# Andrcraft9/ocean_model_arch

Measured on AMD Instinct MI355X. Metric: cell-updates/s, SW barotropic step on 4096x4096 box; %HBM BW at 1/2/4/8 GPU, higher is better.
Workload: dtype f64

## Files before the change

### include/ocn_sw.h

```cpp
#ifndef OCN_SW_H
#define OCN_SW_H

#include <stdint.h>

#ifdef __cplusplus
extern "C" {
#endif

#define OCN_ABI_VERSION 5

enum {
    OCN_OK = 0,
    OCN_ERR_ARG = 1,
    OCN_ERR_HIP = 2,
    OCN_ERR_COMM = 3,
    OCN_ERR_STATE = 4,
    OCN_ERR_BLOWUP = 5
};

typedef struct ocn_block {
    int32_t nx_start, nx_end, ny_start, ny_end;
    int32_t bnd_x1, bnd_x2, bnd_y1, bnd_y2;
    int64_t pitch;
} ocn_block;
// ... 168 lines not shown
int ocn_ctx_comm_info(ocn_ctx *ctx, ocn_comm_info *out);
typedef struct ocn_overlap_info {
    int32_t level, state, kind, pad;
    double seq_ms, overlapped_ms;
} ocn_overlap_info;
int ocn_ctx_overlap_info(ocn_ctx *ctx, ocn_overlap_info *out);
typedef struct ocn_clock_info {
    int64_t launches;
    double clock_ghz, sampled_ms;
} ocn_clock_info;
int ocn_ctx_clock_info(ocn_ctx *ctx, int32_t reset, ocn_clock_info *out);
int ocn_ctx_set_watchdog(ocn_ctx *ctx, double seconds);

int ocn_ctx_set_topography(ocn_ctx *ctx, const float *h, int64_t count);
int ocn_ctx_init_state(ocn_ctx *ctx);

int ocn_ctx_sync(ocn_ctx *ctx, int field_id);
int ocn_ctx_stage(ocn_ctx *ctx, int stage_id, double tau);
int ocn_ctx_tracer_stage(ocn_ctx *ctx, int stage_id, int tracer, double tau);
int ocn_ctx_step(ocn_ctx *ctx, double tau, int32_t nsteps, int32_t check_every);
int ocn_ctx_synchronize(ocn_ctx *ctx);
int ocn_ctx_complete(ocn_ctx *ctx);

int ocn_ctx_download(ocn_ctx *ctx, int k, int field_id, void *host);
int ocn_ctx_upload(ocn_ctx *ctx, int k, int field_id, const void *host);
int ocn_ctx_output_r4(ocn_ctx *ctx, int k, int field_id, float undef, float *host);

int ocn_ctx_set_option(ocn_ctx *ctx, int32_t key, int64_t value);
int ocn_ctx_get_option(const ocn_ctx *ctx, int32_t key, int64_t *value);
enum { OCN_OPT_GRAPH = 1, OCN_OPT_OVERLAP = 2, OCN_OPT_STAGE_TIMING = 3, OCN_OPT_FUSED = 4, OCN_OPT_COMPACT = 5,
       OCN_OPT_MARCH = 6, OCN_OPT_FLIP = 7, OCN_OPT_RECOMPUTE = 8, OCN_OPT_ONEPASS = 9,
       OCN_OPT_KNOWN_CONSTANTS = 10, OCN_OPT_ONEPASS_LAST = 11, OCN_OPT_LAZY_TAIL = 12, OCN_OPT_X2 = 13,
       OCN_OPT_BATCH = 14, OCN_OPT_PAIR = 15, OCN_OPT_MULTI = 16, OCN_OPT_TRACER_STEP = 17,
       OCN_OPT_MULTI_SPIN = 18, OCN_OPT_X4 = 19, OCN_OPT_CO_LAUNCH = 20, OCN_OPT_XCHG_DELAY = 21 };

enum { OCN_TIMER_FUSED_A = OCN_NUM_STAGES, OCN_TIMER_FUSED_B, OCN_TIMER_FUSED_C1, OCN_TIMER_TRACER,
       OCN_TIMER_FUSED_CA = OCN_TIMER_TRACER + OCN_NUM_TSTAGES, OCN_TIMER_ONEPASS, OCN_TIMER_ONEPASS2,
       OCN_TIMER_ONEPASS2_LAST, OCN_TIMER_ONEPASS_MULTI, OCN_TIMER_TRACER_STEP, OCN_TIMER_EXCHANGE,
       OCN_TIMER_EXPOSED, OCN_NUM_TIMERS };

int ocn_ctx_stage_times(ocn_ctx *ctx, double *ms, int64_t *counts);
int ocn_ctx_stage_stats(ocn_ctx *ctx, double *ms, int64_t *counts, double *ms_max);

#define OCN_ENS_MAX_MEMBERS 256
typedef struct ocn_ens_group {
    int32_t variant, rows, tiles, members;
    int32_t member[OCN_ENS_MAX_MEMBERS];
    int32_t first_tile[OCN_ENS_MAX_MEMBERS];
} ocn_ens_group;
int ocn_ens_plan(const ocn_block *geom, const int32_t *variant, int32_t members, int64_t capacity, ocn_ens_group *out,
                 int32_t cap, int32_t *count);

typedef struct ocn_ens ocn_ens;
int ocn_ens_create(const ocn_basin *basin, const ocn_sw_params *sw, const ocn_decomp *dec, const int32_t *mask,
                   int32_t members, ocn_ens **out);
int ocn_ens_destroy(ocn_ens *ens);
int ocn_ens_size(const ocn_ens *ens);
int ocn_ens_member(ocn_ens *ens, int32_t i, ocn_ctx **out);
int ocn_ens_init_state(ocn_ens *ens);
int ocn_ens_step(ocn_ens *ens, double tau, int32_t nsteps, int32_t check_every);
int ocn_ens_complete(ocn_ens *ens);
int ocn_ens_synchronize(ocn_ens *ens, int32_t *status);
typedef struct ocn_ens_info_t {
    int32_t members, groups, batched, rows, tiles, max_group;
    int64_t capacity;
} ocn_ens_info_t;
int ocn_ens_info(ocn_ens *ens, ocn_ens_info_t *out);
// ... 20 lines not shown
```

### ocean_model_arch_amd/_codeobj.py

```python
from __future__ import annotations

import hashlib
import struct

_BUNDLE_MAGIC = b"__CLANG_OFFLOAD_BUNDLE__"


def _sections(elf: bytes):
    if elf[:4] != b"\x7fELF" or elf[4] != 2 or elf[5] != 1:
        raise ValueError("not an ELF64 little-endian image")
    shoff, = struct.unpack_from("<Q", elf, 0x28)
    shentsize, shnum, shstrndx = struct.unpack_from("<HHH", elf, 0x3A)
    hdrs = []
    for i in range(shnum):
        name, _typ, _flags, addr, off, size = struct.unpack_from("<IIQQQQ", elf, shoff + i * shentsize)
        hdrs.append((name, addr, off, size))
    stroff = hdrs[shstrndx][2]
    out = {}
    for i, (name, addr, off, size) in enumerate(hdrs):
        end = elf.index(b"\0", stroff + name)
        out[elf[stroff + name:end].decode()] = (off, size, addr, i)
    return out


# ... 10 lines not shown
            triple = fat[p + 24:p + 24 + tlen].decode()
            p += 24 + tlen
            if triple.endswith("gfx950"):
                yield fat[pos + eoff:pos + eoff + esize]
        pos = fat.find(_BUNDLE_MAGIC, pos + 1)


def gfx950_code_object(lib_path: str) -> bytes:
    for code in gfx950_code_objects(lib_path):
        return code
    raise ValueError("no gfx950 code object in " + lib_path)


def kernel_symbols(code: bytes) -> dict:
    secs = _sections(code)
    symoff, symsize, _a, _i = secs[".symtab"]
    stroff = secs[".strtab"][0]
    by_index = {v[3]: v for v in secs.values()}
    out = {}
    for k in range(symsize // 24):
        st_name, st_info, _other, shndx, value, size = struct.unpack_from("<IBBHQQ", code, symoff + 24 * k)
        if (st_info & 0xF) != 2 or size == 0 or shndx not in by_index:
            continue
        end = code.index(b"\0", stroff + st_name)
        name = code[stroff + st_name:end].decode()
        off, _s, addr, _i = by_index[shndx]
        start = off + (value - addr)
        out[name] = code[start:start + size]
    return out


def march_step_symbol(args: str, batched: bool = False) -> str:
    bits = "".join("Lb1E" if a.strip() == "true" else "Lb0E" for a in args.split(","))
    if batched:
        return f"_ZN3ocn9k_march_bINS_9MarchStepII{bits}EEEEvNS_10MarchGridBENS_4PackIT_EE".replace("II", "I")
    return f"_ZN3ocn7k_marchINS_9MarchStepII{bits}EEEEvNS_9MarchGridET_".replace("II", "I")


def kernel_code_sha(lib_path: str, symbol: str) -> str | None:
    syms = kernel_symbols(gfx950_code_object(lib_path))
    code = syms.get(symbol)
    return hashlib.sha256(code).hexdigest()[:16] if code is not None else None


def sha_by_demangled(lib_path: str, names) -> dict:
    import subprocess
    syms = kernel_symbols(gfx950_code_object(lib_path))
    mangled = sorted(syms)
    dem = subprocess.run(["c++filt"], input="\n".join(mangled), capture_output=True, text=True, check=True).stdout.split("\n")
    key = {"".join(d.split()): m for m, d in zip(mangled, dem)}
    out = {}
    for n in names:
        m = key.get("".join(n.split()))
        if m:
            out[n] = (m, hashlib.sha256(syms[m]).hexdigest()[:16])
    return out
```

### ocean_model_arch_amd/_lib.py

```python
from __future__ import annotations

import ctypes as C
import os
import re
import subprocess

_HERE = os.path.dirname(os.path.abspath(__file__))
LIB_PATH = os.environ.get("OCN_LIB_PATH") or os.path.join(_HERE, "libocn_sw.so")
_CSRC = os.path.join(_HERE, "csrc")

OCN_OK, OCN_ERR_ARG, OCN_ERR_HIP, OCN_ERR_COMM, OCN_ERR_STATE, OCN_ERR_BLOWUP = range(6)

R4_NAMES = ["lu", "luu", "luh", "lcu", "lcv", "llu", "llv", "dx", "dy", "dxt", "dyt", "dxh", "dyh",
            "dxb", "dyb", "rlh_s", "r_diss"]
R8_NAMES = ["ssh", "sshn", "sshp", "ubrtr", "ubrtrn", "ubrtrp", "vbrtr", "vbrtrn", "vbrtrp",
            "hhq", "hhq_p", "hhq_n", "hhu", "hhu_p", "hhu_n", "hhv", "hhv_p", "hhv_n",
            "hhh", "hhh_p", "hhh_n", "hhq_rest", "vort", "str_t", "str_s", "mu",
            "RHSx", "RHSy", "RHSx_adv", "RHSy_adv", "RHSx_dif", "RHSy_dif"]
OCN_FIELD_END = 32 + len(R8_NAMES)
OCN_TRACER_BASE = OCN_FIELD_END + 2
MAX_TRACERS = 64
_TRACER_RE = re.compile(r"^(ff1|ff1p|ff1n)_([0-9]+)$")


# ... 24 lines not shown


def is_r8_name(name: str) -> bool:
    return name not in R4_NAMES

STAGES = ["sw_update_ssh", "hh_update", "uv_trans_vort", "uv_trans", "stress_components", "uv_diff2",
          "sw_update_uv", "sw_next_step", "hh_shift", "hh_init", "check_ssh_err"]
STAGE_ID = {n: i for i, n in enumerate(STAGES)}
TSTAGES = ["tran_diff_fluxes", "tran_diff_tracer", "tracer_next_step"]
TSTAGE_ID = {n: i for i, n in enumerate(TSTAGES)}
TIMERS = STAGES + ["fused_a", "fused_b", "fused_c1"] + TSTAGES + ["fused_ca", "onepass", "onepass2", "onepass2_last", "onepass_multi", "tracer_step",
                                                                       "exchange", "exposed"]
OPT_GRAPH = 1
OPT_OVERLAP = 2
OPT_STAGE_TIMING = 3
OPT_FUSED = 4
OPT_COMPACT = 5
OPT_MARCH = 6
OPT_FLIP = 7
OPT_RECOMPUTE = 8
OPT_ONEPASS = 9
OPT_KNOWN_CONSTANTS = 10
OPT_ONEPASS_LAST = 11
OPT_LAZY_TAIL = 12
OPT_X2 = 13
OPT_BATCH = 14
OPT_PAIR = 15
OPT_MULTI = 16
OPT_TRACER_STEP = 17
OPT_MULTI_SPIN = 18
OPT_X4 = 19
OPT_CO_LAUNCH = 20
OPT_XCHG_DELAY = 21

KERNEL_SYMBOLS = ["ocn_sw_update_ssh", "ocn_hh_update", "ocn_uv_trans_vort", "ocn_uv_trans",
                  "ocn_stress_components", "ocn_uv_diff2", "ocn_sw_update_uv", "ocn_sw_next_step",
                  "ocn_hh_shift", "ocn_hh_init", "ocn_check_ssh_err", "ocn_tran_diff_fluxes",
                  "ocn_tran_diff_tracer", "ocn_tracer_next_step"]
CTX_SYMBOLS = ["ocn_decompose", "ocn_halo_schedule", "ocn_ctx_create", "ocn_ctx_destroy", "ocn_ctx_block_count", "ocn_ctx_block_info",
               "ocn_ctx_field", "ocn_ctx_stream", "ocn_comm_unique_id", "ocn_ctx_attach_comm", "ocn_ctx_attach_loopback",
               "ocn_ctx_set_topography", "ocn_ctx_init_state", "ocn_ctx_sync", "ocn_ctx_stage", "ocn_ctx_tracer_stage", "ocn_ctx_step", "ocn_ctx_synchronize",
               "ocn_ctx_download", "ocn_ctx_complete", "ocn_ctx_upload", "ocn_ctx_output_r4", "ocn_ctx_set_option", "ocn_ctx_get_option", "ocn_ctx_stage_times", "ocn_ctx_stage_stats",
               "ocn_ctx_comm_info", "ocn_ctx_overlap_info", "ocn_ctx_clock_info", "ocn_ctx_set_watchdog", "ocn_last_error", "ocn_abi_version",
               "ocn_build_id", "ocn_launch_count"]
ENS_SYMBOLS = ["ocn_ens_plan", "ocn_ens_create", "ocn_ens_destroy", "ocn_ens_size", "ocn_ens_member",
               "ocn_ens_init_state", "ocn_ens_step", "ocn_ens_complete", "ocn_ens_synchronize", "ocn_ens_info",
               "ocn_ens_set_option", "ocn_ens_stats", "ocn_ens_stats_download", "ocn_ens_stats_output_r4",
               "ocn_ens_extrema"]
ALL_SYMBOLS = KERNEL_SYMBOLS + CTX_SYMBOLS + ENS_SYMBOLS
ENS_MAX_MEMBERS = 256
ENS_OPT_CAPACITY = 1
ENS_OPT_MAX_GROUP = 2
ENS_STATS = {"mean": 1, "var": 2, "spread": 4, "min": 8, "max": 16}


class OcnLibraryError(RuntimeError):
    pass


class OcnError(RuntimeError):
    def __init__(self, code: int, msg: str):
        super().__init__(f"[ocn error {code}] {msg}")
        self.code = code


class OcnBlock(C.Structure):
# ... 162 lines not shown
```

### ocean_model_arch_amd/csrc/ctx_setup.hip

```cpp
#include "ocn_ctx.h"

namespace ocn {

__global__ void k_topography(ocn_block g, double *h, const float *lu, const float *topo, int nxi)
{
    const int w = g.bnd_x2 - g.bnd_x1 + 1, rows = g.bnd_y2 - g.bnd_y1 + 1;
    const long i = (long)blockIdx.x * blockDim.x + threadIdx.x;
    if (i >= (long)w * rows) return;
    const int m = g.bnd_x1 + (int)(i % w), n = g.bnd_y1 + (int)(i / w);
    const long at = (long)(m - g.bnd_x1) + (long)(n - g.bnd_y1) * g.pitch;
    float v = 0.0f;
    if (m >= g.nx_start && m <= g.nx_end && n >= g.ny_start && n <= g.ny_end) v = topo[(long)(m - 3) + (long)(n - 3) * nxi];
    if (fabsf(lu[at]) < 0.5f) v = 0.0f;
    h[at] = (double)v;
}

__global__ void k_fill_r8(double *p, long n, double v)
{
    long i = (long)blockIdx.x * blockDim.x + threadIdx.x;
    if (i < n) p[i] = v;
}

static std::vector<int> uniform_sizes(int total, int parts, std::string &err)
{
// ... 185 lines not shown
        for (int id = OCN_SSH; id < OCN_SSH + nr8; ++id)
            if (std::find(order.begin(), order.end(), id) == order.end()) order.push_back(id);
        for (int k = 1; k <= ntr; ++k) order.push_back(-3 - k);
        b.ffp_alt.assign((size_t)ntr, nullptr);
        for (int id : order) {
            char *p = base + off + 256 - 16 + xr;
            off += r8b;
            if (id == -1) b.sshp_alt = p;
            else if (id == -2) b.up_alt = p;
            else if (id == -3) b.vp_alt = p;
            else if (id < -3) b.ffp_alt[(size_t)(-4 - id)] = p;
            else b.ptr[field_slot(id)] = p;
        }
        for (int id = 0; id < OCN_NUM_R4; ++id) {
            b.ptr[field_slot(id)] = base + off + 256 - 8;
            off += r4b;
        }
    }
    for (LBlock &b : c->blocks) {
        const size_t n = (size_t)b.g.pitch * (b.g.bnd_y2 - b.g.bnd_y1 + 1);
        const size_t nrow = row_table_size((unsigned)(b.g.bnd_y2 - b.g.bnd_y1 + 1));
        HIPCHK(hipMalloc(&b.bits, n));
        c->allocs.push_back(b.bits);
        HIPCHK(hipMalloc(&b.rows, nrow * sizeof(float)));
        c->allocs.push_back(b.rows);
        RC(allocate_x2(c, b));
    }
    const size_t kcb = 16 * c->blocks.size();
    HIPCHK(hipMalloc(&c->d_nbad, 256 + kcb));
    c->allocs.push_back(c->d_nbad);
    HIPCHK(hipMalloc(&c->d_bar, kMultiBarBytes));
    c->allocs.push_back(c->d_bar);
    HIPCHK(hipMemsetAsync(c->d_nbad, 0, 256 + kcb, c->stream));
    c->d_fbz = c->d_nbad + 16;
    c->d_flags = c->d_nbad + 32;
    for (size_t i = 0; i < c->blocks.size(); ++i) c->blocks[i].kc = (double *)((char *)c->d_nbad + 256) + 2 * i;
    return OCN_OK;
}

int prepare_static(ocn_ctx *c)
{
    if (!c->compact_req || c->r4_escaped) { c->compact = false; return OCN_OK; }
    if (!c->static_dirty) return OCN_OK;
    HIPCHK(hipMemsetAsync(c->d_flags, 0, 3 * sizeof(int32_t), c->stream));
    RC(each_block(c, c->stream, [&](const LBlock &b) { return launch_prepare(&b.g, b.ptr.data(), b.bits, b.rows, c->d_flags, c->stream, b.own); }));
    if (c->ext_ok)
        for (const LBlock &b : c->blocks) RC(launch_rows_ext(&b.g, b.rows, b.rows_x, b.ext, c->d_flags + 1, c->stream));
    const bool x4_tabs = c->ext_ok && has_exchange(c);
    int32_t *d_mask = nullptr;
    if (x4_tabs) {
        const size_t nxy = (size_t)c->basin.nx * c->basin.ny;
        HIPCHK(hipMallocAsync((void **)&d_mask, nxy * sizeof(int32_t), c->stream));
        HIPCHK(hipMemcpyAsync(d_mask, c->mask.data(), nxy * sizeof(int32_t), hipMemcpyHostToDevice, c->stream));
        for (const LBlock &b : c->blocks)
            RC(launch_x4_tables(&b.g, b.bits, b.rows, b.ext, b.bits_x4, b.rows_x4, d_mask, c->basin.nx, c->basin.ny, b.own,
                                c->d_flags + 2, c->stream));
        HIPCHK(hipFreeAsync(d_mask, c->stream));
    }
    int32_t flags[3] = {0, 0, 0};
    HIPCHK(hipMemcpyAsync(flags, c->d_flags, sizeof(flags), hipMemcpyDeviceToHost, c->stream));
    HIPCHK(hipStreamSynchronize(c->stream));
    c->ring_sea = (flags[0] & kCompactRingSea) != 0;
    c->edge_ring_sea = (flags[0] & kCompactEdgeRingSea) != 0;
    c->udiv_ok = (flags[0] & kCompactDivisorRange) == 0;
    c->rows_x_ok = c->ext_ok && flags[1] == 0;
    c->x4_tab_ok = x4_tabs && flags[2] == 0;
    c->compact = (flags[0] & ~(kCompactRingSea | kCompactDivisorRange | kCompactEdgeRingSea)) == 0;
    c->static_dirty = false;
    return OCN_OK;
}

static const float kPi = 3.1415926f;
static const double kDPi = 3.14159265358979;
static const double kLatExtr = 89.99999;
static const float kRadEarth = 6371000.0f;
static const float kEarthAngVel = 7.2921159e-5f;
static double dsind(double x) { return std::sin((x / 180.0) * kDPi); }
static double dcosd(double x) { return std::cos((x / 180.0) * kDPi); }

struct GridTables {
    std::vector<float> cos_t, cos_v;
    std::vector<double> sin_v, cosy_v, cos_xu;
    float ext_ct[kExtRows], ext_cv[kExtRows];
    double ext_sin_v[kExtRows], ext_cosy_v[kExtRows];
};
static void grid_tables(const ocn_ctx *c, const ocn_block &g, GridTables &t)
{
    const ocn_basin &bs = c->basin;
    const int w = g.bnd_x2 - g.bnd_x1 + 1, h = g.bnd_y2 - g.bnd_y1 + 1, mmm = 3, nnn = 3;
    std::vector<double> xt(w), xu(w, 0.0), yt(h), yv(h, 0.0);
    for (int m = g.bnd_x1; m <= g.bnd_x2; ++m) xt[m - g.bnd_x1] = bs.rlon + (double)(m - mmm) * bs.dxst;
    for (int n = g.bnd_y1; n <= g.bnd_y2; ++n) yt[n - g.bnd_y1] = bs.rlat + (double)(n - nnn) * bs.dyst;
    for (int i = 0; i + 1 < w; ++i) xu[i] = (xt[i] + xt[i + 1]) / 2.0;
    for (int i = 0; i + 1 < h; ++i) yv[i] = (yt[i] + yt[i + 1]) / 2.0;
    auto lat_mod = [](double y) { return std::max(std::min(y, kLatExtr), -kLatExtr); };
    t.cos_t.assign(h, 0.0f); t.cos_v.assign(h, 0.0f); t.sin_v.assign(h, 0.0); t.cosy_v.assign(h, 0.0);
    t.cos_xu.assign(w, 0.0);
    for (int n = g.ny_start - 1; n <= g.ny_end + 1; ++n) {
        const int r = n - g.bnd_y1;
        t.cos_t[r] = (float)dcosd(lat_mod(yt[r]));
// ... 193 lines not shown
```

### ocean_model_arch_amd/csrc/ocn_ctx.h

```cpp
#pragma once
#include <hip/hip_runtime.h>
#include <rccl/rccl.h>

#include <algorithm>
#include <array>
#include <atomic>
#include <chrono>
#include <cmath>
#include <condition_variable>
#include <cstdio>
#include <cstdlib>
#include <cstring>
#include <deque>
#include <map>
#include <mutex>
#include <string>
#include <thread>
#include <vector>

#include "ocn_internal.h"

namespace ocn {

#define HIPCHK(call)                                          \
// ... 106 lines not shown

#ifndef OCN_COMM_PRIO
#define OCN_COMM_PRIO 1
#endif
struct ocn_ctx {
    ocn_basin basin;
    ocn_sw_params sw;
    ocn_decomp dec;
    std::vector<int32_t> mask;
    std::vector<float> topo;
    int bnx = 1, bny = 1;
    std::vector<GBlock> gblocks;
    std::vector<LBlock> blocks;
    hipStream_t stream = nullptr;
    hipStream_t comm_stream = nullptr;
    hipEvent_t ev_fork = nullptr, ev_join = nullptr;
    hipEvent_t ev_fb = nullptr;
    int32_t *h_fbz = nullptr;
    bool fb_copy = false;
    int overlap = -1;
    int ov_state = 0, ov_kind = 0, ov_level = 2;
    hipEvent_t ov_ev[4] = {nullptr, nullptr, nullptr, nullptr};
    double ov_ms[2] = {0.0, 0.0};
    int xdelay_us = 0;
    int32_t *d_nbad = nullptr;
    unsigned *d_bar = nullptr;
    ncclComm_t comm = nullptr;
    bool comm_aborted = false;
    Loopback *lb = nullptr;
    hipEvent_t lb_ev_a = nullptr, lb_ev_b = nullptr;
    std::map<std::vector<int>, HaloPlan> plans;
    bool initialized = false;
    bool use_graph = false;
    struct Graph { hipGraphExec_t exec; double tau; ocn::StepKind kind; bool compact, march, ring_sea; int role, kc_mode; };
    std::vector<Graph> graphs;
    std::vector<void *> allocs;
    bool stage_timing = false;
    struct Rec { int stage; hipEvent_t a, b; };
    std::vector<Rec> recs;
    std::vector<hipEvent_t> event_pool;
    double stage_ms[OCN_NUM_TIMERS] = {0};
    int64_t stage_n[OCN_NUM_TIMERS] = {0};
    bool fused = true;
    std::vector<int> sync_a, sync_a_reuse, sync_b, sync_ca, sync_ca_reuse;
    bool compact_req = true, compact = false, static_dirty = true;
    bool march = true;
    mutable bool r4_escaped = false;
    bool flip = true, coherent = false, flip_used = false, rc_used = false;
    bool capturing = false;
    bool sync_pending = false;
    bool ring_sea = true;
    bool udiv_ok = true;
    bool recompute = true;
    bool onepass = true;
    int pair = 1;
    bool pair_used = false;
    bool multi = true, multi_used = false;
    bool tr_step = true, tr_call = false, tr_pending = false;
    bool tr_forked = false;
    mutable bool tr_alt_ok = false;
    bool known_const = true;
    bool last_hybrid = true;
    bool one_used = false;
    mutable bool alt_ok = false;
    mutable bool hh_consistent = false, r8_handed = false;
    mutable bool hn_fresh = false;
    mutable bool hqn_stale = false;
    mutable int fb_state = 0;
    int kc_mode = 0;
    int32_t *d_fbz = nullptr;
    bool lazy = true, open = false, open_x2 = false;
    double open_tau = 0.0;
    bool open_pair = false;
    int deferred = 0;
    bool deferred_check[2] = {false, false};
    bool x2 = true, rows_x_ok = false, edge_ring_sea = true, x2_dev_ok = false;
    mutable bool ext_ok = false, hrx_ok = false;
    bool ring2_saved = false, x2_used = false;
    int x4 = 1;
    bool x4_tab_ok = false, x4_dev_ok = false, x4_used = false;
    bool fb_x2 = false;
    mutable bool coherent_known = false, r8_escaped = false;
    int multi_spin = kMultiSpin;
    bool co_launch = true, co_used = false;
    double stage_max[OCN_NUM_TIMERS] = {0};
    int64_t xchg = 0, xdone = -1;
    std::mutex xmu;
    std::deque<std::pair<int64_t, hipEvent_t>> xq;
    std::vector<hipEvent_t> xpool;
    double wd_s = 0;
    std::thread wd;
    std::mutex wd_mu;
    std::condition_variable wd_cv;
    bool wd_stop = false;
    int call_depth = 0;
    std::chrono::steady_clock::time_point call_t0;
    const char *call_name = "";
    std::atomic<bool> wd_fired{false};
    std::string wd_msg;
    std::mutex comm_mu;
    bool comm_abort_done = false;
    int role = 0;
    int steps_run = 0;
    int64_t launches = 0;
    int32_t *d_flags = nullptr;
    bool batch = true;
    ocn::Batcher batcher;
    ocn_ens *ens = nullptr;
    bool ens_collect = false, ens_pending = false;
    ocn::StepKind ens_k{};
};

namespace ocn {

inline int num_r8(const ocn_ctx *c)
{
    return OCN_NUM_R8 + (c->sw.use_tracers > 0 ? 2 + 3 * c->sw.tracer_num : 0);
}
inline bool has_r8(const ocn_ctx *c, int id) { return id >= OCN_SSH && id < OCN_SSH + num_r8(c); }
inline bool has_field(const ocn_ctx *c, int id) { return is_r4(id) || has_r8(c, id); }
inline bool is_tracer_field(int id) { return id >= OCN_TRACER_BASE; }
inline bool is_alt_field(int id) { return id == OCN_SSHP || id == OCN_UBRTRP || id == OCN_VBRTRP; }
inline size_t field_bytes(const LBlock &b) { return (size_t)b.g.pitch * (b.g.bnd_y2 - b.g.bnd_y1 + 1) * 8; }
inline bool has_comm(const ocn_ctx *c) { return c->comm || c->lb || c->comm_aborted; }
inline OnepassKC kc_of(const ocn_ctx *c, const LBlock &b) { return OnepassKC{c->kc_mode, c->d_fbz, b.kc}; }

int make_seglist(ocn_ctx *c, const std::vector<Seg> &v, SegList &out);
int launch_segs(const SegList &l, hipStream_t s, int32_t *cmp = nullptr);
int get_plan(ocn_ctx *c, const std::vector<int> &fields, HaloPlan *&out, int depth = 1, int priv = 0);
int run_sync(ocn_ctx *c, const std::vector<int> &fields, hipStream_t stream = nullptr, int32_t *cmp = nullptr,
             int depth = 1, int priv = 0);
constexpr int kVoteWords = 8;
int allreduce_max(ocn_ctx *c, int32_t *word, hipStream_t s, int words = 1);
int nccl_rc(ncclResult_t r, const char *what);
int fail_fatal(ocn_ctx *c, int rc);
int64_t poll_xdone(ocn_ctx *c);
void wd_loop(ocn_ctx *c);

struct CallGuard {
    ocn_ctx *c;
    CallGuard(ocn_ctx *ctx, const char *name);
    ~CallGuard();
};
template <class F> static int guarded(ocn_ctx *c, const char *name, F &&f)
{
    if (c->wd_fired.load()) return set_error(OCN_ERR_COMM, c->wd_msg);
    int rc;
    {
        CallGuard g(c, name);
        rc = f();
    }
    if (c->wd_fired.load()) {
        std::lock_guard<std::mutex> g(c->comm_mu);
        if (c->comm) { c->comm = nullptr; c->comm_aborted = true; }
        return set_error(OCN_ERR_COMM, c->wd_msg);
    }
    return rc;
}

void set_mask(ocn_ctx *c, const int32_t *mask);
int decompose(ocn_ctx *c);
int host_ctx(const ocn_basin *basin, const ocn_decomp *dec, const int32_t *mask, ocn_ctx *&c);
int allocate(ocn_ctx *c);
int upload_field(ocn_ctx *c, const LBlock &b, int id, const void *host, bool async);
// ... 42 lines not shown
```

### ocean_model_arch_amd/csrc/ocn_ctx.hip

```cpp
#include "ocn_ctx.h"

namespace ocn {

static thread_local std::string g_last_error;

int set_error(int code, const std::string &msg)
{
    g_last_error = msg;
    return code;
}

static std::atomic<long long> g_launches{0};
void count_launch() { g_launches.fetch_add(1, std::memory_order_relaxed); }

int check_hip(hipError_t e, const char *what)
{
    if (e == hipSuccess) return OCN_OK;
    return set_error(OCN_ERR_HIP, std::string(what) + ": " + hipGetErrorString(e));
}

template <typename T>
__global__ void k_output_r4(const T *src, const float *lu, long pitch, int w, int h, float undef, float *dst)
{
    const int i = (int)(blockIdx.x * blockDim.x + threadIdx.x), j = (int)blockIdx.y;
// ... 303 lines not shown
    c->role ^= 16;
}
static int copy_to_alt(ocn_ctx *c, int nsw, bool tracers)
{
    for (LBlock &b : c->blocks) {
        const std::pair<void *, int> sw[3] = {{b.sshp_alt, OCN_SSHP}, {b.up_alt, OCN_UBRTRP}, {b.vp_alt, OCN_VBRTRP}};
        for (int i = 0; i < nsw; ++i)
            HIPCHK(hipMemcpyAsync(sw[i].first, b.ptr[field_slot(sw[i].second)], field_bytes(b), hipMemcpyDeviceToDevice,
                                  c->stream));
        for (int t = 1; tracers && t <= c->sw.tracer_num; ++t)
            HIPCHK(hipMemcpyAsync(b.ffp_alt[(size_t)t - 1], b.ptr[field_slot(OCN_FF1P(t))], field_bytes(b),
                                  hipMemcpyDeviceToDevice, c->stream));
    }
    return OCN_OK;
}
static int copy_pairs(ocn_ctx *c)
{
    for (const LBlock &b : c->blocks)
        for (const auto &pr : kFlipPairs)
            HIPCHK(hipMemcpyAsync(b.ptr[field_slot(pr[1])], b.ptr[field_slot(pr[0])], field_bytes(b),
                                  hipMemcpyDeviceToDevice, c->stream));
    return OCN_OK;
}
static bool is_flip_field(int id)
{
    for (const auto &pr : kFlipPairs)
        if (id == pr[0] || id == pr[1]) return true;
    return id >= OCN_TRACER_BASE && (id - OCN_TRACER_BASE) % 3 != 1;
}

enum { kVoteIncoherent = 0, kVoteIneligible, kVoteUdiv, kVoteHhStale, kVoteX2, kVoteX4, kVoteOvSeq, kVoteOvOv,
       kVoteUsed };
static_assert(kVoteUsed <= kVoteWords, "vote words");
struct VoteIn { bool eligible, udiv_ok, hh_consistent, x2_ok, x4_ok; };
struct VoteOut { bool udiv_ok, hh_consistent, x2_ok, x4_ok; };

struct HaloZero {
    const double *a[6], *d[9];
    int w, h, nxs, nxe, nys, nye, bx1, by1;
    long pitch;
    unsigned own;
};
__global__ void k_halo_zero(HaloZero q, int32_t *flag)
{
    const long i = (long)blockIdx.x * blockDim.x + threadIdx.x;
    if (i >= (long)q.w * q.h) return;
    const int m = q.bx1 + (int)(i % q.w), n = q.by1 + (int)(i / q.w);
    const unsigned cx = m < q.nxs ? 0u : m > q.nxe ? 2u : 1u, cy = n < q.nys ? 0u : n > q.nye ? 2u : 1u;
    if ((cx == 1u && cy == 1u) || ((q.own >> (cx * 3u + cy)) & 1u)) return;
    const long at = (i % q.w) + (i / q.w) * q.pitch;
    auto nz = [&](const double *p) {
        unsigned long long x;
        const double v = p[at];
        __builtin_memcpy(&x, &v, 8);
        return x != 0ull;
    };
    bool bad = false;
    for (int k = 0; k < 6; ++k) bad |= nz(q.a[k]);
    const bool outer = (m == q.nxe + 1 && n >= q.nys - 1 && n <= q.nye + 1) ||
                       (n == q.nye + 1 && m >= q.nxs - 1 && m <= q.nxe + 1);
    if (outer)
        for (int k = 0; k < 9; ++k) bad |= nz(q.d[k]);
    if (bad) atomicOr(flag, 1);
}
static int launch_halo_zero(ocn_ctx *c, int32_t *flag)
{
    static const int ids[6] = {OCN_SSH, OCN_SSHP, OCN_UBRTR, OCN_UBRTRP, OCN_VBRTR, OCN_VBRTRP};
    static const int dids[9] = {OCN_HHU, OCN_HHU_P, OCN_HHU_N, OCN_HHV, OCN_HHV_P, OCN_HHV_N, OCN_HHH, OCN_HHH_P, OCN_HHH_N};
    for (const LBlock &b : c->blocks) {
        HaloZero q{};
        for (int k = 0; k < 6; ++k) q.a[k] = b.f<double>(ids[k]);
        for (int k = 0; k < 9; ++k) q.d[k] = b.f<double>(dids[k]);
        q.w = b.g.bnd_x2 - b.g.bnd_x1 + 1; q.h = b.g.bnd_y2 - b.g.bnd_y1 + 1;
        q.nxs = b.g.nx_start; q.nxe = b.g.nx_end; q.nys = b.g.ny_start; q.nye = b.g.ny_end;
        q.bx1 = b.g.bnd_x1; q.by1 = b.g.bnd_y1; q.pitch = (long)b.g.pitch; q.own = b.own;
        const long pts = (long)q.w * q.h;
        hipLaunchKernelGGL(k_halo_zero, dim3((unsigned)((pts + 255) / 256)), dim3(256), 0, c->stream, q, flag);
        RC(check_launch());
    }
    return OCN_OK;
}

static int check_coherence(ocn_ctx *c, const VoteIn &in, VoteOut &out)
{
    int32_t host[kVoteWords] = {0};
    host[kVoteIneligible] = !in.eligible;
    host[kVoteUdiv] = !in.udiv_ok;
    host[kVoteHhStale] = !in.hh_consistent;
    host[kVoteX2] = !in.x2_ok;
    host[kVoteX4] = !in.x4_ok;
    host[kVoteOvSeq] = host[kVoteOvOv] = INT32_MAX;
    if (c->ov_state == 2) {
        float ms[2] = {0.f, 0.f};
        HIPCHK(hipEventSynchronize(c->ov_ev[3]));
        HIPCHK(hipEventElapsedTime(&ms[0], c->ov_ev[0], c->ov_ev[1]));
        HIPCHK(hipEventElapsedTime(&ms[1], c->ov_ev[2], c->ov_ev[3]));
        for (int i = 0; i < 2; ++i) {
            c->ov_ms[i] = ms[i];
            host[kVoteOvSeq + i] = (int32_t)std::min(1.0e9, std::max(1.0, std::round(1000.0 * ms[i])));
        }
    }
    HIPCHK(hipMemcpyAsync(c->d_flags, host, sizeof(host), hipMemcpyHostToDevice, c->stream));
    if (in.eligible)
        RC(each_block(c, c->stream, [&](const LBlock &b) { return launch_coherence(&b.g, b.ptr.data(), b.bits, c->d_flags, c->stream); }));
    if (in.eligible && c->sw.use_tracers > 0 && c->tr_step)
        for (int t = 1; t <= c->sw.tracer_num; ++t)
            RC(each_block(c, c->stream, [&](const LBlock &b) {
                return launch_tracer_coherence(&b.g, b.ptr.data(), b.bits, t, c->d_flags, c->stream);
            }));
    const bool exch = has_exchange(c);
    if (exch) RC(run_sync(c, kHaloCheck, c->stream, c->d_flags));
    if (exch && c->x2) {
        RC(run_sync(c, {OCN_SSHP, OCN_UBRTRP, OCN_VBRTRP}, c->stream, c->d_flags + kVoteX2));
        if (c->sw.use_tracers > 0 && c->tr_step) RC(run_sync(c, {OCN_MU}, c->stream, c->d_flags + kVoteX2));
        RC(launch_halo_zero(c, c->d_flags + kVoteX2));
    }
    RC(allreduce_max(c, c->d_flags, c->stream, kVoteUsed));
    int32_t w[kVoteWords] = {0};
    HIPCHK(hipMemcpyAsync(w, c->d_flags, sizeof(int32_t) * kVoteUsed, hipMemcpyDeviceToHost, c->stream));
    HIPCHK(hipStreamSynchronize(c->stream));
    c->coherent = w[kVoteIncoherent] == 0 && w[kVoteIneligible] == 0;
    c->coherent_known = !c->r8_escaped && !has_comm(c);
    out.udiv_ok = w[kVoteUdiv] == 0;
    out.hh_consistent = w[kVoteHhStale] == 0;
    out.x2_ok = w[kVoteX2] == 0 && exch && c->x2;
    c->x2_dev_ok = out.x2_ok;
    out.x4_ok = out.x2_ok && w[kVoteX4] == 0;
    if (w[kVoteOvSeq] != INT32_MAX && w[kVoteOvOv] != INT32_MAX) {
        c->ov_ms[0] = 1.0e-3 * w[kVoteOvSeq];
        c->ov_ms[1] = 1.0e-3 * w[kVoteOvOv];
        c->ov_level = w[kVoteOvOv] < w[kVoteOvSeq] ? 2 : 1;
        c->ov_state = 3;
    } else if (c->ov_state == 2) {
        c->ov_state = 0;
    }
    c->x4_dev_ok = out.x4_ok;
    return OCN_OK;
}

static bool flip_eligible(ocn_ctx *c)
{
    return c->flip && c->fused && c->compact && c->march;
}

static bool reuse_allowed(const ocn_ctx *c)
{
    return c->sw.trans_terms > 0 || !(has_exchange(c) || has_comm(c));
}

static int run_tracer_step(ocn_ctx *c, double tau);
static int run_tracer_step(ocn_ctx *c, double tau, hipStream_t st);
static int tracer_step_block(ocn_ctx *c, const LBlock &b, int k, double tau, hipStream_t st);
static std::vector<int> with_tracers(const ocn_ctx *c, const std::vector<int> &fields);

static bool side_fed(const LBlock &b, int side)
{
    static const int diag[5][2] = {{0, 0}, {5, 6}, {7, 8}, {5, 7}, {6, 8}};
    return b.nbr_rank[side - 1] >= 0 || b.nbr_rank[diag[side][0] - 1] >= 0 || b.nbr_rank[diag[side][1] - 1] >= 0;
}
static Range inner_range(const LBlock &b, int ew, int ns)
{
    Range r{b.g.nx_start, b.g.nx_end, b.g.ny_start, b.g.ny_end};
    if (side_fed(b, 2)) r.m0 += ew;
    if (side_fed(b, 1)) r.m1 -= ew;
    if (side_fed(b, 4)) r.n0 += ns;
    if (side_fed(b, 3)) r.n1 -= ns;
    return r;
}
static int band_cols(const LBlock &b, int tile, int depth)
// ... 701 lines not shown
#ifndef OCN_BUILD_ID
#define OCN_BUILD_ID "unknown"
#endif
const char *ocn_build_id(void) { return OCN_BUILD_ID; }
int64_t ocn_launch_count(void) { return (int64_t)g_launches.load(std::memory_order_relaxed); }

extern "C++" int ocn::ctx_create(const ocn_basin *basin, const ocn_sw_params *sw, const ocn_decomp *dec, const int32_t *mask,
                                 hipStream_t shared, ocn_ens *ens, ocn_ctx **out)
{
    if (!basin || !sw || !dec || !out) return set_error(OCN_ERR_ARG, "null argument");
    if (basin->nx < 5 || basin->ny < 5) return set_error(OCN_ERR_ARG, "nx, ny must be >= 5");
    if (dec->bnx < 1 || dec->bny < 1 || dec->nranks < 1 || dec->rank < 0 || dec->rank >= dec->nranks)
        return set_error(OCN_ERR_ARG, "bad decomposition request");
    if (sw->use_tracers > 0 && (sw->tracer_num < 1 || sw->tracer_num > kMaxTracers))
        return set_error(OCN_ERR_ARG, "tracer_num must be 1.." + std::to_string(kMaxTracers));
    ocn_ctx *c = new ocn_ctx();
    c->basin = *basin; c->sw = *sw; c->dec = *dec;
    c->bnx = dec->bnx; c->bny = dec->bny;
    c->ens = ens;
    set_mask(c, mask);
    int rc = check_hip(hipSetDevice(dec->device), "hipSetDevice");
    if (shared) c->stream = shared;
    else if (!rc) rc = check_hip(hipStreamCreateWithFlags(&c->stream, hipStreamNonBlocking), "hipStreamCreate");
    if (!rc) {
        int lo = 0, hi = 0;
        rc = check_hip(hipDeviceGetStreamPriorityRange(&lo, &hi), "hipDeviceGetStreamPriorityRange");
        if (!rc)
            rc = check_hip(hipStreamCreateWithPriority(&c->comm_stream, hipStreamNonBlocking, OCN_COMM_PRIO ? hi : lo),
                           "hipStreamCreateWithPriority");
    }
    if (!rc) rc = check_hip(hipEventCreateWithFlags(&c->ev_fork, hipEventDisableTiming), "hipEventCreate");
    if (!rc) rc = check_hip(hipEventCreateWithFlags(&c->ev_join, hipEventDisableTiming), "hipEventCreate");
    if (!rc) rc = check_hip(hipEventCreateWithFlags(&c->ev_fb, hipEventDisableTiming), "hipEventCreate");
    if (!rc) rc = check_hip(hipHostMalloc((void **)&c->h_fbz, sizeof(int32_t), hipHostMallocDefault), "hipHostMalloc");
    if (!rc) rc = decompose(c);
    if (!rc) rc = allocate(c);
    if (!rc) rc = prebuild_plans(c);
    if (!rc) rc = check_hip(hipStreamSynchronize(c->stream), "hipStreamSynchronize");
    if (rc) { ctx_destroy(c); return rc; }
    *out = c;
    return OCN_OK;
}

int ocn_ctx_create(const ocn_basin *basin, const ocn_sw_params *sw, const ocn_decomp *dec, const int32_t *mask,
                   ocn_ctx **out)
{
    return ctx_create(basin, sw, dec, mask, nullptr, nullptr, out);
}

int ocn_ctx_destroy(ocn_ctx *c)
{
    if (c && c->ens) return set_error(OCN_ERR_ARG, "a member of an ensemble is destroyed by ocn_ens_destroy");
    return ctx_destroy(c);
}

extern "C++" int ocn::ctx_destroy(ocn_ctx *c)
{
    if (!c) return OCN_OK;
    if (c->wd.joinable()) {
        {
            std::lock_guard<std::mutex> g(c->wd_mu);
            c->wd_stop = true;
            c->wd_cv.notify_all();
        }
        c->wd.join();
    }
    (void)hipSetDevice(c->dec.device);
// ... 230 lines not shown
        fields_changed(c, Changed::Stage);
        RC(prepare_static(c));
        return envoke(c, stage_id, tau);
    });
}

static void drop_graphs(ocn_ctx *c)
{
    for (auto &g : c->graphs) (void)hipGraphExecDestroy(g.exec);
    c->graphs.clear();
}

extern "C++" int ocn::run_step(ocn_ctx *c, double tau, const StepKind &k)
{
    if (c->tr_forked) {
        RC(join_sync(c));
        c->tr_forked = false;
    }
    if (c->tr_call && k.one && !k.x2) RC(run_tracer_step(c, tau));
    if (!c->fused) c->hn_fresh = false;
    RC(c->fused ? one_step_fused(c, tau, k) : one_step(c, tau, k.check));
    if (c->tr_call && k.one) {
        c->tr_pending = true;
        return OCN_OK;
    }
    return expl_tracer(c, tau, c->compact);
}

static int graph_step(ocn_ctx *c, double tau, const StepKind &k)
{
    c->hn_fresh = false;
    for (const auto &g : c->graphs)
        if (g.tau == tau && g.kind == k && g.compact == c->compact && g.march == c->march && g.ring_sea == c->ring_sea &&
            g.role == c->role && g.kc_mode == c->kc_mode) {
            HIPCHK(hipGraphLaunch(g.exec, c->stream));
            if (k.rc) swap_sshp(c);
            if (k.one || k.one_last) swap_alt3(c);
            if (k.flip || k.one_last) swap_roles(c);
            return OCN_OK;
        }
    if (c->graphs.size() >= 16) drop_graphs(c);
    const int role = c->role;
    hipGraph_t graph;
    HIPCHK(hipStreamBeginCapture(c->stream, hipStreamCaptureModeThreadLocal));
    c->capturing = true;
    int rc = run_step(c, tau, k);
    c->capturing = false;
    hipError_t e = hipStreamEndCapture(c->stream, &graph);
    if (rc) return rc;
    HIPCHK(e);
    hipGraphExec_t exec;
    e = hipGraphInstantiate(&exec, graph, nullptr, nullptr, 0);
    (void)hipGraphDestroy(graph);
    HIPCHK(e);
    c->graphs.push_back(ocn_ctx::Graph{exec, tau, k, c->compact, c->march, c->ring_sea, role, c->kc_mode});
    HIPCHK(hipGraphLaunch(exec, c->stream));
    return OCN_OK;
}

int ocn_ctx_tracer_stage(ocn_ctx *c, int stage_id, int tracer, double tau)
{
    return entry(c, __func__, [&]() -> int {
        HIPCHK(hipSetDevice(c->dec.device));
        if (c->sw.use_tracers <= 0 || tracer < 1 || tracer > c->sw.tracer_num)
            return set_error(OCN_ERR_ARG, "no such tracer (use_tracers / tracer_num)");
        if (stage_id < 0 || stage_id >= OCN_NUM_TSTAGES) return set_error(OCN_ERR_ARG, "bad tracer stage id");
        RC(complete_open(c));
        return tracer_stage(c, stage_id, tracer, tau, false);
    });
}

static int alt_home(ocn_ctx *c)
{
    if (!(c->role & 4)) return OCN_OK;
    RC(copy_to_alt(c, 3, false));
    swap_alt3(c);
    return OCN_OK;
}

static void learn_fb(ocn_ctx *c)
{
    if (c->fb_state != kFbDevice) return;
    int32_t f = 0;
    if (hipMemcpy(&f, c->d_fbz, sizeof(f), hipMemcpyDeviceToHost) != hipSuccess) return;
    c->fb_state = f == 0 ? kFbZero : f == 1 ? kFbHr : kFbGeneral;
    c->fb_copy = false;
}

static void learn_fb_async(ocn_ctx *c)
{
    if (c->fb_state != kFbDevice || !c->fb_copy || hipEventQuery(c->ev_fb) != hipSuccess) return;
    const int32_t f = *(volatile int32_t *)c->h_fbz;
    c->fb_state = f == 0 ? kFbZero : f == 1 ? kFbHr : kFbGeneral;
    c->fb_copy = false;
}

static int kc_of_fb(const ocn_ctx *c)
{
    return c->fb_state == kFbZero ? OCN_KC_KNOWN : c->fb_state == kFbHr ? OCN_KC_KNOWN_HR
         : c->fb_state == kFbGeneral ? OCN_KC_GENERAL : OCN_KC_DEVICE;
}
static int prepare_kc(ocn_ctx *c, bool x2 = false)
{
    if (!c->known_const || c->r8_handed) { c->kc_mode = OCN_KC_GENERAL; return OCN_OK; }
    learn_fb_async(c);
    if (c->fb_state != kFbUnchecked && x2 && !c->fb_x2) c->fb_state = kFbUnchecked;
    if (c->fb_state == kFbUnchecked) {
        HIPCHK(hipMemsetAsync(c->d_fbz, 0, sizeof(int32_t), c->stream));
        for (const LBlock &b : c->blocks) {
            std::vector<void *> tab = b.ptr;
            if (x2) tab[field_slot(OCN_HHQ_REST)] = b.hr_x;
            const Range r = x2 ? Range{b.g.nx_start, b.g.nx_end, b.g.ny_start, b.g.ny_end} : inner_range(b, 1, 1);
            RC(launch_fallback_check(&b.g, tab.data(), b.bits, r, c->d_fbz, b.kc, c->stream, x2 ? b.own : 0u));
        }
        if (!c->capturing) {
            HIPCHK(hipMemcpyAsync(c->h_fbz, c->d_fbz, sizeof(int32_t), hipMemcpyDeviceToHost, c->stream));
            HIPCHK(hipEventRecord(c->ev_fb, c->stream));
            c->fb_copy = true;
        }
        c->fb_state = kFbDevice;
        c->fb_x2 = x2;
    }
    c->kc_mode = kc_of_fb(c);
    return OCN_OK;
}

extern "C++" int ocn::finish_call(ocn_ctx *c, int rc)
{
    if (const int rj = join_sync(c); rc == OCN_OK) rc = rj;
    if (rc != OCN_OK) c->ring2_saved = false;
    if (c->role & 1) swap_roles(c);
    if (c->role & 2) {
        RC(copy_to_alt(c, 1, false));
        swap_sshp(c);
    }
    if ((c->role & 4) && c->r8_handed) RC(alt_home(c));
    if (c->role & 8) swap_tracer_roles(c);
    if (c->role & 16) {
        RC(copy_to_alt(c, 0, true));
        swap_tracer_alt(c);
    }
    c->tr_pending = false;
    c->hh_consistent = rc == OCN_OK && !c->r8_handed;
    return rc;
}

static bool lazy_allowed(const ocn_ctx *c, bool x2)
{
    return c->lazy && !has_comm(c) && !c->r8_handed && (c->sw.use_tracers <= 0 || c->tr_step) &&
           (x2 || (!c->ring_sea && !has_exchange(c)));
}

static bool x2_local(const ocn_ctx *c)
{
    if (!c->x2 || !c->compact || !c->rows_x_ok || c->edge_ring_sea || !has_exchange(c))
        return false;
    for (const GBlock &g : c->gblocks)
        if (g.rank >= 0 && (g.g.nx_end - g.g.nx_start < 1 || g.g.ny_end - g.g.ny_start < 1)) return false;
    return true;
}

static bool x4_local(const ocn_ctx *c)
{
    if (!c->x4 || !c->x4_tab_ok || !c->known_const || c->r8_handed || (c->sw.use_tracers > 0 && !c->tr_step) ||
        !c->march)
        return false;
    if (c->sw.use_tracers > 0 && c->x4 < 3 && !(has_comm(c) && c->dec.nranks > 1)) return false;
    for (const GBlock &g : c->gblocks)
        if (g.rank >= 0 && (g.g.nx_end - g.g.nx_start < 3 || g.g.ny_end - g.g.ny_start < 3)) return false;
    for (const LBlock &b : c->blocks)
        if (b.g.pitch < (int64_t)(b.g.bnd_x2 - b.g.bnd_x1 + 1 + 2 * kXRing)) return false;
    return true;
}
static bool x4_now(const ocn_ctx *c)
{
    return (c->kc_mode == OCN_KC_KNOWN || c->kc_mode == OCN_KC_KNOWN_HR) &&
           (has_comm(c) ? c->x4_dev_ok : x4_local(c) && c->fb_x2);
}

static int await_kc(ocn_ctx *c, bool x2, int nsteps)
{
    if (c->kc_mode != OCN_KC_DEVICE || !c->fb_copy || c->capturing || has_comm(c) || nsteps < 4) return OCN_OK;
    c->kc_mode = OCN_KC_KNOWN;
    const bool pairs = x2 ? x4_now(c) : pair_ok(c);
    c->kc_mode = OCN_KC_DEVICE;
    if (!pairs) return OCN_OK;
    HIPCHK(hipEventSynchronize(c->ev_fb));
    learn_fb_async(c);
    c->kc_mode = kc_of_fb(c);
    return OCN_OK;
}

static StepKind continuing_step(bool check, bool x2)
{
    StepKind k{};
    k.check = check;
    k.flip = k.one = k.next_one = k.a_done = true;
    k.x2 = x2;
    return k;
}
static StepKind continuing_pair(bool check, bool check2, bool x2)
{
    StepKind k = continuing_step(check, x2);
    k.pair = true;
    k.check2 = check2;
    return k;
}
static StepKind multi_step(bool check, int nsteps)
{
    StepKind k = continuing_step(check, false);
    k.multi = nsteps;
    return k;
}
static StepKind last_step(ocn_ctx *c, bool check)
{
    StepKind k{};
    k.last = k.one_last = true;
    k.check = check;
    k.x2_end = c->ring2_saved;
    c->ring2_saved = false;
    return k;
}
// ... 11 lines not shown
    if (!c->open) return OCN_OK;
    c->open = false;
    HIPCHK(hipSetDevice(c->dec.device));
    if (c->deferred) {
        const int d = c->deferred;
        c->deferred = 0;
        c->open_pair = false;
        if (d == 2 && pair_ok(c))
            return finish_call(c, run_step(c, c->open_tau, last_pair(c->deferred_check[0], c->deferred_check[1])));
        if (d == 2) {
            const StepKind k1 = continuing_step(c->deferred_check[0], c->open_x2);
            if (const int rc = run_step(c, c->open_tau, k1)) return finish_call(c, rc);
        }
        return finish_call(c, run_step(c, c->open_tau, last_step(c, c->deferred_check[d - 1])));
    }
    swap_roles(c);
    swap_alt3(c);
    c->tr_pending = false;
    if (c->open_pair) {
        c->open_pair = false;
        if (pair_ok(c)) return finish_call(c, run_step(c, c->open_tau, last_pair(false, false)));
        if (const int rc = run_step(c, c->open_tau, continuing_step(false, c->open_x2))) return finish_call(c, rc);
        c->tr_pending = false;
    }
    return finish_call(c, run_step(c, c->open_tau, last_step(c, false)));
}

static int step_impl(ocn_ctx *c, double tau, int32_t nsteps, int32_t check_every)
{
    HIPCHK(hipSetDevice(c->dec.device));
    if (nsteps < 0) return set_error(OCN_ERR_ARG, "nsteps < 0");
    if (nsteps == 0) return OCN_OK;
    const bool graph_ok = c->use_graph && !has_comm(c) && !c->stage_timing && !(c->sw.use_tracers > 0 && c->tr_step);
    c->pair_used = false;
    c->co_used = false;
    c->multi_used = false;
    if (c->open) {
        if (tau == c->open_tau && c->onepass && lazy_allowed(c, c->open_x2)) {
            RC(prepare_kc(c, c->open_x2));
            const bool pairs = c->open_x2 ? x4_now(c) : pair_ok(c);
            c->x4_used = c->open_x2 && pairs;
            int rc = OCN_OK;
            if (pairs) {
                std::vector<char> chk(c->deferred_check, c->deferred_check + c->deferred);
                for (int s = 1; s <= nsteps; ++s) chk.push_back(check_every > 0 && (s % check_every == 0));
                c->deferred = 0;
                size_t i = 0;
                for (; i + 2 < chk.size() && rc == OCN_OK; i += 2) {
                    const StepKind k = continuing_pair(chk[i], chk[i + 1], c->open_x2);
                    rc = graph_ok ? graph_step(c, tau, k) : run_step(c, tau, k);
                    c->open_pair = c->pair_used = true;
                }
                if (rc == OCN_OK) {
                    c->deferred = (int)(chk.size() - i);
                    for (int j = 0; j < c->deferred; ++j) c->deferred_check[j] = chk[i + j];
                }
            } else {
                for (int j = 0; j < c->deferred && rc == OCN_OK; ++j)
                    rc = run_step(c, tau, continuing_step(c->deferred_check[j], c->open_x2));
                c->deferred = 0;
                if (!c->open_x2 && !graph_ok && nsteps >= 2 && rc == OCN_OK && multi_ok(c, check_every)) {
                    const StepKind k = multi_step(check_every == 1, nsteps);
                    if (c->ens_collect) { c->ens_k = k; c->ens_pending = true; }
                    else rc = run_step(c, tau, k);
                    c->open_pair = false;
                    c->multi_used = true;
                } else {
                    for (int s = 1; s <= nsteps && rc == OCN_OK; ++s) {
                        const StepKind k = continuing_step(check_every > 0 && (s % check_every == 0), c->open_x2);
                        rc = graph_ok ? graph_step(c, tau, k) : run_step(c, tau, k);
                        c->open_pair = false;
                    }
                }
            }
            if (rc) { c->open = false; c->deferred = 0; c->open_pair = false; return finish_call(c, rc); }
            return OCN_OK;
        }
        RC(complete_open(c));
    }
    RC(prepare_static(c));
    const bool eligible = flip_eligible(c);
    const bool x2_here = x2_local(c);
    const bool x4_here = x2_here && x4_local(c) && (c->fb_state == kFbZero || c->fb_state == kFbHr) && c->fb_x2;
    const bool lazy_cand = eligible && c->onepass && lazy_allowed(c, x2_here);
    bool udiv_ok = c->udiv_ok, first_one = c->hh_consistent, x2_ok = x2_here && c->x2_dev_ok;
    int N = lazy_cand ? nsteps + 1 : nsteps;
    if (N >= 2 && (eligible || (has_comm(c) && c->flip)) && !c->coherent_known) {
        VoteOut v;
        RC(check_coherence(c, VoteIn{eligible, c->udiv_ok, c->hh_consistent, x2_here, x4_here}, v));
        udiv_ok = v.udiv_ok;
        first_one = v.hh_consistent;
        x2_ok = x2_here && v.x2_ok;
    }
    bool flip_call = false, ca = false, one_call = false;
    const bool tr_ok = c->sw.use_tracers <= 0 ||
                       (c->tr_step && first_one &&
                        (has_exchange(c) ? x2_ok && c->last_hybrid
                                         : !c->ring_sea && (c->last_hybrid || (c->blocks.size() == 1 && !has_comm(c)))));
    auto decide = [&](int n) {
        flip_call = n >= 2 && eligible && c->coherent && (c->sw.full_free_surface != 1 || reuse_allowed(c));
        ca = flip_call && c->sw.full_free_surface == 1;
        one_call = ca && c->onepass && (n >= 3 || (n >= 2 && first_one)) && c->sw.trans_terms > 0 &&
                   c->sw.ksw_lat > 0 && tr_ok && udiv_ok;
    };
    decide(N);
    const bool x2_call = one_call && x2_ok && c->last_hybrid;
    const bool lazy_end = lazy_cand && one_call && (nsteps >= 2 || first_one) &&
                          (x2_call || (!c->ring_sea && !has_exchange(c)));
    if (!lazy_end && N != nsteps) decide(N = nsteps);
    c->x2_used = x2_call && one_call;
    c->flip_used = flip_call;
    c->tr_call = c->sw.use_tracers > 0 && one_call;
    c->tr_pending = false;
    if (c->tr_call && !c->tr_alt_ok) {
        RC(copy_to_alt(c, 0, true));
        c->tr_alt_ok = true;
    }
    c->hh_consistent = false;
    const bool last_one = one_call && ((c->blocks.size() == 1 && !has_exchange(c) && !has_comm(c) && !c->ring_sea) ||
                                       c->last_hybrid);
    c->one_used = one_call;
    if (x2_call && one_call) {
// ... 18 lines not shown
    const bool pairs = one_call && (x2_call ? x4_call : pair_ok(c));
    auto plain_one = [&](int s) {
        const bool one = one_call && (s >= 2 || first_one) && s <= N - 1, next_one = one_call && s + 1 <= N - 1;
        const bool next_a = ca && flip_call && s != N && !next_one && !(last_one && s + 1 == N);
        return one && !next_a && !(last_one && s == N);
    };
    int rc = OCN_OK;
    for (int s = 1; s <= nsteps && rc == OCN_OK; ++s) {
        StepKind k;
        k.check = check_every > 0 && (s % check_every == 0);
        k.first = s == 1;
        k.last = s == N;
        k.flip = flip_call && !k.last;
        k.one = one_call && (s >= 2 || first_one) && s <= N - 1;
        k.next_one = one_call && s + 1 <= N - 1;
        k.one_last = last_one && k.last;
        k.a_done = ca && !k.first;
        k.next_a = ca && k.flip && !k.next_one && !(last_one && s + 1 == N);
        k.next_reuse = k.next_a && s + 1 < N;
        k.rc = rc_call && k.flip && !k.first;
        k.rc_next = rc_call && s + 1 < N;
        k.x2 = x2_call && k.one;
        k.x2_save = k.x2 && !c->ring2_saved;
        k.x2_end = k.one_last && c->ring2_saved;
        if (k.x2_save) c->ring2_saved = true;
        if (k.x2_end) c->ring2_saved = false;
        if (pairs && k.one && s + 1 < nsteps && plain_one(s + 1)) {
            k.pair = true;
            k.check2 = check_every > 0 && ((s + 1) % check_every == 0);
            k.next_one = one_call && s + 2 <= N - 1;
            k.next_a = k.next_reuse = false;
            ++s;
            c->pair_used = true;
        }
        rc = graph_ok ? graph_step(c, tau, k) : run_step(c, tau, k);
    }
    if (lazy_end && rc == OCN_OK) {
        c->open = true;
        c->open_pair = false;
        c->deferred = 0;
        c->open_tau = tau;
        c->open_x2 = x2_call;
        return OCN_OK;
    }
    return finish_call(c, rc);
}

extern "C++" int ocn::step_entry(ocn_ctx *c, double tau, int32_t nsteps, int32_t check_every)
{
    if (!c->initialized) return set_error(OCN_ERR_STATE, "ocn_ctx_init_state not called");
    return fail_fatal(c, step_impl(c, tau, nsteps, check_every));
}

int ocn_ctx_step(ocn_ctx *c, double tau, int32_t nsteps, int32_t check_every)
{
    return entry(c, __func__, [&] { return step_entry(c, tau, nsteps, check_every); });
}

int ocn_ctx_complete(ocn_ctx *c)
{
    return entry(c, __func__, [&] { return complete_open(c); });
}

static int run_deferred(ocn_ctx *c)
{
    if (!c->open || !c->deferred) return OCN_OK;
// ... 155 lines not shown
        return OCN_OK;
    case OCN_OPT_OVERLAP:
        if (c->overlap != value) drop_graphs(c);
        c->overlap = value < 0 ? -1 : value > 2 ? 2 : (int)value;
        if (c->overlap < 0) c->ov_state = 0;
        return OCN_OK;
    case OCN_OPT_XCHG_DELAY: c->xdelay_us = value < 0 ? 0 : value > 1000000 ? 1000000 : (int)value; return OCN_OK;
    case OCN_OPT_MARCH:
        if (c->march != (value != 0)) drop_graphs(c);
        c->march = value != 0;
        return OCN_OK;
    case OCN_OPT_FLIP: c->flip = value != 0; return OCN_OK;
    case OCN_OPT_RECOMPUTE: c->recompute = value != 0; return OCN_OK;
    case OCN_OPT_ONEPASS: c->onepass = value != 0; return OCN_OK;
    case OCN_OPT_ONEPASS_LAST: c->last_hybrid = value != 0; return OCN_OK;
    case OCN_OPT_KNOWN_CONSTANTS:
        c->known_const = value != 0;
        return OCN_OK;
    case OCN_OPT_LAZY_TAIL: c->lazy = value != 0; return OCN_OK;
    case OCN_OPT_X2: c->x2 = value != 0; c->coherent_known = false; return OCN_OK;
    case OCN_OPT_PAIR: c->pair = value < 0 ? 0 : value > 2 ? 2 : (int)value; return OCN_OK;
    case OCN_OPT_MULTI: c->multi = value != 0; return OCN_OK;
    case OCN_OPT_TRACER_STEP:
        c->tr_step = value != 0;
        c->coherent_known = false;
        return OCN_OK;
    case OCN_OPT_MULTI_SPIN: c->multi_spin = value < 1 ? 1 : value > kMultiSpin ? kMultiSpin : (int)value; return OCN_OK;
    case OCN_OPT_X4:
        c->x4 = value <= 0 ? 0 : value >= 3 ? 3 : 1;
        c->coherent_known = false;
        c->hrx_ok = false;
        return OCN_OK;
    case OCN_OPT_CO_LAUNCH: c->co_launch = value != 0; return OCN_OK;
    case OCN_OPT_BATCH:
        if (c->batch != (value != 0)) drop_graphs(c);
        c->batch = value != 0;
        return OCN_OK;
    case OCN_OPT_COMPACT:
        c->compact_req = value != 0;
        c->r4_escaped = false;
        c->static_dirty = true;
        return OCN_OK;
    default: return set_error(OCN_ERR_ARG, "unknown option");
    }
}

int ocn_ctx_get_option(const ocn_ctx *c, int32_t key, int64_t *value)
{
    if (!c || !value) return set_error(OCN_ERR_ARG, "null argument");
    switch (key) {
    case OCN_OPT_GRAPH: *value = c->use_graph; return OCN_OK;
    case OCN_OPT_STAGE_TIMING: *value = c->stage_timing; return OCN_OK;
    case OCN_OPT_FUSED: *value = c->fused; return OCN_OK;
    case OCN_OPT_OVERLAP: *value = overlap_level(c); return OCN_OK;
    case OCN_OPT_COMPACT: *value = c->compact; return OCN_OK;
    case OCN_OPT_MARCH: *value = c->march; return OCN_OK;
    case OCN_OPT_FLIP: *value = c->flip && c->flip_used; return OCN_OK;
    case OCN_OPT_RECOMPUTE: *value = c->recompute && c->rc_used; return OCN_OK;
    case OCN_OPT_ONEPASS: {
        const bool z = c->kc_mode == OCN_KC_KNOWN || (c->kc_mode == OCN_KC_DEVICE && c->fb_state == kFbZero);
        const bool h = c->kc_mode == OCN_KC_KNOWN_HR || (c->kc_mode == OCN_KC_DEVICE && c->fb_state == kFbHr);
        *value = c->onepass && c->one_used ? (z ? 2 : h ? 3 : 1) : 0;
        return OCN_OK;
    }
    case OCN_OPT_KNOWN_CONSTANTS: *value = c->known_const; return OCN_OK;
    case OCN_OPT_ONEPASS_LAST: *value = c->last_hybrid; return OCN_OK;
    case OCN_OPT_LAZY_TAIL: *value = c->open ? 2 : c->lazy; return OCN_OK;
    case OCN_OPT_X2: *value = c->x2 && c->x2_used; return OCN_OK;
    case OCN_OPT_BATCH: *value = c->batch; return OCN_OK;
    case OCN_OPT_PAIR: *value = c->pair_used ? 2 : c->pair > 0; return OCN_OK;
    case OCN_OPT_MULTI: *value = c->multi_used ? 2 : c->multi; return OCN_OK;
    case OCN_OPT_TRACER_STEP: *value = c->tr_call ? 2 : c->tr_step; return OCN_OK;
    case OCN_OPT_MULTI_SPIN: *value = c->multi_spin; return OCN_OK;
    case OCN_OPT_X4: *value = c->x4_used ? 2 : c->x4 ? 1 : 0; return OCN_OK;
    case OCN_OPT_CO_LAUNCH: *value = c->co_used ? 2 : c->co_launch; return OCN_OK;
    case OCN_OPT_XCHG_DELAY: *value = c->xdelay_us; return OCN_OK;
    default: return set_error(OCN_ERR_ARG, "unknown option");
    }
}

}
```

### ocean_model_arch_amd/csrc/ocn_internal.h

```cpp
#pragma once
#include <hip/hip_runtime.h>

#include <initializer_list>
#include <string>
#include <vector>

#include "../../include/ocn_sw.h"

#ifndef OCN_TW
#define OCN_TW 64
#endif
#ifndef OCN_ROWS
#define OCN_ROWS 8
#endif
#ifndef OCN_XCD_REMAP
#define OCN_XCD_REMAP 1
#endif
#define OCN_WY (256 / OCN_TW)
static_assert(OCN_TW % 64 == 0 && 256 % OCN_TW == 0, "OCN_TW must be 64, 128 or 256");

#ifndef OCN_FIELD_SKEW
#define OCN_FIELD_SKEW 0
#endif
static_assert(OCN_FIELD_SKEW % 256 == 0, "OCN_FIELD_SKEW must keep fields 256-B aligned");
// ... 36 lines not shown
                    const ocn_sw_params &sw, int32_t *nbad, hipStream_t s, const double *sshp_in = nullptr,
                    const double *up_in = nullptr, const double *vp_in = nullptr);
struct TailCopy { const double *src[3]; double *dst[3]; };
int launch_fused_c2(const ocn_block *b, void *const *ptr, int nptr, const Compact *cp, int part,
                    const ocn_sw_params &sw, bool full, hipStream_t s, bool keep_n = false,
                    const TailCopy *copy = nullptr);
int launch_fused_ca(const ocn_block *b, void *const *ptr, int nptr, const Compact *cp, int part,
                    const ocn_sw_params &sw, double tau_next, bool next_reuse, bool skip_rc, hipStream_t s,
                    const Range *inner = nullptr);
size_t row_table_size(unsigned nrows);

struct GridInit {
    ocn_block g;
    const int32_t *mask;
    int nx;
    float *r4[OCN_NUM_R4];
    const float *cos_t, *cos_v;
    const double *sin_v, *cosy_v, *cos_xu;
    double cos_rot, sin_rot, sin_extr;
    float sx, sy, cor, sqrt2;
    int curve;
    static constexpr int kExt = 6;
    float ext_ct[kExt], ext_cv[kExt];
    double ext_sin_v[kExt], ext_cosy_v[kExt];
    float *ext;
};
constexpr int kExtRows = GridInit::kExt;
constexpr int kExtRowFloats = kExtRows * (OCN_NUM_R4 - OCN_DX);
constexpr int kXRing = 2;
int launch_init_grid(const GridInit &q, hipStream_t s);
int launch_gaussian(const ocn_block &g, double *p, const float *lu, int nx0, int ny0, double sigma, hipStream_t s);
int launch_fill_field(const ocn_block &g, double *p, double v, hipStream_t s);
enum { OCN_KC_GENERAL = 0, OCN_KC_KNOWN = 1, OCN_KC_DEVICE = 2, OCN_KC_KNOWN_HR = 3 };
struct OnepassKC { int mode; const int32_t *flag; const double *kc; };
int launch_onepass(const ocn_block *b, void *const *ptr, int nptr, const Compact *cp, const ocn_sw_params &sw,
                   double tau, int32_t *nbad, double *sshp_out, double *up_out, double *vp_out, hipStream_t s,
                   const Range *range, bool last, const OnepassKC &kc, unsigned own = 0,
                   const Range *frame_of = nullptr);
int clock_read(bool reset, unsigned long long out[3]);
int launch_onepass_pair(const ocn_block *b, void *const *ptr, int nptr, const Compact *cp, const ocn_sw_params &sw,
                        double tau, int32_t *nbad1, int32_t *nbad2, double *sshp_out, double *up_out, double *vp_out,
                        hipStream_t s, const OnepassKC &kc, bool last = false);
int launch_onepass_pair_x4(const ocn_block *bx, void *const *ptr, int nptr, const Compact *cp, const ocn_sw_params &sw,
                           double tau, int32_t *nbad1, int32_t *nbad2, double *sshp_out, double *up_out, double *vp_out,
                           hipStream_t s, const OnepassKC &kc, unsigned own, const Range *range = nullptr,
                           int nblk = 1, const Range *frame_of = nullptr, double *const *trs = nullptr);
int launch_x4_tables(const ocn_block *g, const uint8_t *bits, const float *rows, const float *ext, uint8_t *bits4,
                     float *rows4, const int32_t *mask, int nx, int ny, unsigned own, int32_t *flags, hipStream_t s);
constexpr size_t kMultiBarBytes = 17 * 128;
constexpr int kMultiSpin = 1 << 20;
int onepass_multi_fits(const ocn_block *b);
int launch_onepass_multi(const ocn_block *b, void *const *ptr, int nptr, const Compact *cp, const ocn_sw_params &sw,
                         double tau, int nsteps, int32_t *nbad, double *sshp_alt, double *up_alt, double *vp_alt,
                         unsigned *ctr, int32_t *err, hipStream_t s, const OnepassKC &kc, int spin = kMultiSpin);
struct EnsMember {
    const ocn_block *b;
    void *const *ptr;
    int nptr;
    const Compact *cp;
    int32_t *nbad;
    double *alt[3];
    unsigned *ctr;
    int32_t *err;
    const double *kc;
    int spin;
};
int onepass_multi_variant(int kc_mode, double tau, bool check);
size_t onepass_multi_b_entry_bytes();
long onepass_multi_b_capacity();
int launch_onepass_multi_b(const EnsMember *m, int n, int variant, int rows, const ocn_sw_params &sw, double tau,
                           int nsteps, void *d_tab, void *h_tab, size_t tab_bytes, long capacity, hipStream_t s);
constexpr int kEnsStatsReg = 32;
int launch_ens_stats(const ocn_block *b, const double *const *src, int n, bool need_var, double *const out[5],
                     hipStream_t s);
struct EnsPartial { double min, max; long long nonfinite, count; };
struct EnsExtBlock { long off, pitch; int w, h, first_tile, tiles_x; };
struct EnsExtSrc { const double *src; const float *lu; };
int ens_extrema_tiles(int w, int h, int *tiles_x);
int launch_ens_extrema(const EnsExtBlock *d_blk, int nblk, const EnsExtSrc *d_tab, int members, int ntiles,
                       EnsPartial *d_part, EnsPartial *d_out, hipStream_t s);
int launch_fallback_check(const ocn_block *b, void *const *ptr, const uint8_t *bits, const Range &r, int32_t *flag,
                          double *kc, hipStream_t s, unsigned own = 0);
int launch_prepare(const ocn_block *b, void *const *ptr, uint8_t *bits, float *rows, int32_t *flags, hipStream_t s,
                   unsigned own = 0);
int launch_rows_ext(const ocn_block *b, const float *rows, float *rows_x, const float *ext, int32_t *flags,
                    hipStream_t s);
constexpr int kCompactEdgeRingSea = 16;
int launch_stage(const ocn_block *b, void *const *ptr, int nptr, const Compact *cp, int stage, const ocn_sw_params &sw,
                 double tau, int32_t *nbad, hipStream_t s);
int launch_tracer(const ocn_block *b, void *const *ptr, int nptr, const Compact *cp, int stage, int k, double tau,
                  double ts, hipStream_t s);
int launch_tracer_step(const ocn_block *b, void *const *ptr, int nptr, const Compact *cp, int k, double tau,
                       double ts, double *ffn_out, double *ffp_out, unsigned own, hipStream_t s, bool ext = false);
int launch_coherence(const ocn_block *b, void *const *ptr, const uint8_t *bits, int32_t *flags, hipStream_t s);
int launch_tracer_coherence(const ocn_block *b, void *const *ptr, const uint8_t *bits, int k, int32_t *flags,
                            hipStream_t s);
constexpr int kCompactRingSea = 4;
constexpr int kCompactDivisorRange = 8;

struct BatchEntry {
    virtual ~BatchEntry() {}
    virtual int flush(hipStream_t s) = 0;
    virtual bool co_flush(BatchEntry *next, hipStream_t s, int &rc) { (void)next; (void)s; (void)rc; return false; }
    const void *kind = nullptr;
};
struct Batcher {
    bool active = false;
    bool co_launch = false;
    int co_launched = 0;
    hipStream_t s = nullptr;
    int cur = -1;
    std::vector<BatchEntry *> entries;
    int flush();
    ~Batcher();
};
extern thread_local Batcher *g_batcher;
void batch_begin(Batcher *bt, hipStream_t s);
inline void batch_next(Batcher *bt) { if (bt) bt->cur = -1; }
int batch_end(Batcher *bt);

int check_hip(hipError_t e, const char *what);
void count_launch();
int batch_violation();
inline int check_launch()
{
    count_launch();
    if (g_batcher && g_batcher->active) return batch_violation();
    return check_hip(hipGetLastError(), "kernel launch");
}

}
// ... 1 lines not shown
```

### ocean_model_arch_amd/csrc/sw_kernels.hip

```cpp
#include <hip/hip_runtime.h>

#include <climits>
#include <cmath>
#include <cstdlib>
#include <cstring>
#include <map>
#include <mutex>
#include <type_traits>

#include "ocn_internal.h"
#include "sw_stencils.h"

namespace ocn {

#define RC_KB(x) do { int _rc = (x); if (_rc) return _rc; } while (0)

template <typename Body>
__device__ __forceinline__ void range_tile(int w0, int m0, int m1, int n0, int n1, int ntx, int tile, const Body &body)
{
    const int tx = tile % ntx, ty = tile / ntx;
    const int m = w0 + tx * OCN_TW + (int)threadIdx.x;
    if (m < m0 || m > m1) return;
    const int nb = n0 + ty * OCN_ROWS;
    const int ne = min(n1, nb + OCN_ROWS - 1);
// ... 1454 lines not shown
typedef unsigned ocn_u32x2 __attribute__((ext_vector_type(2)));
template <int AUX = 0>
__device__ __forceinline__ void st_on(double *p, unsigned nbytes, unsigned i, double v, bool on)
{
    const __amdgpu_buffer_rsrc_t r = __builtin_amdgcn_make_buffer_rsrc(p, (short)0, (int)nbytes, 0x00020000);
    __builtin_amdgcn_raw_buffer_store_b64(__builtin_bit_cast(ocn_u32x2, v), r, on ? i * 8u : 0xfffffff8u, 0, AUX);
}

__device__ __forceinline__ double udiv(double x, double d, double rd)
{
    const double q = x * rd;
    const double t = __builtin_fma(q, d, -x);
    return __builtin_fma(-t, rd, q);
}
__device__ __forceinline__ void exp_check(int &acc, double x)
{
    acc = min(acc, __builtin_amdgcn_frexp_exp(x));
}
constexpr int kUdivMinExp = -899;

enum RowC { RC_DX, RC_DY, RC_DXT, RC_DYT, RC_DXH, RC_DYH, RC_DXB, RC_DYB, RC_RDXT, RC_RDYH, RC_RDXH, RC_RDYT,
            RC_RDXB, RC_RDYB, RC_RAT0, RC_RAT1, RC_RAT2, RC_RAT3, RC_RLH, RC_DY2, RC_DX2, RC_AREA, RC_RAREA,
            RC_DXB2, RC_DYB2, RC_RDSELF, RC_RDNEXT, kRowC };
#ifndef OCN_PAIR_WAVES
#define OCN_PAIR_WAVES OCN_STEP_WAVES
#endif
#ifndef OCN_PAIR_MAX_ROWS
#define OCN_PAIR_MAX_ROWS 150
#endif
constexpr int kStepLdsRows = 4 * OCN_STEP_ROWS + 4 > OCN_PAIR_MAX_ROWS + 10 ? 4 * OCN_STEP_ROWS + 4 : OCN_PAIR_MAX_ROWS + 10;

__shared__ double g_step_rc[kStepLdsRows * kRowC];
__shared__ unsigned g_step_rlo;
__shared__ double g_pair[4][6][120];

__device__ __forceinline__ double row_const(const float *rows, unsigned nrows, unsigned r, int k)
{
    auto g = [&](int id) { return rows[(unsigned)(id - OCN_DX) * nrows + r]; };
    auto rc = [&](int j) { return ((const double *)(rows + recip_offset(nrows)))[(unsigned)j * nrows + r]; };
    switch (k) {
    case RC_DX: return D(g(OCN_DX));
    case RC_DY: return D(g(OCN_DY));
    case RC_DXT: return D(g(OCN_DXT));
    case RC_DYT: return D(g(OCN_DYT));
    case RC_DXH: return D(g(OCN_DXH));
    case RC_DYH: return D(g(OCN_DYH));
    case RC_DXB: return D(g(OCN_DXB));
    case RC_DYB: return D(g(OCN_DYB));
    case RC_RDXT: return rc(OCN_RC_DXT);
    case RC_RDYH: return rc(OCN_RC_DYH);
    case RC_RDXH: return rc(OCN_RC_DXH);
    case RC_RDYT: return rc(OCN_RC_DYT);
    case RC_RDXB: return rc(OCN_RC_DXB);
    case RC_RDYB: return rc(OCN_RC_DYB);
    case RC_RAT0: case RC_RAT1: case RC_RAT2: case RC_RAT3:
        return D(rows[(unsigned)(kNumRowFields + k - RC_RAT0) * nrows + r]);
    case RC_RLH: return D(g(OCN_RLH_S));
    case RC_DY2: { const float a = g(OCN_DY); return D(a * a); }
    case RC_DX2: { const float a = g(OCN_DX); return D(a * a); }
    case RC_AREA: { const float a = g(OCN_DX) * g(OCN_DY); return D(a); }
    case RC_RAREA: return rc(OCN_RC_AREA);
    case RC_DXB2: { const float a = g(OCN_DXB); return D(a * a); }
    case RC_DYB2: { const float a = g(OCN_DYB); return D(a * a); }
    case RC_RDSELF: { const float a = g(OCN_R_DISS); const float rd = a + a; return D(rd); }
    case RC_RDNEXT: {
        const float a = g(OCN_R_DISS), an = rows[(unsigned)(OCN_R_DISS - OCN_DX) * nrows + min(r + 1, nrows - 1)];
// ... 13 lines not shown
    const unsigned hi = c == 0 ? 0x7ff00000u : 0x3ff00000u - ((c >> 1) << 20);
    return __builtin_bit_cast(double, (unsigned long long)hi << 32);
}

constexpr int kRing = 5;

struct StepRegs {
    template <class T> struct Win {
        T r[kRing];
        template <int PH> __device__ __forceinline__ T &s(int k) { return r[(PH + k) % kRing]; }
        template <int PH> __device__ __forceinline__ T s(int k) const { return r[(PH + k) % kRing]; }
        template <int PH> __device__ __forceinline__ T at(int dx, int dy) const
        {
            if (dy < -1 || dy > 2) ocn_march_bad_access();
            return shz(s<PH>(dy + 1), dx);
        }
        __device__ __forceinline__ void rotate() { r[0] = r[1]; r[1] = r[2]; r[2] = r[3]; }
    };
    Win<double> u, v, up, vp, ssh, shp, hr, mu;
    Win<unsigned> bits;
    double rhsx, rhsy;
    Win<double> hu, hv, hh, hu1, hv1, vort, stt, sts;
    Win<double> w0, w1;
    Win<double> pu, pv, vh, t3, cx, rr, dt, dxq;
    Win<double> w0r, vr;
    const __attribute__((address_space(4))) float *rows;
    const __attribute__((address_space(4))) double *rcp;
    unsigned nrows, rn;
    double qb, qc;
    double tau, inv_tau, f;
    int32_t *nbp;
    bool cnt;
    int pj;
    double fyx, fyy, vht, a2t;
    double hr0, mu0;
    const __attribute__((address_space(3))) double *lds;
    unsigned rlo;
    template <bool LDS> __device__ __forceinline__ double cst(int k, int dy) const
    {
        if (LDS) return lds[(rn + dy - rlo) * kRowC + k];
        switch (k) {
        case RC_RDXT: return rc(OCN_RC_DXT, dy);
        case RC_RDYH: return rc(OCN_RC_DYH, dy);
        case RC_RDXH: return rc(OCN_RC_DXH, dy);
        case RC_RDYT: return rc(OCN_RC_DYT, dy);
        case RC_RDXB: return rc(OCN_RC_DXB, dy);
        case RC_RDYB: return rc(OCN_RC_DYB, dy);
        case RC_RAREA: return rc(OCN_RC_AREA, dy);
        default: break;
        }
        return row_const_s(k, dy);
    }
    __device__ __forceinline__ double row_const_s(int k, int dy) const
    {
        auto g = [&](int id) { return met(id, dy); };
        switch (k) {
        case RC_DX: return D(g(OCN_DX));
        case RC_DY: return D(g(OCN_DY));
        case RC_DXT: return D(g(OCN_DXT));
        case RC_DYT: return D(g(OCN_DYT));
        case RC_DXH: return D(g(OCN_DXH));
        case RC_DYH: return D(g(OCN_DYH));
        case RC_DXB: return D(g(OCN_DXB));
        case RC_DYB: return D(g(OCN_DYB));
        case RC_RAT0: case RC_RAT1: case RC_RAT2: case RC_RAT3: return D(met(OCN_DX + kNumRowFields + k - RC_RAT0, dy));
        case RC_RLH: return D(g(OCN_RLH_S));
        case RC_DY2: { const float a = g(OCN_DY); return D(a * a); }
        case RC_DX2: { const float a = g(OCN_DX); return D(a * a); }
        case RC_AREA: { const float a = g(OCN_DX) * g(OCN_DY); return D(a); }
        case RC_DXB2: { const float a = g(OCN_DXB); return D(a * a); }
        case RC_DYB2: { const float a = g(OCN_DYB); return D(a * a); }
        case RC_RDSELF: { const float a = g(OCN_R_DISS); const float rd = a + a; return D(rd); }
// ... 9 lines not shown
    {
        return rows[(unsigned)(id - OCN_DX) * nrows + row(dy)];
    }
    __device__ __forceinline__ double rc(int k, int dy) const
    {
        return rcp[(unsigned)k * nrows + row(dy)];
    }
    __device__ __forceinline__ void rotate()
    {
        u.rotate(); v.rotate(); up.rotate(); vp.rotate(); ssh.rotate(); shp.rotate(); hr.rotate(); mu.rotate();
        bits.rotate();
        hu.rotate(); hv.rotate(); hh.rotate(); hu1.rotate(); hv1.rotate(); vort.rotate(); stt.rotate(); sts.rotate();
        w0.rotate(); w1.rotate(); pu.rotate(); pv.rotate(); vh.rotate(); t3.rotate(); cx.rotate(); rr.rotate();
        w0r.rotate(); vr.rotate();
        dt.rotate(); dxq.rotate();
    }
    template <int PH> __device__ __forceinline__ unsigned bit(int id, int dx, int dy) const
    {
        return (bits.at<PH>(dx, dy) >> id) & 1u;
    }
    template <int PH> __device__ __forceinline__ float mk(int id, int dx, int dy) const
    {
        return (bits.at<PH>(dx, dy) >> id) & 1u ? 1.0f : 0.0f;
    }
    template <int PH> __device__ __forceinline__ double mkd(int id, int dx, int dy) const
    {
        const unsigned hi = ((bits.at<PH>(dx, dy) >> id) & 1u) * 0x3ff00000u;
        return __builtin_bit_cast(double, (unsigned long long)hi << 32);
    }
};

#define OCN_MD(id, dy) D(x.met((id), (dy)))

template <bool P2, bool LAST = false, bool ZF = false, bool X2 = false, bool HR = false, bool PAIR = false,
          bool WT = false>
struct MarchStep {
    static_assert(!PAIR || !X2 || (ZF && !LAST), "two-step launches with exchanges: the known-constant variants");
    static constexpr int kStAux = WT ? 16 : 0;
    static constexpr bool kPair = PAIR;
    static constexpr bool kX2 = X2;
    static constexpr bool kCoTracer = X2 && ZF && !HR && !LAST && !WT;
    static constexpr int kPairCols = 116;
    static constexpr bool kAligned = false;
    static constexpr int kHalo = 2;
    static constexpr int kWaves = PAIR ? OCN_PAIR_WAVES : OCN_STEP_WAVES;
    ocn_block b; Tab<true> t; ocn_sw_params sw; double tau; int32_t *nbad;
    double *sshp_out, *up_out, *vp_out;
    const double *kc; const int32_t *fbz; int gate;
    unsigned own;
    int32_t *nbad2 = nullptr;
    double *trs[4] = {nullptr, nullptr, nullptr, nullptr};
    static constexpr bool kGate = true;
    __device__ __forceinline__ bool enabled() const
    {
        if (gate == 0) return true;
        const int f = *(const volatile int32_t *)fbz;
        return gate == 1 ? f == 0 : gate == 3 ? f == 1 : (f & 2) != 0;
    }

    __device__ __forceinline__ double qtau(const StepRegs &x, double a) const { return P2 ? a * x.inv_tau : a / x.tau; }

    struct Batch { double u, v, up, vp, ssh, shp, hr, mu, rhsx, rhsy; unsigned bits; };
    __device__ __forceinline__ int rowc(int r, int RO) const { return RO == 1 ? min(max(r, b.bnd_y1), b.bnd_y2) : r; }
    template <int RO = 0> __device__ __forceinline__ void load(const StepRegs &x, Batch &q, int m, int n) const
    {
        if constexpr (RO == 2) {
            const Geo I = geo(&b);
            const Pt c2 = I(m, n + 2);
            q.ssh = g_pair[(n + 2) & 3][0][x.pj]; q.shp = g_pair[(n + 2) & 3][1][x.pj];
            q.u = g_pair[(n + 2) & 3][2][x.pj]; q.up = g_pair[(n + 2) & 3][3][x.pj];
            q.v = g_pair[(n + 1) & 3][4][x.pj]; q.vp = g_pair[(n + 1) & 3][5][x.pj];
            q.hr = ZF && !HR ? x.hr0 : ld(t.f(OCN_HHQ_REST), c2);
            q.bits = ld(t.bits, c2);
            if (ZF) {
                q.mu = x.mu0;
                q.rhsx = q.rhsy = 0.0;
            } else {
                q.mu = ld(t.f(OCN_MU), I(m, n + 1));
                q.rhsx = ld(t.f(OCN_RHSX), I(m, n));
                q.rhsy = ld(t.f(OCN_RHSY), I(m, n));
            }
            return;
        }
        const Geo I = geo(&b);
        const Pt c = I(m, rowc(n, RO)), c1 = I(m, rowc(n + 1, RO)), c2 = I(m, rowc(n + 2, RO));
        q.u = ld(t.f(OCN_UBRTR), c2); q.up = ld(t.f(OCN_UBRTRP), c2);
        q.ssh = ld(t.f(OCN_SSH), c2); q.shp = ld(t.f(OCN_SSHP), c2);
        q.hr = ZF && !HR ? x.hr0 : ld(t.f(OCN_HHQ_REST), c2);
        q.bits = ld(t.bits, c2);
        q.v = ld(t.f(OCN_VBRTR), c1); q.vp = ld(t.f(OCN_VBRTRP), c1); q.mu = ZF ? x.mu0 : ld(t.f(OCN_MU), c1);
        if (ZF) q.rhsx = q.rhsy = 0.0;
        else { q.rhsx = ld(t.f(OCN_RHSX), c); q.rhsy = ld(t.f(OCN_RHSY), c); }
    }
    template <int PH> __device__ __forceinline__ static void take(StepRegs &x, const Batch &q)
    {
        x.u.s<PH>(3) = q.u; x.up.s<PH>(3) = q.up; x.ssh.s<PH>(3) = q.ssh; x.shp.s<PH>(3) = q.shp; x.hr.s<PH>(3) = q.hr;
        x.bits.s<PH>(3) = q.bits;
        x.v.s<PH>(2) = q.v; x.vp.s<PH>(2) = q.vp; x.mu.s<PH>(2) = q.mu;
        x.rhsx = q.rhsx; x.rhsy = q.rhsy;
    }

    template <int PH> __device__ __forceinline__ static void weights(StepRegs &x, int dy)
    {
        const int k = dy + 1;
        const double gx = x.cst<kLds>(RC_DX, dy), gy = x.cst<kLds>(RC_DY, dy);
        const double l = x.mkd<PH>(OCN_LU, 0, dy);
        x.w0.s<PH>(k) = (x.hr.s<PH>(k) + x.ssh.s<PH>(k)) * gx * gy * l;
        x.w1.s<PH>(k) = (x.hr.s<PH>(k) + x.shp.s<PH>(k)) * gx * gy * l;
        x.w0r.s<PH>(k) = shz(x.w0.s<PH>(k), 1);
    }

    struct Fallback {
        bool llu, llv, luh, vt, st, ss;
        double hu, hv, hh, hu1, hv1, vort, stt, sts;
    };
    template <int PH, int RO = 0>
    __device__ __forceinline__ void fallback(const StepRegs &x, Fallback &f, int m, int r, int slot) const
    {
        const Pt c = geo(&b)(m, rowc(r, RO));
        const unsigned bc = x.bits.s<PH>(slot);
        bool hh_rng = m >= b.nx_start - 1 && m <= b.nx_end && r >= b.ny_start - 1 && r <= b.ny_end;
        bool in = m >= b.nx_start && m <= b.nx_end && r >= b.ny_start && r <= b.ny_end;
        if (X2) {
            const bool owned = (own >> (own_class(m, b.nx_start, b.nx_end) * 3u + own_class(r, b.ny_start, b.ny_end))) & 1u;
            hh_rng = hh_rng || owned;
            in = in || owned;
        }
        f.llu = hh_rng && (bc & (1u << OCN_LLU));
        f.llv = hh_rng && (bc & (1u << OCN_LLV));
        f.luh = hh_rng && (bc & (1u << OCN_LUH));
        f.vt = in && (bc & (1u << OCN_LUU));
        f.st = in && (bc & (1u << OCN_LU));
// ... 21 lines not shown
            for (int i = 0; i < N; ++i) out[i] = a[i] / d[i];
        } else {
            double q[N], t[N];
#pragma unroll
            for (int i = 0; i < N; ++i) q[i] = a[i] * rd[i];
#pragma unroll
            for (int i = 0; i < N; ++i) t[i] = __builtin_fma(q[i], d[i], -a[i]);
#pragma unroll
            for (int i = 0; i < N; ++i) out[i] = __builtin_fma(-t[i], rd[i], q[i]);
        }
    }
    template <bool E, int PH>
    __device__ __forceinline__ void derive(StepRegs &x, const Fallback &fb, int &acc, double &qb_next,
                                           double &qc_next) const
    {
        weights<PH>(x, 2);
        const unsigned b00 = x.bit<PH>(OCN_LU, 0, 1), b10 = x.bit<PH>(OCN_LU, 1, 1), b01 = x.bit<PH>(OCN_LU, 0, 2),
                       b11 = x.bit<PH>(OCN_LU, 1, 2);
        const unsigned cu = b00 + b10, cv = b00 + b01, ch = cu + b01 + b11;
        const double dxt = x.cst<kLds>(RC_DXT, 1), dyt = x.cst<kLds>(RC_DYT, 1), dxh = x.cst<kLds>(RC_DXH, 1),
                     dyh = x.cst<kLds>(RC_DYH, 1), dxb = x.cst<kLds>(RC_DXB, 1), dyb = x.cst<kLds>(RC_DYB, 1);
        const double w00 = x.w0.s<PH>(2), w10 = x.w0r.s<PH>(2), w01 = x.w0.s<PH>(3), w11 = x.w0r.s<PH>(3);
        const double p00 = x.w1.s<PH>(2), p10 = shz(p00, 1), p01 = x.w1.s<PH>(3);
        const double s0 = w00 + w10;
        const double rxt = x.cst<kLds>(RC_RDXT, 1), ryh = x.cst<kLds>(RC_RDYH, 1), rxh = x.cst<kLds>(RC_RDXH, 1),
                     ryt = x.cst<kLds>(RC_RDYT, 1);
        const double ru = rcp_sea(cu), rv = rcp_sea(cv);
        const double a_u0 = s0 * ru, a_v0 = (w00 + w01) * rv, a_u1 = (p00 + p10) * ru, a_v1 = (p00 + p01) * rv;
        const double sh = s0 + w01 + w11;
        const double a_h0 = ch == 3 ? (E ? sh / 3.0 : udiv(sh, 3.0, 1.0 / 3.0)) : sh * rcp_sea(ch);
        if (!E) exp_check(acc, sh);
        if (!E) {
            exp_check(acc, a_u0); exp_check(acc, a_v0); exp_check(acc, a_h0); exp_check(acc, a_u1);
            exp_check(acc, a_v1); exp_check(acc, x.up.s<PH>(2)); exp_check(acc, x.vp.s<PH>(2)); exp_check(acc, x.up.s<PH>(3));
        }
        double q1[9], q2[5];
        dvn<E, 9>({a_u0, a_v0, a_h0, a_u1, a_v1, x.up.s<PH>(2), x.vp.s<PH>(2), x.up.s<PH>(3), x.vp.s<PH>(2)},
                  {dxt, dxh, dxb, dxt, dxh, dyh, dxh, x.cst<kLds>(RC_DXT, 2), dyt},
                  {rxt, rxh, x.cst<kLds>(RC_RDXB, 1), rxt, rxh, ryh, rxh, x.cst<kLds>(RC_RDXT, 2), ryt}, q1);
        dvn<E, 5>({q1[0], q1[1], q1[2], q1[3], q1[4]}, {dyh, dyt, dyb, dyh, dyt},
                  {ryh, ryt, x.cst<kLds>(RC_RDYB, 1), ryh, ryt}, q2);
        const double u0 = q2[0], v0 = q2[1], h0 = q2[2], u1 = q2[3], v1 = q2[4];
        const double u_0 = x.u.s<PH>(2), u_1 = x.u.s<PH>(3), v_0 = x.v.s<PH>(2), v_r = shz(v_0, 1);
        x.vr.s<PH>(2) = v_r;
        const double vort = (v_r * dyt - v_0 * dyt) - (u_1 * x.cst<kLds>(RC_DXT, 2) - u_0 * dxt)
                            - ((v_r - v_0) * dyb - (u_1 - u_0) * dxb);
        const double qa = q1[5], qb = q1[6], qc1 = q1[7], qe = q1[8];
        const double st = x.cst<kLds>(RC_RAT0, 1) * (qa - shz(qa, -1)) - x.cst<kLds>(RC_RAT1, 1) * (qb - x.qb);
        const double ss = x.cst<kLds>(RC_RAT2, 1) * (qc1 - x.qc) + x.cst<kLds>(RC_RAT3, 1) * (shz(qe, 1) - qe);
        qb_next = qb;
        qc_next = qc1;
        const double hu = fb.llu ? u0 : fb.hu;
        const double hv = fb.llv ? v0 : fb.hv;
        const double hh = fb.luh ? h0 : fb.hh;
        const double vt = fb.vt ? vort : fb.vort;
        const double stt = fb.st ? st : fb.stt;
        x.hu.s<PH>(2) = hu; x.hv.s<PH>(2) = hv; x.hh.s<PH>(2) = hh; x.vort.s<PH>(2) = vt; x.stt.s<PH>(2) = stt;
        x.hu1.s<PH>(2) = fb.llu ? u1 : fb.hu1;
        x.hv1.s<PH>(2) = fb.llv ? v1 : fb.hv1;
        x.sts.s<PH>(2) = fb.ss ? ss : fb.sts;
        x.pu.s<PH>(2) = u_0 * dyh * hu;
        x.pv.s<PH>(2) = v_0 * dxh * hv;
        x.vh.s<PH>(2) = vt * hh;
        x.t3.s<PH>(2) = v_0 * hv * dxh;
        const double rr = x.cst<kLds>(RC_RLH, 1) * hh * dxb * dyb;
        x.rr.s<PH>(2) = rr;
        x.cx.s<PH>(2) = rr * (v_r + v_0);
        const double hq = x.hr.s<PH>(2) + x.ssh.s<PH>(2);
        if constexpr (kLds) {
            x.dt.s<PH>(2) = x.cst<kLds>(RC_DY2, 1) * hq * stt;
            x.dxq.s<PH>(2) = x.cst<kLds>(RC_DX2, 1) * hq * stt;
        } else {
            x.dt.s<PH>(2) = x.cst<kLds>(RC_DY2, 1) * x.mu.s<PH>(2) * hq * stt;
            x.dxq.s<PH>(2) = x.cst<kLds>(RC_DX2, 1) * x.mu.s<PH>(2) * hq * stt;
        }
    }

    template <int PH> __device__ __forceinline__ void face(StepRegs &x) const
    {
        const double u = x.u.s<PH>(1), v = x.v.s<PH>(1), u_n = x.u.s<PH>(2), v_n = x.v.s<PH>(2);
        const double v_r = x.vr.s<PH>(1);
        const double pv = x.pv.s<PH>(1), pvn = x.pv.s<PH>(2), luu = x.mkd<PH>(OCN_LUU, 0, 0);
        x.fyx = (pv + shz(pv, 1)) / 2.0 * (u_n + u) / 2.0 * luu;
        x.vht = x.vh.s<PH>(1) * (v_r + v);
        x.fyy = (pv + pvn) / 2.0 * (v + v_n) / 2.0;
        if constexpr (ZF) {
            const double mu = x.mu.s<PH>(1), mu_n = x.mu.s<PH>(2), muh_p = (mu + mu + mu_n + mu_n) / 4.0;
            (void)muh_p;
            x.a2t = x.cst<kLds>(RC_DXB2, 0) * x.hh.s<PH>(1) * x.sts.s<PH>(1);
        }
    }

    struct Out {
        bool lu = false, cu = false, cv = false, uu = false;
        double sshn = 0.0, fx = 0.0, un = 0.0, fa = 0.0, vn = 0.0, fb = 0.0;
        double vort = 0.0, sts = 0.0, stt = 0.0, rxa = 0.0, rxd = 0.0, rya = 0.0, ryd = 0.0;
        double fyx = 0.0, fyy = 0.0, vht = 0.0, a2t = 0.0;
    };
    template <bool E, int PH>
    __device__ __forceinline__ void step(const StepRegs &x, const Lane &L, int n, int &acc, bool &bad, Out &o) const
    {
        (void)n;
        const double u = x.u.s<PH>(1), v = x.v.s<PH>(1), hu = x.hu.s<PH>(1), hv = x.hv.s<PH>(1), hh = x.hh.s<PH>(1);
        const double dxt = x.cst<kLds>(RC_DXT, 0), dyt = x.cst<kLds>(RC_DYT, 0), dxh = x.cst<kLds>(RC_DXH, 0),
                     dyh = x.cst<kLds>(RC_DYH, 0);
        const double t1 = u * hu * dyh;
        const double a_ssh = t1 - shz(t1, -1) + x.t3.s<PH>(1) - x.t3.s<PH>(0);
        if (!E) exp_check(acc, a_ssh);
        const double u_r = shz(u, 1), u_n = x.u.s<PH>(2);
        const double v_r = x.vr.s<PH>(1), v_n = x.v.s<PH>(2);
        const double pu = x.pu.s<PH>(1), pun = x.pu.s<PH>(2), pv = x.pv.s<PH>(1), pvn = x.pv.s<PH>(2);
        const double luu = x.mkd<PH>(OCN_LUU, 0, 0);
        double rxa, rya;
        {
            const double fx_p = (pu + shz(pu, 1)) / 2.0 * (u + u_r) / 2.0;
            const double fx_m = shz(fx_p, -1);
            const double fy_p = (pv + shz(pv, 1)) / 2.0 * (u_n + u) / 2.0 * luu;
            const double cor = x.vh.s<PH>(1) * (v_r + v);
            rxa = -(fx_p - fx_m + fy_p - x.fyx) + (cor + x.vht) / 4.0;
            o.fyx = fy_p;
            o.vht = cor;
        }
        {
            const double fy_p = (pv + pvn) / 2.0 * (v + v_n) / 2.0;
            const double sn = pu + pun;
            const double fx_p = sn / 2.0 * (v_r + v) / 2.0;
            const double fx_m = shz(fx_p, -1);
            const double q = x.vh.s<PH>(1) * (u_n + u);
            rya = -(fx_p - fx_m + fy_p - x.fyy) - (q + shz(q, -1)) / 4.0;
            o.fyy = fy_p;
        }
        double rxd, ryd;
        double q_ssh = 0.0;
        {
            auto sh = [](double a, int d) { return ZF ? a : shz(a, d); };
            const double mu = x.mu.s<PH>(1), mu_r = sh(mu, 1), mu_l = sh(mu, -1), mu_n = x.mu.s<PH>(2), mu_s = x.mu.s<PH>(0);
            const double muh_p = (mu + mu_r + mu_n + sh(mu_n, 1)) / 4.0;
            const double muh_m = (mu + mu_r + mu_s + sh(mu_s, 1)) / 4.0;
            const double muh_m2 = (mu + mu_l + mu_n + sh(mu_n, -1)) / 4.0;
            const double dxb2 = x.cst<kLds>(RC_DXB2, 0), dxb2m = x.cst<kLds>(RC_DXB2, -1), dyb2 = x.cst<kLds>(RC_DYB2, 0);
            const double sts = x.sts.s<PH>(1);
            const double dtc = x.dt.s<PH>(1);
            double a2, a4;
            if constexpr (ZF) {
                (void)dxb2m; (void)muh_m; (void)muh_m2;
                (void)muh_p;
                const double a2p = dxb2 * hh * sts, a4p = dyb2 * hh * sts;
                a2 = a2p - x.a2t;
                a4 = a4p - shz(a4p, -1);
                o.a2t = a2p;
            } else {
                a2 = dxb2 * muh_p * hh * sts - dxb2m * muh_m * x.hh.s<PH>(0) * x.sts.s<PH>(0);
                a4 = dyb2 * muh_p * hh * sts - dyb2 * muh_m2 * shz(hh, -1) * shz(sts, -1);
            }
            const double a1 = shz(dtc, 1) - dtc, a3 = x.dxq.s<PH>(2) - x.dxq.s<PH>(1);
            {
                if (!E) { exp_check(acc, a1); exp_check(acc, a2); exp_check(acc, a3); exp_check(acc, a4); }
                double qd[5];
                dvn<E, 5>({a_ssh, a1, a2, a3, a4}, {x.cst<kLds>(RC_AREA, 0), dyh, dxt, dxh, dyt},
                          {x.cst<kLds>(RC_RAREA, 0), x.cst<kLds>(RC_RDYH, 0), x.cst<kLds>(RC_RDXT, 0),
                           x.cst<kLds>(RC_RDXH, 0), x.cst<kLds>(RC_RDYT, 0)}, qd);
                q_ssh = qd[0];
                rxd = qd[1] + qd[2];
                ryd = -qd[3] + qd[4];
            }
        }
        const double sshn = x.shp.s<PH>(1) + 2.0 * x.tau * (-q_ssh);
        double un, vn;
        {
            const double g = D(OCN_FREE_FALL_ACC);
            const double ssh = x.ssh.s<PH>(1);
            {
                const double bp = qtau(x, hu * dxt * dyh / 2.0);
                const double bp0 = qtau(x, x.hu1.s<PH>(1) * dxt * dyh / 2.0);
                const double slx = -(g * (shz(ssh, 1) - ssh) * dyh * hu);
                const double fric = (kLds ? x.cst<kLds>(RC_RDSELF, 0) : x.cst<kLds>(RC_RDSELF, 0) / 2.0) * x.up.s<PH>(1) * dxt *
                                    dyh * hu;
                const double grx = x.rhsx + slx + rxd + rxa - fric + (x.cx.s<PH>(1) + x.cx.s<PH>(0)) / 4.0;
                un = (x.up.s<PH>(1) * bp0 + grx) / (bp);
            }
            {
                const double bp = qtau(x, hv * dyt * dxh / 2.0);
                const double bp0 = qtau(x, x.hv1.s<PH>(1) * dyt * dxh / 2.0);
                const double sly = -(g * (x.ssh.s<PH>(2) - ssh) * dxh * hv);
                const double fric = (kLds ? x.cst<kLds>(RC_RDNEXT, 0) : x.cst<kLds>(RC_RDNEXT, 0) / 2.0) * x.vp.s<PH>(1) * dxh *
                                    dyt * hv;
                const double c1 = x.rr.s<PH>(1) * (u_n + u);
                const double gry = x.rhsy + sly + ryd + rya - fric - (c1 + shz(c1, -1)) / 4.0;
                vn = (x.vp.s<PH>(1) * bp0 + gry) / (bp);
            }
        }
        const double ts = sw.time_smooth;
        const double fx = asselin(x.ssh.s<PH>(1), sshn, x.shp.s<PH>(1), ts);
        const double fa = asselin(u, un, x.up.s<PH>(1), ts), fb = asselin(v, vn, x.vp.s<PH>(1), ts);
        const unsigned bc = x.bits.s<PH>(1);
        o.lu = L.out && (bc & (1u << OCN_LU));
        o.cu = L.out && (bc & (1u << OCN_LCU));
        o.cv = L.out && (bc & (1u << OCN_LCV));
        o.sshn = sshn; o.fx = fx; o.un = un; o.fa = fa; o.vn = vn; o.fb = fb;
        if (LAST) {
            o.uu = L.out && (bc & (1u << OCN_LUU));
            o.vort = x.vort.s<PH>(1); o.sts = x.sts.s<PH>(1); o.stt = x.stt.s<PH>(1);
            o.rxa = rxa; o.rxd = rxd; o.rya = rya; o.ryd = ryd;
        }
        const bool bd = o.lu && !(sshn < 10000.0 && sshn > -10000.0);
        if (__builtin_expect(x.nbp && x.cnt && bd != (E && bad), 0)) atomicAdd(x.nbp, bd ? 1 : -1);
        bad = bd;
    }

    __device__ __forceinline__ void store_out(const Out &o, unsigned c) const
    {
        const unsigned nbytes = (unsigned)b.pitch * (unsigned)(b.bnd_y2 - b.bnd_y1 + 1) * 8u;
        st_on<kStAux>(t.f(OCN_SSHN), nbytes, c, o.sshn, o.lu);
        st_on<kStAux>(sshp_out, nbytes, c, o.fx, o.lu);
        st_on<kStAux>(t.f(OCN_UBRTRN), nbytes, c, o.un, o.cu);
        st_on<kStAux>(up_out, nbytes, c, o.fa, o.cu);
        st_on<kStAux>(t.f(OCN_VBRTRN), nbytes, c, o.vn, o.cv);
        st_on<kStAux>(vp_out, nbytes, c, o.fb, o.cv);
        if (LAST) {
            st_on<kStAux>(t.f(OCN_VORT), nbytes, c, o.vort, o.uu);
            st_on<kStAux>(t.f(OCN_STR_S), nbytes, c, o.sts, o.uu);
            st_on<kStAux>(t.f(OCN_STR_T), nbytes, c, o.stt, o.lu);
            st_on<kStAux>(t.f(OCN_RHSX_ADV), nbytes, c, o.rxa, o.cu);
            st_on<kStAux>(t.f(OCN_RHSX_DIF), nbytes, c, o.rxd, o.cu);
            st_on<kStAux>(t.f(OCN_RHSY_ADV), nbytes, c, o.rya, o.cv);
            st_on<kStAux>(t.f(OCN_RHSY_DIF), nbytes, c, o.ryd, o.cv);
        }
    }

    __device__ __forceinline__ static void pair_barrier()
    {
        __builtin_amdgcn_fence(__ATOMIC_RELEASE, "workgroup", "local");
        __builtin_amdgcn_s_barrier();
        __builtin_amdgcn_fence(__ATOMIC_ACQUIRE, "workgroup", "local");
    }
    template <int PH> __device__ __forceinline__ void pair_put(const StepRegs &x, const Out &o, int n) const
    {
        const int lane = (int)threadIdx.x & 63;
        if (lane >= kHalo && lane < 64 - kHalo) {
            double(*r)[120] = g_pair[n & 3];
            r[0][x.pj] = o.lu ? o.sshn : x.ssh.s<PH>(1);
            r[1][x.pj] = o.lu ? o.fx : x.shp.s<PH>(1);
            r[2][x.pj] = o.cu ? o.un : x.u.s<PH>(1);
            r[3][x.pj] = o.cu ? o.fa : x.up.s<PH>(1);
            r[4][x.pj] = o.cv ? o.vn : x.v.s<PH>(1);
            r[5][x.pj] = o.cv ? o.fb : x.vp.s<PH>(1);
        }
    }
    static constexpr bool kLds = ZF;
    static constexpr bool kUnroll = ZF;
    static constexpr bool kPrologue = kLds;
    __device__ void prologue(const MarchRect &R, int ty) const
    {
        const int h = R.vert ? 4 * R.rows : R.rows, nb = R.n0 + ty * h;
        if (nb > R.n1) return;
        const int ne = min(R.n1, nb + h - 1), lo = nb - (PAIR ? 5 : 2) - b.bnd_y1, i = (int)threadIdx.x;
        if (i < ne - nb + (PAIR ? 10 : 5)) {
            const unsigned r = (unsigned)min(max(lo + i, 0), (int)t.nrows - 1);
            const double mu0 = kc[1], muh = (mu0 + mu0 + mu0 + mu0) / 4.0;
#pragma unroll
            for (int k = 0; k < kRowC; ++k) {
                double v = row_const(t.rows, t.nrows, r, k);
                if (k == RC_DY2 || k == RC_DX2) v = v * mu0;
                else if (k == RC_DXB2 || k == RC_DYB2) v = v * muh;
                else if (k == RC_RDSELF || k == RC_RDNEXT) v = v / 2.0;
                g_step_rc[i * kRowC + k] = v;
            }
        }
        if (threadIdx.x == 0) g_step_rlo = (unsigned)lo;
        if constexpr (!PAIR) __syncthreads();
    }

    __device__ void march(const Lane &L, int nb, int ne) const
    {
        if constexpr (PAIR) {
            if (L.pr == 1) {
                march_role<1>(L, nb - 2, ne + 2);
                pair_barrier();
                pair_barrier();
            } else {
#pragma unroll
                for (int k = 0; k < 5 + (kPrologue ? 1 : 0); ++k) pair_barrier();
                march_role<2>(L, nb, ne);
            }
            return;
        }
        march_role<0>(L, nb, ne);
    }
    template <int RO> __device__ void march_role(const Lane &L, int nb, int ne) const
    {
        const Geo I = geo(&b);
        StepRegs x{};
        x.nbp = RO == 2 ? nbad2 : nbad;
        x.cnt = true;
        x.pj = L.j;
        if (kLds) x.lds = (const __attribute__((address_space(3))) double *)g_step_rc;
        x.rows = (const __attribute__((address_space(4))) float *)t.rows;
        x.rcp = (const __attribute__((address_space(4))) double *)(t.rows + recip_offset(t.nrows));
        x.nrows = t.nrows;
        x.rn = (unsigned)(nb - 2 - b.bnd_y1);
        x.tau = tau;
        x.inv_tau = 1.0 / tau;
        x.f = (double)sw.full_free_surface;
        if (ZF) { x.hr0 = kc[0]; x.mu0 = kc[1]; }
        const int n0 = nb - 2;
        {
            const Pt c = I(L.m, rowc(n0, RO)), c1 = I(L.m, rowc(n0 + 1, RO));
            if constexpr (RO == 2) {
                x.ssh.s<0>(2) = g_pair[(n0 + 1) & 3][0][x.pj]; x.shp.s<0>(2) = g_pair[(n0 + 1) & 3][1][x.pj];
                x.u.s<0>(2) = g_pair[(n0 + 1) & 3][2][x.pj]; x.up.s<0>(2) = g_pair[(n0 + 1) & 3][3][x.pj];
                x.vp.s<0>(1) = g_pair[n0 & 3][5][x.pj];
            } else {
                x.up.s<0>(2) = ld(t.f(OCN_UBRTRP), c1); x.ssh.s<0>(2) = ld(t.f(OCN_SSH), c1);
                x.shp.s<0>(2) = ld(t.f(OCN_SSHP), c1); x.u.s<0>(2) = ld(t.f(OCN_UBRTR), c1);
                x.vp.s<0>(1) = ld(t.f(OCN_VBRTRP), c);
            }
            x.hr.s<0>(2) = ZF && !HR ? x.hr0 : ld(t.f(OCN_HHQ_REST), c1);
            x.bits.s<0>(2) = ld(t.bits, c1);
        }
        Fallback fb;
        fallback<0, RO>(x, fb, L.m, n0 + 1, 2);
        Batch q;
        load<RO>(x, q, L.m, n0);
        if constexpr (PAIR && RO == 1 && kPrologue) pair_barrier();
        if (kLds) x.rlo = g_step_rlo;
        x.qb = x.vp.s<0>(1) / x.cst<kLds>(RC_DXH, 0);
        x.qc = x.up.s<0>(2) / x.cst<kLds>(RC_DXT, 1);
        weights<0>(x, 1);
        if (RO != 1) store_out(Out{}, 0u);
        if constexpr (RO == 2) pair_barrier();
        iteration<0, true, RO>(x, fb, q, L, n0, nb, ne);
        if constexpr (kUnroll) {
            iteration<1, true, RO>(x, fb, q, L, n0 + 1, nb, ne);
            for (int n = nb;; n += kRing) {
                if (iteration<2, false, RO>(x, fb, q, L, n, nb, ne)) break;
                if (iteration<3, false, RO>(x, fb, q, L, n + 1, nb, ne)) break;
                if (iteration<4, false, RO>(x, fb, q, L, n + 2, nb, ne)) break;
                if (iteration<0, false, RO>(x, fb, q, L, n + 3, nb, ne)) break;
                if (iteration<1, false, RO>(x, fb, q, L, n + 4, nb, ne)) break;
            }
        } else {
            x.rotate();
            iteration<0, true, RO>(x, fb, q, L, n0 + 1, nb, ne);
            x.rotate();
            for (int n = nb;; ++n) {
                if (iteration<0, false, RO>(x, fb, q, L, n, nb, ne)) break;
                x.rotate();
            }
        }
    }

    template <int PH, bool WARM = false, int RO = 0>
    __device__ __forceinline__ bool iteration(StepRegs &x, Fallback &fb, Batch &q, const Lane &L0, int n, int nb,
                                              int ne) const
    {
        Lane L = L0;
        asm volatile("" : "+v"(L.m));
        if (RO == 1) {
            const bool iny = n >= b.ny_start && n <= b.ny_end;
            if constexpr (X2) {
                const bool inx = L.m >= b.nx_start && L.m <= b.nx_end;
                const bool owned =
                    (own >> (own_class(L.m, b.nx_start, b.nx_end) * 3u + own_class(n, b.ny_start, b.ny_end))) & 1u;
                L.out = L.out && ((inx && iny) || owned);
            } else {
                L.out = L.out && iny;
            }
            x.cnt = L.ccol && n >= nb + 2 && n <= ne - 2;
        }
        take<PH>(x, q);
        Fallback fbn;
        if (n < ne) fallback<PH, RO>(x, fbn, L.m, n + 2, 3);
        if (n < ne) load<RO>(x, q, L.m, n + 1);
        Out o;
        {
            int acc = 0;
            double qb, qc;
            derive<false, PH>(x, fb, acc, qb, qc);
            if (__builtin_expect(__builtin_amdgcn_ballot_w64(acc < kUdivMinExp) != 0, 0))
                derive<true, PH>(x, fb, acc, qb, qc);
            acc = 0;
            if (WARM) {
                if (n == nb - 1) face<PH>(x);
            } else {
                bool bad = false;
                step<false, PH>(x, L, n, acc, bad, o);
                if (__builtin_expect(__builtin_amdgcn_ballot_w64(acc < kUdivMinExp) != 0, 0))
                    step<true, PH>(x, L, n, acc, bad, o);
                x.fyx = o.fyx;
                x.fyy = o.fyy;
                x.vht = o.vht;
                if (ZF) x.a2t = o.a2t;
            }
            x.qb = qb;
            x.qc = qc;
        }
        if constexpr (RO == 1) {
            if (!WARM) pair_put<PH>(x, o, n);
            if constexpr (X2) {
                if (!WARM && trs[0]) {
                    const unsigned nbytes = (unsigned)b.pitch * (unsigned)(b.bnd_y2 - b.bnd_y1 + 1) * 8u;
                    const unsigned ci = geo(&b)(L.m, min(max(n, b.bnd_y1), b.bnd_y2)).c;
                    const bool on = L0.out && n >= b.ny_start - 2 && n <= b.ny_end + 2;
                    st_on(trs[0], nbytes, ci, o.lu ? o.sshn : x.ssh.s<PH>(1), on);
                    st_on(trs[1], nbytes, ci, o.lu ? o.fx : x.shp.s<PH>(1), on);
                    st_on(trs[2], nbytes, ci, o.cu ? o.un : x.u.s<PH>(1), on);
                    st_on(trs[3], nbytes, ci, o.cv ? o.vn : x.v.s<PH>(1), on);
                }
            }
            pair_barrier();
            ++x.rn;
            fb = fbn;
            return n >= ne;
        }
        store_out(o, geo(&b)(L.m, n).c);
        if constexpr (RO == 2) pair_barrier();
        ++x.rn;
        fb = fbn;
        return n >= ne;
    }
};
#undef OCN_MD

#define CHECK(...)                                                \
    do {                                                          \
        int _rc = check_block(b);                                 \
        if (_rc) return _rc;                                      \
        _rc = nonnull({__VA_ARGS__});                             \
        if (_rc) return _rc;                                      \
    } while (0)

static int check_block(const ocn_block *b)
{
    if (!b) return set_error(OCN_ERR_ARG, "null ocn_block");
    if (b->nx_start > b->nx_end || b->ny_start > b->ny_end)
        return set_error(OCN_ERR_ARG, "empty interior");
    if (b->bnd_x1 > b->nx_start - 1 || b->bnd_x2 < b->nx_end + 1 || b->bnd_y1 > b->ny_start - 1 ||
        b->bnd_y2 < b->ny_end + 1)
        return set_error(OCN_ERR_ARG, "array bounds must include a 1-wide halo ring");
    if (b->pitch < (int64_t)(b->bnd_x2 - b->bnd_x1 + 1))
        return set_error(OCN_ERR_ARG, "pitch smaller than bnd_x2-bnd_x1+1");
    if (b->pitch * (int64_t)(b->bnd_y2 - b->bnd_y1 + 1) >= (int64_t(1) << 29))
        return set_error(OCN_ERR_ARG, "block array of 2^29 elements or more (32-bit byte offsets of r8 fields)");
    return OCN_OK;
}

static int nonnull(std::initializer_list<const void *> ps)
{
    for (const void *p : ps)
        if (!p) return set_error(OCN_ERR_ARG, "null array pointer");
    return OCN_OK;
}

#define RC_K(x) do { int _rc = (x); if (_rc) return _rc; } while (0)
// ... 137 lines not shown
    g.ntiles = g.r[0].tiles;
    return issue_march(g, body, s);
}

#ifndef OCN_FRAME_STEP_ROWS
#define OCN_FRAME_STEP_ROWS 4
#endif
template <class Body>
static int launch_step_frame(const ocn_block *b, const Range &all, const Range &inner, const Body &body, hipStream_t s)
{
    const Range in = range_clip(all, inner);
    if (range_empty(in)) return launch_step(b, all, body, s);
    const Rects q = frame_rects(all, in);
    MarchGrid g{};
    for (int i = 0; i < 4; ++i) {
        if (q.w[i] <= 0 || q.h[i] <= 0) continue;
        const Range r{q.m0[i], q.m0[i] + q.w[i] - 1, q.n0[i], q.n0[i] + q.h[i] - 1};
        g.r[g.nr] = march_rect<Body>(b, r, OCN_FRAME_STEP_ROWS, i >= 2);
        g.ntiles += g.r[g.nr].tiles;
        ++g.nr;
    }
    return issue_march(g, body, s);
}

struct FallbackCheck {
    ocn_block b; const uint8_t *bits; const double *hu, *hu1, *hv, *hv1, *hh, *vort, *stt, *sts, *rx, *ry; int *flag;
    Range r;
    const double *hr, *mu;
    double *kc;
    unsigned own;
    OCN_HD void operator()(int m, int n) const
    {
        const Pt c = geo(&b)(m, n), c0 = geo(&b)(r.m0, r.n0);
        if (m == r.m0 && n == r.n0) { kc[0] = ld(hr, c0); kc[1] = ld(mu, c0); }
        if (fbits64(ld(hr, c)) != fbits64(ld(hr, c0))) OCN_ATOMIC_OR(flag, 1);
        if (m < r.m0 - 1 || m > r.m1 + 1 || n < r.n0 - 1 || n > r.n1 + 1) return;
        if (fbits64(ld(mu, c)) != fbits64(ld(mu, c0))) OCN_ATOMIC_OR(flag, 2);
        const unsigned bc = ld(bits, c);
        const bool owned = (own >> (own_class(m, b.nx_start, b.nx_end) * 3u + own_class(n, b.ny_start, b.ny_end))) & 1u;
        const bool hh_rng = owned || (m >= b.nx_start - 1 && m <= b.nx_end && n >= b.ny_start - 1 && n <= b.ny_end);
        const bool in = owned || (m >= b.nx_start && m <= b.nx_end && n >= b.ny_start && n <= b.ny_end);
        auto nz = [&](const double *p) { return fbits64(ld(p, c)) != 0; };
        bool bad = false;
        if (!(hh_rng && (bc & (1u << OCN_LLU)))) bad |= nz(hu) || nz(hu1);
        if (!(hh_rng && (bc & (1u << OCN_LLV)))) bad |= nz(hv) || nz(hv1);
        if (!(hh_rng && (bc & (1u << OCN_LUH)))) bad |= nz(hh);
        if (!(in && (bc & (1u << OCN_LUU)))) bad |= nz(vort) || nz(sts);
        if (!(in && (bc & (1u << OCN_LU)))) bad |= nz(stt);
        if (m >= r.m0 && m <= r.m1 && n >= r.n0 && n <= r.n1) bad |= nz(rx) || nz(ry);
        if (bad) OCN_ATOMIC_OR(flag, 2);
    }
};

int launch_fallback_check(const ocn_block *b, void *const *ptr, const uint8_t *bits, const Range &r, int32_t *flag,
                          double *kc, hipStream_t s, unsigned own)
{
    RC_K(check_block(b));
    auto f = [&](int id) { return (const double *)ptr[ocn_field_slot(id)]; };
    const FallbackCheck k{*b, bits, f(OCN_HHU), f(OCN_HHU_P), f(OCN_HHV), f(OCN_HHV_P), f(OCN_HHH), f(OCN_VORT),
                          f(OCN_STR_T), f(OCN_STR_S), f(OCN_RHSX), f(OCN_RHSY), (int *)flag, r, f(OCN_HHQ_REST),
                          f(OCN_MU), kc, own};
    const int m0 = max(r.m0 - 2, b->bnd_x1), m1 = min(r.m1 + 2, b->bnd_x2);
    const int n0 = max(r.n0 - 2, b->bnd_y1), n1 = min(r.n1 + 2, b->bnd_y2);
    if (m0 > m1 || n0 > n1) return OCN_OK;
    return launch_range(m0, m1, n0, n1, k, s);
}

// ... 361 lines not shown
    long cost = -1;
    for (int rows = 8; rows <= OCN_PAIR_MAX_ROWS; ++rows) {
        const long tiles = (h + rows - 1) / rows, waves = 4 * tiles * wx * mult,
                   rounds = (waves + kPairSlots - 1) / kPairSlots, c = rounds * (rows + 8);
        if (cost < 0 || c < cost) { cost = c; best = rows; }
    }
    return best;
}

int launch_onepass_pair(const ocn_block *b, void *const *ptr, int nptr, const Compact *cp, const ocn_sw_params &sw,
                        double tau, int32_t *nbad1, int32_t *nbad2, double *sshp_out, double *up_out, double *vp_out,
                        hipStream_t s, const OnepassKC &kc, bool last)
{
    if (!cp || !cp->march || sw.full_free_surface != 1 || sw.trans_terms <= 0 || sw.ksw_lat <= 0 || !sshp_out ||
        !up_out || !vp_out)
        return set_error(OCN_ERR_ARG, "two-step launch: compact tables, march, full_free_surface = 1, trans_terms and "
                                      "ksw_lat on, three second buffers");
    if (kc.mode == OCN_KC_DEVICE || (kc.mode != OCN_KC_GENERAL && !kc.kc))
        return set_error(OCN_ERR_ARG, "two-step launch: a variant chosen on the host");
    RC_K(check_block(b));
    const Tab<true> t = make_tab<true>(ptr, nptr, cp->bits, cp->rows, block_rows(b), 0);
    const Range r = range_interior(b);
    if (range_empty(r)) return OCN_OK;
    using KP = MarchStep<true, false, true, false, false, true>;
    const int cols = KP::kPairCols, rows = pair_rows(r, cols);
    MarchGrid g{};
    const int ntx = (r.m1 - r.m0 + cols) / cols;
    g.r[0] = MarchRect{r.m0, r.m1, r.n0, r.n1, r.m0, ntx, ntx * ((r.n1 - r.n0 + rows) / rows), max(r.m0 - 4, b->bnd_x1),
                       min(r.m1 + 4, b->bnd_x2), rows, 0};
    g.nr = 1;
    g.ntiles = g.r[0].tiles;
    int ex;
    const bool p2 = std::frexp(tau, &ex) == 0.5 && ex > -1020 && ex < 1020;
#define OCN_PAIR_LAUNCH(P, L, Z, H)                                                                              \
    return issue_march(g, MarchStep<P, L, Z, false, H, true>{*b, t, sw, tau, nbad1, sshp_out, up_out, vp_out,        \
                                                             kc.kc, nullptr, 0, 0u, nbad2}, s)
#define OCN_PAIR_VARIANT(L)                                                                                      \
    if (kc.mode == OCN_KC_GENERAL) { if (p2) OCN_PAIR_LAUNCH(true, L, false, false); OCN_PAIR_LAUNCH(false, L, false, false); } \
    if (kc.mode == OCN_KC_KNOWN_HR) { if (p2) OCN_PAIR_LAUNCH(true, L, true, true); OCN_PAIR_LAUNCH(false, L, true, true); }    \
    if (p2) OCN_PAIR_LAUNCH(true, L, true, false);                                                                \
    OCN_PAIR_LAUNCH(false, L, true, false)
    if (last) { OCN_PAIR_VARIANT(true); }
    OCN_PAIR_VARIANT(false);
#undef OCN_PAIR_VARIANT
#undef OCN_PAIR_LAUNCH
}

int launch_onepass_pair_x4(const ocn_block *bx, void *const *ptr, int nptr, const Compact *cp, const ocn_sw_params &sw,
                           double tau, int32_t *nbad1, int32_t *nbad2, double *sshp_out, double *up_out, double *vp_out,
                           hipStream_t s, const OnepassKC &kc, unsigned own, const Range *range, int nblk,
                           const Range *frame_of, double *const *trs)
{
    if (!cp || !cp->march || sw.full_free_surface != 1 || sw.trans_terms <= 0 || sw.ksw_lat <= 0 || !sshp_out ||
        !up_out || !vp_out)
        return set_error(OCN_ERR_ARG, "x4 two-step launch: compact tables, march, full_free_surface = 1, trans_terms "
                                      "and ksw_lat on, three second buffers");
    if ((kc.mode != OCN_KC_KNOWN && kc.mode != OCN_KC_KNOWN_HR) || !kc.kc)
        return set_error(OCN_ERR_ARG, "x4 two-step launch: a known-constant variant chosen on the host");
    RC_K(check_block(bx));
    if (bx->bnd_x1 > bx->nx_start - 4 || bx->bnd_x2 < bx->nx_end + 4 || bx->bnd_y1 > bx->ny_start - 4 ||
        bx->bnd_y2 < bx->ny_end + 4)
        return set_error(OCN_ERR_ARG, "x4 two-step launch: the geometry must reach 4 points past the interior");
    const Tab<true> t = make_tab<true>(ptr, nptr, cp->bits, cp->rows, block_rows(bx), 0);
    const Range all = range ? *range : range_interior(bx);
    if (range_empty(all)) return OCN_OK;
    using KP = MarchStep<true, false, true, true, false, true>;
    constexpr int P = kPack<KP> < kBatchMax / 4 ? kPack<KP> : kBatchMax / 4;
    const int cols = KP::kPairCols, mult = batching(s) ? std::max(1, std::min(nblk, P)) : 1;
    Range rs[4];
    int nr = 0;
    if (!frame_of) {
        rs[nr++] = all;
    } else {
        const Range &in = *frame_of;
        const Range cand[4] = {{all.m0, all.m1, all.n0, in.n0 - 1}, {all.m0, all.m1, in.n1 + 1, all.n1},
                               {all.m0, in.m0 - 1, in.n0, in.n1}, {in.m1 + 1, all.m1, in.n0, in.n1}};
        for (const Range &q : cand)
            if (!range_empty(q)) rs[nr++] = q;
    }
    MarchGrid g{};
    for (int i = 0; i < nr; ++i) {
        const Range &r = rs[i];
        const int rows = pair_rows(r, cols, mult), ntx = (r.m1 - r.m0 + cols) / cols;
        g.r[g.nr++] = MarchRect{r.m0, r.m1, r.n0, r.n1, r.m0, ntx, ntx * ((r.n1 - r.n0 + rows) / rows),
                                max(r.m0 - 4, bx->bnd_x1), min(r.m1 + 4, bx->bnd_x2), rows, 0};
        g.ntiles += g.r[g.nr - 1].tiles;
    }
    int ex;
    auto go = [&](auto body) {
        if (trs)
            for (int i = 0; i < 4; ++i) body.trs[i] = trs[i];
        return issue_march(g, body, s);
    };
    const bool p2 = std::frexp(tau, &ex) == 0.5 && ex > -1020 && ex < 1020;
    if (kc.mode == OCN_KC_KNOWN_HR) {
        if (p2)
            return go(MarchStep<true, false, true, true, true, true>{*bx, t, sw, tau, nbad1, sshp_out, up_out, vp_out,
                                                                     kc.kc, nullptr, 0, own, nbad2});
        return go(MarchStep<false, false, true, true, true, true>{*bx, t, sw, tau, nbad1, sshp_out, up_out, vp_out, kc.kc,
                                                                  nullptr, 0, own, nbad2});
    }
    if (p2)
        return go(MarchStep<true, false, true, true, false, true>{*bx, t, sw, tau, nbad1, sshp_out, up_out, vp_out, kc.kc,
                                                                  nullptr, 0, own, nbad2});
    return go(MarchStep<false, false, true, true, false, true>{*bx, t, sw, tau, nbad1, sshp_out, up_out, vp_out, kc.kc,
                                                               nullptr, 0, own, nbad2});
}

__global__ void k_bits_x4(ocn_block bx, ocn_block g, const uint8_t *bits, uint8_t *out, const int32_t *mask, int nx, int ny,
                          unsigned own)
{
    const int w = bx.bnd_x2 - bx.bnd_x1 + 1, h = bx.bnd_y2 - bx.bnd_y1 + 1;
    const long i = (long)blockIdx.x * blockDim.x + threadIdx.x;
    if (i >= (long)w * h) return;
    const int m = bx.bnd_x1 + (int)(i % w), n = bx.bnd_y1 + (int)(i / w);
    const unsigned cls = own_class(m, g.nx_start, g.nx_end) * 3u + own_class(n, g.ny_start, g.ny_end);
    unsigned v = 0;
    if (cls != 4u && ((own >> cls) & 1u) && m >= 1 && m < nx && n >= 1 && n < ny) {
        auto lu = [&](int mm, int nn) -> unsigned { return mask[(long)(mm - 1) + (long)(nn - 1) * nx] == 0 ? 1u : 0u; };
        const unsigned a = lu(m, n), b = lu(m + 1, n), c = lu(m, n + 1), d = lu(m + 1, n + 1);
        v = (a << OCN_LU) | ((a & b & c & d) << OCN_LUU) | ((a | b | c | d) << OCN_LUH) | ((a & b) << OCN_LCU) |
            ((a & c) << OCN_LCV) | ((a | b) << OCN_LLU) | ((a | c) << OCN_LLV);
    } else if (m >= g.bnd_x1 && m <= g.bnd_x2 && n >= g.bnd_y1 && n <= g.bnd_y2) {
        v = bits[(long)(m - g.bnd_x1) + (long)(n - g.bnd_y1) * g.pitch];
    }
    out[(long)(m - bx.bnd_x1) + (long)(n - bx.bnd_y1) * bx.pitch] = (uint8_t)v;
}

__global__ void k_rows_x4(float *rows4, unsigned nrows4, const float *rows, unsigned nrows, const float *ext, int *flags)
{
    const unsigned r = blockIdx.x * blockDim.x + threadIdx.x;
    if (r >= nrows4) return;
    float v[kNumRowFields];
    const int e = r == 0 ? 3 : r == 1 ? 2 : r == 2 ? 0 : r == nrows4 - 3 ? 1 : r == nrows4 - 2 ? 4 : r == nrows4 - 1 ? 5 : -1;
    for (int k = 0; k < kNumRowFields; ++k)
        v[k] = e >= 0 ? ext[e * kNumRowFields + k] : rows[(unsigned)k * nrows + (r - kXRing)];
    if (!write_table_row(rows4, nrows4, r, v)) atomicOr(flags, (int)OCN_COMPACT_DIVISOR_RANGE);
}

int launch_x4_tables(const ocn_block *g, const uint8_t *bits, const float *rows, const float *ext, uint8_t *bits4,
                     float *rows4, const int32_t *mask, int nx, int ny, unsigned own, int32_t *flags, hipStream_t s)
{
    RC_K(check_block(g));
    ocn_block bx = *g;
    bx.bnd_x1 -= kXRing; bx.bnd_x2 += kXRing; bx.bnd_y1 -= kXRing; bx.bnd_y2 += kXRing;
    const long pts = (long)(bx.bnd_x2 - bx.bnd_x1 + 1) * (bx.bnd_y2 - bx.bnd_y1 + 1);
    hipLaunchKernelGGL(k_bits_x4, dim3((unsigned)((pts + 255) / 256)), dim3(256), 0, s, bx, *g, bits, bits4, mask, nx, ny,
                       own);
    RC_K(check_launch());
    const unsigned nrows = block_rows(g), nrows4 = block_rows(&bx);
    hipLaunchKernelGGL(k_rows_x4, dim3((nrows4 + 63) / 64), dim3(64), 0, s, rows4, nrows4, rows, nrows, ext, (int *)flags);
    return check_launch();
}

int launch_tracer(const ocn_block *b, void *const *ptr, int nptr, const Compact *cp, int stage, int k, double tau,
                  double ts, hipStream_t s)
{
    const Range ri = range_interior(b), rr = range_ring(b);
    switch (stage) {
    case OCN_TSTAGE_TRAN_DIFF_FLUXES:
        return launch_fused<KTranDiffFluxes>(ri, ri, OCN_PART_ALL, b, ptr, nptr, cp, k, s, 1.0);
    case OCN_TSTAGE_TRAN_DIFF_TRACER:
        return launch_fused<KTranDiffTracer>(ri, ri, OCN_PART_ALL, b, ptr, nptr, cp, k, s, tau);
    case OCN_TSTAGE_TRACER_NEXT_STEP:
        return launch_fused<KTracerNextStep>(rr, rr, OCN_PART_ALL, b, ptr, nptr, cp, k, s, ts);
    default: return set_error(OCN_ERR_ARG, "bad tracer stage id");
    }
}

constexpr int kTrRows = 4;
// ... 463 lines not shown
```

### ocean_model_arch_amd/csrc/sw_stencils.h

```cpp
#pragma once

#include <stdint.h>

#include "../../include/ocn_sw.h"

#ifndef OCN_HD
#define OCN_HD __host__ __device__
#endif
#ifndef OCN_INLINE
#define OCN_INLINE __forceinline__
#endif
#ifndef OCN_ATOMIC_INC
#define OCN_ATOMIC_INC(p) atomicAdd((p), 1)
#endif
#ifndef OCN_ATOMIC_OR
#define OCN_ATOMIC_OR(p, v) atomicOr((p), (v))
#endif
#ifndef OCN_FREE_FALL_ACC
#define OCN_FREE_FALL_ACC 9.8f
#endif

namespace ocn {

struct Pt {
// ... 675 lines not shown
        if (bv) {
            if (do_adv && full) st(a4.RHSy, c, rya);
            if (do_dif && full) st(a6.RHSy, c, ryd);
            st(a7.vbrtrn, c, vn);
        }
    }
};

template <bool C> struct FusedC1 {
    int sx, ex, sy, ey;
    bool do_hh;
    int *nbad;
    SwNextStep<C> a8; HhShift<C> a9;
    OCN_HD void operator()(int m, int n) const
    {
        const Pt c = a8.I(m, n);
        const double x = a8.step(c);
        if (do_hh && (m == ex + 1 || n == ey + 1)) a9(m, n);
        if (nbad && m >= sx && m <= ex && n >= sy && n <= ey && ld(a8.lu, c) > 0.5f && !(x < 10000.0 && x > -10000.0))
            OCN_ATOMIC_INC(nbad);
    }
};

constexpr int kNumMasks = OCN_DX;
constexpr int kNumRowFields = OCN_NUM_R4 - OCN_DX;
constexpr int kNumRowRatios = 4;
constexpr int kRowTable = kNumRowFields + kNumRowRatios;
enum { OCN_RC_DXT = 0, OCN_RC_DYH, OCN_RC_DXH, OCN_RC_DYT, OCN_RC_DXB, OCN_RC_DYB, OCN_RC_AREA, kNumRecips };
OCN_HD inline unsigned recip_offset(unsigned nrows) { return ((unsigned)kRowTable * nrows + 1u) & ~1u; }
inline size_t row_table_floats(unsigned nrows) { return recip_offset(nrows) + 2u * (unsigned)kNumRecips * nrows; }
enum { OCN_COMPACT_MASK_NOT_BINARY = 1, OCN_COMPACT_METRIC_NOT_ROW_CONSTANT = 2,
       OCN_COMPACT_RING_SEA = 4,
       OCN_COMPACT_DIVISOR_RANGE = 8,
       OCN_COMPACT_EDGE_RING_SEA = 16 };

OCN_HD inline unsigned own_class(int v, int lo, int hi) { return v < lo ? 0u : v > hi ? 2u : 1u; }

OCN_HD inline bool write_table_row(float *rows, unsigned nrows, unsigned r, const float *v)
{
    for (int k = 0; k < kNumRowFields; ++k) rows[(unsigned)k * nrows + r] = v[k];
    const float dx = v[0], dy = v[OCN_DY - OCN_DX], dxb = v[OCN_DXB - OCN_DX], dyb = v[OCN_DYB - OCN_DX];
    const float rat[kNumRowRatios] = {dy / dx, dx / dy, dxb / dyb, dyb / dxb};
    for (int k = 0; k < kNumRowRatios; ++k) rows[(unsigned)(kNumRowFields + k) * nrows + r] = rat[k];
    const float area = dx * dy;
    const float g[kNumRecips] = {v[OCN_DXT - OCN_DX], v[OCN_DYH - OCN_DX], v[OCN_DXH - OCN_DX], v[OCN_DYT - OCN_DX],
                                 dxb, dyb, area};
    double *rc = (double *)(rows + recip_offset(nrows));
    bool range = true;
    for (int k = 0; k < kNumRecips; ++k) {
        rc[(unsigned)k * nrows + r] = 1.0 / (double)g[k];
        range &= g[k] >= 0x1p-60f && g[k] <= 0x1p60f;
    }
    return range;
}

struct Prepare {
    Geo I; int ms, me, ns, ne;
    const float *__restrict__ r4[OCN_NUM_R4];
    uint8_t *__restrict__ bits; float *__restrict__ rows; unsigned nrows; int *flags;
    unsigned own;
    int bx2, by2;
    OCN_HD void operator()(int m, int n) const
    {
        const Pt q = I(m, n);
        unsigned b = 0;
        bool bad = false;
        for (int id = 0; id < kNumMasks; ++id) {
            const uint32_t v = fbits(ld(r4[id], q));
            if (v == 0x3f800000u) b |= 1u << id;
            else if (v != 0u) bad = true;
        }
        st(bits, q, (uint8_t)b);
        if (bad) OCN_ATOMIC_OR(flags, (int)OCN_COMPACT_MASK_NOT_BINARY);
        {
            auto sea = [&](int dm, int dn) {
                const int mm = m + dm, nn = n + dn;
                return mm <= bx2 && nn <= by2 && fbits(ld(r4[OCN_LU], I(mm, nn))) == 0x3f800000u;
            };
            const bool s00 = (b >> OCN_LU) & 1u, s10 = sea(1, 0), s01 = sea(0, 1), s11 = sea(1, 1);
            if ((((b >> OCN_LLU) & 1u) && !(s00 || s10)) || (((b >> OCN_LLV) & 1u) && !(s00 || s01)) ||
                (((b >> OCN_LUH) & 1u) && !(s00 || s10 || s01 || s11)))
                OCN_ATOMIC_OR(flags, (int)OCN_COMPACT_DIVISOR_RANGE);
        }
        if (m < ms || m > me || n < ns || n > ne) return;
        const unsigned a8m = (1u << OCN_LU) | (1u << OCN_LCU) | (1u << OCN_LCV);
        const unsigned a9m = (1u << OCN_LU) | (1u << OCN_LLU) | (1u << OCN_LLV) | (1u << OCN_LUH);
        const bool a8w = (m == ms || m == me || n == ns || n == ne) && (b & a8m);
        if (a8w || ((m == me || n == ne) && (b & a9m))) OCN_ATOMIC_OR(flags, (int)OCN_COMPACT_RING_SEA);
        const unsigned cls = own_class(m, ms + 1, me - 1) * 3u + own_class(n, ns + 1, ne - 1);
        if (a8w && !((own >> cls) & 1u)) OCN_ATOMIC_OR(flags, (int)OCN_COMPACT_EDGE_RING_SEA);
        const Pt q0 = I(ms, n);
        bool vary = false;
        float v[kNumRowFields];
        for (int k = 0; k < kNumRowFields; ++k) {
            v[k] = ld(r4[OCN_DX + k], q);
            vary |= fbits(v[k]) != fbits(ld(r4[OCN_DX + k], q0));
        }
        if (m == ms && !write_table_row(rows, nrows, q.r, v)) OCN_ATOMIC_OR(flags, (int)OCN_COMPACT_DIVISOR_RANGE);
        if (vary) OCN_ATOMIC_OR(flags, (int)OCN_COMPACT_METRIC_NOT_ROW_CONSTANT);
    }
};

struct Coherence {
    Geo I; int ms, me, ns, ne;
    const uint8_t *__restrict__ bits;
    const double *a[3], *b[3];
    int *flags;
    OCN_HD void operator()(int m, int n) const
    {
        const Pt q = I(m, n);
        const bool inside = m >= ms && m <= me && n >= ns && n <= ne;
        const unsigned mb = ld(bits, q);
        const unsigned mask_bit[3] = {1u << OCN_LU, 1u << OCN_LCU, 1u << OCN_LCV};
        bool bad = false;
        for (int k = 0; k < 3; ++k) {
            if (inside && (mb & mask_bit[k])) continue;
            uint64_t x, y;
            const double va = ld(a[k], q), vb = ld(b[k], q);
            __builtin_memcpy(&x, &va, 8);
            __builtin_memcpy(&y, &vb, 8);
            bad |= x != y;
        }
        if (bad) OCN_ATOMIC_OR(flags, 1);
    }
};

inline int ocn_field_slot(int id) { return id < OCN_NUM_R4 ? id : OCN_NUM_R4 + (id - OCN_SSH); }
OCN_HD inline Geo geo(const ocn_block *b) { return Geo{b->bnd_x1, b->bnd_y1, (unsigned)b->pitch}; }
OCN_HD inline unsigned block_rows(const ocn_block *b) { return (unsigned)(b->bnd_y2 - b->bnd_y1 + 1); }

#ifndef OCN_RANGE_DEFINED
// ... 273 lines not shown
```

### ocean_model_arch_amd/model.py

```python
from __future__ import annotations

import ctypes as C
from dataclasses import dataclass

import numpy as np

from . import _lib
from ._lib import FIELD_ID, R4_NAMES, R8_NAMES, STAGE_ID, TSTAGE_ID, check, is_r8_name, lib, tracer_names
from .config import BasinConfig, ParallelConfig, SWConfig


@dataclass
class BlockInfo:
    k: int
    bm: int
    bn: int
    nx_start: int
    nx_end: int
    ny_start: int
    ny_end: int
    bnd_x1: int
    bnd_x2: int
    bnd_y1: int
    bnd_y2: int
# ... 172 lines not shown
    def set_lazy_tail(self, on: bool = True):
        check(lib().ocn_ctx_set_option(self.ctx, _lib.OPT_LAZY_TAIL, int(on)), "ocn_ctx_set_option")
        return self

    def set_x2(self, on: bool = True):
        check(lib().ocn_ctx_set_option(self.ctx, _lib.OPT_X2, int(on)), "ocn_ctx_set_option")
        return self

    def set_batch(self, on: bool = True):
        check(lib().ocn_ctx_set_option(self.ctx, _lib.OPT_BATCH, int(on)), "ocn_ctx_set_option")
        return self

    def set_multi(self, on: bool = True):
        check(lib().ocn_ctx_set_option(self.ctx, _lib.OPT_MULTI, int(on)), "ocn_ctx_set_option")
        return self

    def set_x4(self, on=True):
        mode = 3 if on == 3 else int(bool(on))
        check(lib().ocn_ctx_set_option(self.ctx, _lib.OPT_X4, mode), "ocn_ctx_set_option")
        return self

    @property
    def x4_active(self) -> bool:
        return self.option(_lib.OPT_X4) == 2

    def set_co_launch(self, on: bool = True):
        check(lib().ocn_ctx_set_option(self.ctx, _lib.OPT_CO_LAUNCH, int(on)), "ocn_ctx_set_option")
        return self

    @property
    def co_launched(self) -> bool:
        return self.option(_lib.OPT_CO_LAUNCH) == 2

    def set_multi_spin(self, polls: int):
        check(lib().ocn_ctx_set_option(self.ctx, _lib.OPT_MULTI_SPIN, int(polls)), "ocn_ctx_set_option")
        return self

    def set_tracer_step(self, on: bool = True):
        check(lib().ocn_ctx_set_option(self.ctx, _lib.OPT_TRACER_STEP, int(on)), "ocn_ctx_set_option")
        return self

    @property
    def tracer_step_active(self) -> bool:
        return self.option(_lib.OPT_TRACER_STEP) == 2

    def set_pair(self, mode: int = 1):
        check(lib().ocn_ctx_set_option(self.ctx, _lib.OPT_PAIR, int(mode)), "ocn_ctx_set_option")
        return self

    @property
    def multi_active(self) -> bool:
        return self.option(_lib.OPT_MULTI) == 2

    @property
    def pair_active(self) -> bool:
        return self.option(_lib.OPT_PAIR) == 2

    @property
    def x2_active(self) -> bool:
        return bool(self.option(_lib.OPT_X2))

    @property
    def tail_pending(self) -> bool:
        return self.option(_lib.OPT_LAZY_TAIL) == 2

    def complete(self):
# ... 116 lines not shown
```

Before: 60.61 billion.

## Add inviscid specialization of fused march kernel when viscosity and dissipation are zero

Adds an NV template variant of the fused march step. It is chosen when a device-side check shows the lateral viscosity mu is zero everywhere, r_diss is zero in every row, and the metric ratios are finite. The variant skips the viscous stress and diffusion terms, keeps a smaller row-constant LDS table, and adds a cheaper exponent check that falls back to the exact path when needed. The eligibility signal travels through a second fallback flag word, a table flag and a multi-GPU vote. This adds more kernel instantiations and extra control logic, and results could diverge if a check is missed.

```diff
diff --git a/include/ocn_sw.h b/include/ocn_sw.h
--- a/include/ocn_sw.h
+++ b/include/ocn_sw.h
@@ -224,7 +224,8 @@
        OCN_OPT_MARCH = 6, OCN_OPT_FLIP = 7, OCN_OPT_RECOMPUTE = 8, OCN_OPT_ONEPASS = 9,
        OCN_OPT_KNOWN_CONSTANTS = 10, OCN_OPT_ONEPASS_LAST = 11, OCN_OPT_LAZY_TAIL = 12, OCN_OPT_X2 = 13,
        OCN_OPT_BATCH = 14, OCN_OPT_PAIR = 15, OCN_OPT_MULTI = 16, OCN_OPT_TRACER_STEP = 17,
-       OCN_OPT_MULTI_SPIN = 18, OCN_OPT_X4 = 19, OCN_OPT_CO_LAUNCH = 20, OCN_OPT_XCHG_DELAY = 21 };
+       OCN_OPT_MULTI_SPIN = 18, OCN_OPT_X4 = 19, OCN_OPT_CO_LAUNCH = 20, OCN_OPT_XCHG_DELAY = 21,
+       OCN_OPT_INVISCID = 22 };
 
 enum { OCN_TIMER_FUSED_A = OCN_NUM_STAGES, OCN_TIMER_FUSED_B, OCN_TIMER_FUSED_C1, OCN_TIMER_TRACER,
        OCN_TIMER_FUSED_CA = OCN_TIMER_TRACER + OCN_NUM_TSTAGES, OCN_TIMER_ONEPASS, OCN_TIMER_ONEPASS2,
diff --git a/ocean_model_arch_amd/_codeobj.py b/ocean_model_arch_amd/_codeobj.py
--- a/ocean_model_arch_amd/_codeobj.py
+++ b/ocean_model_arch_amd/_codeobj.py
@@ -66,9 +66,10 @@
 
 def march_step_symbol(args: str, batched: bool = False) -> str:
     bits = "".join("Lb1E" if a.strip() == "true" else "Lb0E" for a in args.split(","))
+    body = "10MarchStepT" if len(args.split(",")) == 8 else "9MarchStep"
     if batched:
-        return f"_ZN3ocn9k_march_bINS_9MarchStepII{bits}EEEEvNS_10MarchGridBENS_4PackIT_EE".replace("II", "I")
-    return f"_ZN3ocn7k_marchINS_9MarchStepII{bits}EEEEvNS_9MarchGridET_".replace("II", "I")
+        return f"_ZN3ocn9k_march_bINS_{body}I{bits}EEEEvNS_10MarchGridBENS_4PackIT_EE"
+    return f"_ZN3ocn7k_marchINS_{body}I{bits}EEEEvNS_9MarchGridET_"
 
 
 def kernel_code_sha(lib_path: str, symbol: str) -> str | None:
diff --git a/ocean_model_arch_amd/_lib.py b/ocean_model_arch_amd/_lib.py
--- a/ocean_model_arch_amd/_lib.py
+++ b/ocean_model_arch_amd/_lib.py
@@ -80,6 +80,7 @@
 OPT_X4 = 19
 OPT_CO_LAUNCH = 20
 OPT_XCHG_DELAY = 21
+OPT_INVISCID = 22
 
 KERNEL_SYMBOLS = ["ocn_sw_update_ssh", "ocn_hh_update", "ocn_uv_trans_vort", "ocn_uv_trans",
                   "ocn_stress_components", "ocn_uv_diff2", "ocn_sw_update_uv", "ocn_sw_next_step",
diff --git a/ocean_model_arch_amd/csrc/ctx_setup.hip b/ocean_model_arch_amd/csrc/ctx_setup.hip
--- a/ocean_model_arch_amd/csrc/ctx_setup.hip
+++ b/ocean_model_arch_amd/csrc/ctx_setup.hip
@@ -241,7 +241,7 @@
     HIPCHK(hipMalloc(&c->d_bar, kMultiBarBytes));
     c->allocs.push_back(c->d_bar);
     HIPCHK(hipMemsetAsync(c->d_nbad, 0, 256 + kcb, c->stream));
-    c->d_fbz = c->d_nbad + 16;
+    c->d_fbz = c->d_nbad + kFbzWord;
     c->d_flags = c->d_nbad + 32;
     for (size_t i = 0; i < c->blocks.size(); ++i) c->blocks[i].kc = (double *)((char *)c->d_nbad + 256) + 2 * i;
     return OCN_OK;
@@ -273,8 +273,9 @@
     c->edge_ring_sea = (flags[0] & kCompactEdgeRingSea) != 0;
     c->udiv_ok = (flags[0] & kCompactDivisorRange) == 0;
     c->rows_x_ok = c->ext_ok && flags[1] == 0;
-    c->x4_tab_ok = x4_tabs && flags[2] == 0;
-    c->compact = (flags[0] & ~(kCompactRingSea | kCompactDivisorRange | kCompactEdgeRingSea)) == 0;
+    c->x4_tab_ok = x4_tabs && (flags[2] & ~kCompactViscousRow) == 0;
+    c->rdiss_zero = ((flags[0] | flags[2]) & kCompactViscousRow) == 0;
+    c->compact = (flags[0] & ~(kCompactRingSea | kCompactDivisorRange | kCompactEdgeRingSea | kCompactViscousRow)) == 0;
     c->static_dirty = false;
     return OCN_OK;
 }
diff --git a/ocean_model_arch_amd/csrc/ocn_ctx.h b/ocean_model_arch_amd/csrc/ocn_ctx.h
--- a/ocean_model_arch_amd/csrc/ocn_ctx.h
+++ b/ocean_model_arch_amd/csrc/ocn_ctx.h
@@ -162,7 +162,7 @@
     std::map<std::vector<int>, HaloPlan> plans;
     bool initialized = false;
     bool use_graph = false;
-    struct Graph { hipGraphExec_t exec; double tau; ocn::StepKind kind; bool compact, march, ring_sea; int role, kc_mode; };
+    struct Graph { hipGraphExec_t exec; double tau; ocn::StepKind kind; bool compact, march, ring_sea; int role, kc_mode; bool kc_nv; };
     std::vector<Graph> graphs;
     std::vector<void *> allocs;
     bool stage_timing = false;
@@ -198,6 +198,8 @@
     mutable bool hqn_stale = false;
     mutable int fb_state = 0;
     int kc_mode = 0;
+    bool inviscid = true, rdiss_zero = false, nv_dev_ok = false, kc_nv = false, nv_used = false;
+    mutable bool fb_inviscid = false;
     int32_t *d_fbz = nullptr;
     bool lazy = true, open = false, open_x2 = false;
     double open_tau = 0.0;
@@ -253,13 +255,14 @@
 inline bool is_alt_field(int id) { return id == OCN_SSHP || id == OCN_UBRTRP || id == OCN_VBRTRP; }
 inline size_t field_bytes(const LBlock &b) { return (size_t)b.g.pitch * (b.g.bnd_y2 - b.g.bnd_y1 + 1) * 8; }
 inline bool has_comm(const ocn_ctx *c) { return c->comm || c->lb || c->comm_aborted; }
-inline OnepassKC kc_of(const ocn_ctx *c, const LBlock &b) { return OnepassKC{c->kc_mode, c->d_fbz, b.kc}; }
+inline OnepassKC kc_of(const ocn_ctx *c, const LBlock &b) { return OnepassKC{c->kc_mode, c->d_fbz, b.kc, c->kc_nv}; }
 
 int make_seglist(ocn_ctx *c, const std::vector<Seg> &v, SegList &out);
 int launch_segs(const SegList &l, hipStream_t s, int32_t *cmp = nullptr);
 int get_plan(ocn_ctx *c, const std::vector<int> &fields, HaloPlan *&out, int depth = 1, int priv = 0);
 int run_sync(ocn_ctx *c, const std::vector<int> &fields, hipStream_t stream = nullptr, int32_t *cmp = nullptr,
              int depth = 1, int priv = 0);
+constexpr int kFbzWord = 16, kFbzWords = 2;
 constexpr int kVoteWords = 8;
 int allreduce_max(ocn_ctx *c, int32_t *word, hipStream_t s, int words = 1);
 int nccl_rc(ncclResult_t r, const char *what);
diff --git a/ocean_model_arch_amd/csrc/ocn_ctx.hip b/ocean_model_arch_amd/csrc/ocn_ctx.hip
--- a/ocean_model_arch_amd/csrc/ocn_ctx.hip
+++ b/ocean_model_arch_amd/csrc/ocn_ctx.hip
@@ -359,7 +359,7 @@
 enum { kVoteIncoherent = 0, kVoteIneligible, kVoteUdiv, kVoteHhStale, kVoteX2, kVoteX4, kVoteOvSeq, kVoteOvOv,
        kVoteUsed };
 static_assert(kVoteUsed <= kVoteWords, "vote words");
-struct VoteIn { bool eligible, udiv_ok, hh_consistent, x2_ok, x4_ok; };
+struct VoteIn { bool eligible, udiv_ok, hh_consistent, x2_ok, x4_ok, nv_ok; };
 struct VoteOut { bool udiv_ok, hh_consistent, x2_ok, x4_ok; };
 
 struct HaloZero {
@@ -415,7 +415,7 @@
     host[kVoteUdiv] = !in.udiv_ok;
     host[kVoteHhStale] = !in.hh_consistent;
     host[kVoteX2] = !in.x2_ok;
-    host[kVoteX4] = !in.x4_ok;
+    host[kVoteX4] = !in.x4_ok ? 2 : !in.nv_ok ? 1 : 0;
     host[kVoteOvSeq] = host[kVoteOvOv] = INT32_MAX;
     if (c->ov_state == 2) {
         float ms[2] = {0.f, 0.f};
@@ -452,7 +452,7 @@
     out.hh_consistent = w[kVoteHhStale] == 0;
     out.x2_ok = w[kVoteX2] == 0 && exch && c->x2;
     c->x2_dev_ok = out.x2_ok;
-    out.x4_ok = out.x2_ok && w[kVoteX4] == 0;
+    out.x4_ok = out.x2_ok && w[kVoteX4] < 2;
     if (w[kVoteOvSeq] != INT32_MAX && w[kVoteOvOv] != INT32_MAX) {
         c->ov_ms[0] = 1.0e-3 * w[kVoteOvSeq];
         c->ov_ms[1] = 1.0e-3 * w[kVoteOvOv];
@@ -462,6 +462,7 @@
         c->ov_state = 0;
     }
     c->x4_dev_ok = out.x4_ok;
+    c->nv_dev_ok = w[kVoteX4] == 0;
     return OCN_OK;
 }
 
@@ -1229,7 +1230,7 @@
     if (!rc) rc = check_hip(hipEventCreateWithFlags(&c->ev_fork, hipEventDisableTiming), "hipEventCreate");
     if (!rc) rc = check_hip(hipEventCreateWithFlags(&c->ev_join, hipEventDisableTiming), "hipEventCreate");
     if (!rc) rc = check_hip(hipEventCreateWithFlags(&c->ev_fb, hipEventDisableTiming), "hipEventCreate");
-    if (!rc) rc = check_hip(hipHostMalloc((void **)&c->h_fbz, sizeof(int32_t), hipHostMallocDefault), "hipHostMalloc");
+    if (!rc) rc = check_hip(hipHostMalloc((void **)&c->h_fbz, kFbzWords * sizeof(int32_t), hipHostMallocDefault), "hipHostMalloc");
     if (!rc) rc = decompose(c);
     if (!rc) rc = allocate(c);
     if (!rc) rc = prebuild_plans(c);
@@ -1526,7 +1527,7 @@
     c->hn_fresh = false;
     for (const auto &g : c->graphs)
         if (g.tau == tau && g.kind == k && g.compact == c->compact && g.march == c->march && g.ring_sea == c->ring_sea &&
-            g.role == c->role && g.kc_mode == c->kc_mode) {
+            g.role == c->role && g.kc_mode == c->kc_mode && g.kc_nv == c->kc_nv) {
             HIPCHK(hipGraphLaunch(g.exec, c->stream));
             if (k.rc) swap_sshp(c);
             if (k.one || k.one_last) swap_alt3(c);
@@ -1547,7 +1548,7 @@
     e = hipGraphInstantiate(&exec, graph, nullptr, nullptr, 0);
     (void)hipGraphDestroy(graph);
     HIPCHK(e);
-    c->graphs.push_back(ocn_ctx::Graph{exec, tau, k, c->compact, c->march, c->ring_sea, role, c->kc_mode});
+    c->graphs.push_back(ocn_ctx::Graph{exec, tau, k, c->compact, c->march, c->ring_sea, role, c->kc_mode, c->kc_nv});
     HIPCHK(hipGraphLaunch(exec, c->stream));
     return OCN_OK;
 }
@@ -1575,9 +1576,11 @@
 static void learn_fb(ocn_ctx *c)
 {
     if (c->fb_state != kFbDevice) return;
-    int32_t f = 0;
-    if (hipMemcpy(&f, c->d_fbz, sizeof(f), hipMemcpyDeviceToHost) != hipSuccess) return;
+    int32_t fv[kFbzWords] = {0, 0};
+    if (hipMemcpy(fv, c->d_fbz, sizeof(fv), hipMemcpyDeviceToHost) != hipSuccess) return;
+    const int32_t f = fv[0];
     c->fb_state = f == 0 ? kFbZero : f == 1 ? kFbHr : kFbGeneral;
+    c->fb_inviscid = fv[1] == 0;
     c->fb_copy = false;
 }
 
@@ -1586,6 +1589,7 @@
     if (c->fb_state != kFbDevice || !c->fb_copy || hipEventQuery(c->ev_fb) != hipSuccess) return;
     const int32_t f = *(volatile int32_t *)c->h_fbz;
     c->fb_state = f == 0 ? kFbZero : f == 1 ? kFbHr : kFbGeneral;
+    c->fb_inviscid = ((volatile int32_t *)c->h_fbz)[1] == 0;
     c->fb_copy = false;
 }
 
@@ -1594,13 +1598,23 @@
     return c->fb_state == kFbZero ? OCN_KC_KNOWN : c->fb_state == kFbHr ? OCN_KC_KNOWN_HR
          : c->fb_state == kFbGeneral ? OCN_KC_GENERAL : OCN_KC_DEVICE;
 }
+static bool nv_local(const ocn_ctx *c)
+{
+    return c->inviscid && c->known_const && !c->r8_handed && c->rdiss_zero && c->fb_inviscid &&
+           (c->fb_state == kFbZero || c->fb_state == kFbHr);
+}
+static void set_kc_mode(ocn_ctx *c, int mode)
+{
+    c->kc_mode = mode;
+    c->kc_nv = (mode == OCN_KC_KNOWN || mode == OCN_KC_KNOWN_HR) && nv_local(c) && (!has_comm(c) || c->nv_dev_ok);
+}
 static int prepare_kc(ocn_ctx *c, bool x2 = false)
 {
-    if (!c->known_const || c->r8_handed) { c->kc_mode = OCN_KC_GENERAL; return OCN_OK; }
+    if (!c->known_const || c->r8_handed) { set_kc_mode(c, OCN_KC_GENERAL); return OCN_OK; }
     learn_fb_async(c);
     if (c->fb_state != kFbUnchecked && x2 && !c->fb_x2) c->fb_state = kFbUnchecked;
     if (c->fb_state == kFbUnchecked) {
-        HIPCHK(hipMemsetAsync(c->d_fbz, 0, sizeof(int32_t), c->stream));
+        HIPCHK(hipMemsetAsync(c->d_fbz, 0, kFbzWords * sizeof(int32_t), c->stream));
         for (const LBlock &b : c->blocks) {
             std::vector<void *> tab = b.ptr;
             if (x2) tab[field_slot(OCN_HHQ_REST)] = b.hr_x;
@@ -1608,14 +1622,14 @@
             RC(launch_fallback_check(&b.g, tab.data(), b.bits, r, c->d_fbz, b.kc, c->stream, x2 ? b.own : 0u));
         }
         if (!c->capturing) {
-            HIPCHK(hipMemcpyAsync(c->h_fbz, c->d_fbz, sizeof(int32_t), hipMemcpyDeviceToHost, c->stream));
+            HIPCHK(hipMemcpyAsync(c->h_fbz, c->d_fbz, kFbzWords * sizeof(int32_t), hipMemcpyDeviceToHost, c->stream));
             HIPCHK(hipEventRecord(c->ev_fb, c->stream));
             c->fb_copy = true;
         }
         c->fb_state = kFbDevice;
         c->fb_x2 = x2;
     }
-    c->kc_mode = kc_of_fb(c);
+    set_kc_mode(c, kc_of_fb(c));
     return OCN_OK;
 }
 
@@ -1681,7 +1695,7 @@
     if (!pairs) return OCN_OK;
     HIPCHK(hipEventSynchronize(c->ev_fb));
     learn_fb_async(c);
-    c->kc_mode = kc_of_fb(c);
+    set_kc_mode(c, kc_of_fb(c));
     return OCN_OK;
 }
 
@@ -1759,7 +1773,7 @@
     if (nsteps < 0) return set_error(OCN_ERR_ARG, "nsteps < 0");
     if (nsteps == 0) return OCN_OK;
     const bool graph_ok = c->use_graph && !has_comm(c) && !c->stage_timing && !(c->sw.use_tracers > 0 && c->tr_step);
-    c->pair_used = false;
+    c->pair_used = c->nv_used = false;
     c->co_used = false;
     c->multi_used = false;
     if (c->open) {
@@ -1777,6 +1791,7 @@
                     const StepKind k = continuing_pair(chk[i], chk[i + 1], c->open_x2);
                     rc = graph_ok ? graph_step(c, tau, k) : run_step(c, tau, k);
                     c->open_pair = c->pair_used = true;
+                    if (!k.one_last) c->nv_used = c->kc_nv;
                 }
                 if (rc == OCN_OK) {
                     c->deferred = (int)(chk.size() - i);
@@ -1814,7 +1829,7 @@
     int N = lazy_cand ? nsteps + 1 : nsteps;
     if (N >= 2 && (eligible || (has_comm(c) && c->flip)) && !c->coherent_known) {
         VoteOut v;
-        RC(check_coherence(c, VoteIn{eligible, c->udiv_ok, c->hh_consistent, x2_here, x4_here}, v));
+        RC(check_coherence(c, VoteIn{eligible, c->udiv_ok, c->hh_consistent, x2_here, x4_here, nv_local(c)}, v));
         udiv_ok = v.udiv_ok;
         first_one = v.hh_consistent;
         x2_ok = x2_here && v.x2_ok;
@@ -1899,6 +1914,7 @@
             k.next_a = k.next_reuse = false;
             ++s;
             c->pair_used = true;
+            if (!k.one_last) c->nv_used = c->kc_nv;
         }
         rc = graph_ok ? graph_step(c, tau, k) : run_step(c, tau, k);
     }
@@ -2120,6 +2136,7 @@
         c->hrx_ok = false;
         return OCN_OK;
     case OCN_OPT_CO_LAUNCH: c->co_launch = value != 0; return OCN_OK;
+    case OCN_OPT_INVISCID: c->inviscid = value != 0; return OCN_OK;
     case OCN_OPT_BATCH:
         if (c->batch != (value != 0)) drop_graphs(c);
         c->batch = value != 0;
@@ -2163,6 +2180,7 @@
     case OCN_OPT_X4: *value = c->x4_used ? 2 : c->x4 ? 1 : 0; return OCN_OK;
     case OCN_OPT_CO_LAUNCH: *value = c->co_used ? 2 : c->co_launch; return OCN_OK;
     case OCN_OPT_XCHG_DELAY: *value = c->xdelay_us; return OCN_OK;
+    case OCN_OPT_INVISCID: *value = c->nv_used ? 2 : c->inviscid; return OCN_OK;
     default: return set_error(OCN_ERR_ARG, "unknown option");
     }
 }
diff --git a/ocean_model_arch_amd/csrc/ocn_internal.h b/ocean_model_arch_amd/csrc/ocn_internal.h
--- a/ocean_model_arch_amd/csrc/ocn_internal.h
+++ b/ocean_model_arch_amd/csrc/ocn_internal.h
@@ -92,7 +92,7 @@
 int launch_gaussian(const ocn_block &g, double *p, const float *lu, int nx0, int ny0, double sigma, hipStream_t s);
 int launch_fill_field(const ocn_block &g, double *p, double v, hipStream_t s);
 enum { OCN_KC_GENERAL = 0, OCN_KC_KNOWN = 1, OCN_KC_DEVICE = 2, OCN_KC_KNOWN_HR = 3 };
-struct OnepassKC { int mode; const int32_t *flag; const double *kc; };
+struct OnepassKC { int mode; const int32_t *flag; const double *kc; bool nv = false; };
 int launch_onepass(const ocn_block *b, void *const *ptr, int nptr, const Compact *cp, const ocn_sw_params &sw,
                    double tau, int32_t *nbad, double *sshp_out, double *up_out, double *vp_out, hipStream_t s,
                    const Range *range, bool last, const OnepassKC &kc, unsigned own = 0,
@@ -157,6 +157,7 @@
                             hipStream_t s);
 constexpr int kCompactRingSea = 4;
 constexpr int kCompactDivisorRange = 8;
+constexpr int kCompactViscousRow = 32;
 
 struct BatchEntry {
     virtual ~BatchEntry() {}
diff --git a/ocean_model_arch_amd/csrc/sw_kernels.hip b/ocean_model_arch_amd/csrc/sw_kernels.hip
--- a/ocean_model_arch_amd/csrc/sw_kernels.hip
+++ b/ocean_model_arch_amd/csrc/sw_kernels.hip
@@ -1510,6 +1510,9 @@
 
 __shared__ double g_step_rc[kStepLdsRows * kRowC];
 __shared__ unsigned g_step_rlo;
+constexpr int kRowCNV = 17;
+constexpr int nv_col(int k) { return k <= RC_RDYB ? k : k == RC_RLH ? 14 : k == RC_AREA ? 15 : k == RC_RAREA ? 16 : -1; }
+__shared__ double g_step_rc_nv[kStepLdsRows * kRowCNV];
 __shared__ double g_pair[4][6][120];
 
 __device__ __forceinline__ double row_const(const float *rows, unsigned nrows, unsigned r, int k)
@@ -1589,12 +1592,14 @@
     int32_t *nbp;
     bool cnt;
     int pj;
+    bool big;
     double fyx, fyy, vht, a2t;
     double hr0, mu0;
     const __attribute__((address_space(3))) double *lds;
     unsigned rlo;
-    template <bool LDS> __device__ __forceinline__ double cst(int k, int dy) const
-    {
+    template <int LDS> __device__ __forceinline__ double cst(int k, int dy) const
+    {
+        if (LDS == 2) return lds[(rn + dy - rlo) * kRowCNV + nv_col(k)];
         if (LDS) return lds[(rn + dy - rlo) * kRowC + k];
         switch (k) {
         case RC_RDXT: return rc(OCN_RC_DXT, dy);
@@ -1670,10 +1675,10 @@
 
 #define OCN_MD(id, dy) D(x.met((id), (dy)))
 
-template <bool P2, bool LAST = false, bool ZF = false, bool X2 = false, bool HR = false, bool PAIR = false,
-          bool WT = false>
-struct MarchStep {
+template <bool P2, bool LAST, bool ZF, bool X2, bool HR, bool PAIR, bool WT, bool NV>
+struct MarchStepT {
     static_assert(!PAIR || !X2 || (ZF && !LAST), "two-step launches with exchanges: the known-constant variants");
+    static_assert(!NV || (ZF && !LAST), "the inviscid body: a known-constant variant, not a last step");
     static constexpr int kStAux = WT ? 16 : 0;
     static constexpr bool kPair = PAIR;
     static constexpr bool kX2 = X2;
@@ -1736,6 +1741,15 @@
         x.bits.s<PH>(3) = q.bits;
         x.v.s<PH>(2) = q.v; x.vp.s<PH>(2) = q.vp; x.mu.s<PH>(2) = q.mu;
         x.rhsx = q.rhsx; x.rhsy = q.rhsy;
+        if constexpr (NV) guard(x, q.u, q.up, q.ssh, q.shp, q.v, q.vp, q.hr);
+    }
+    __device__ __forceinline__ static void guard(StepRegs &x, double a, double b, double c, double d, double e, double f,
+                                                 double hr)
+    {
+        double s = __builtin_fabs(a) + __builtin_fabs(b) + __builtin_fabs(c) + __builtin_fabs(d) + __builtin_fabs(e) +
+                   __builtin_fabs(f);
+        if (HR) s += __builtin_fabs(hr);
+        x.big = x.big || !(s < 0x1p300);
     }
 
     template <int PH> __device__ __forceinline__ static void weights(StepRegs &x, int dy)
@@ -1823,12 +1837,22 @@
         if (!E) exp_check(acc, sh);
         if (!E) {
             exp_check(acc, a_u0); exp_check(acc, a_v0); exp_check(acc, a_h0); exp_check(acc, a_u1);
-            exp_check(acc, a_v1); exp_check(acc, x.up.s<PH>(2)); exp_check(acc, x.vp.s<PH>(2)); exp_check(acc, x.up.s<PH>(3));
+            exp_check(acc, a_v1);
+            if (!NV) { exp_check(acc, x.up.s<PH>(2)); exp_check(acc, x.vp.s<PH>(2)); exp_check(acc, x.up.s<PH>(3)); }
         }
         double q1[9], q2[5];
-        dvn<E, 9>({a_u0, a_v0, a_h0, a_u1, a_v1, x.up.s<PH>(2), x.vp.s<PH>(2), x.up.s<PH>(3), x.vp.s<PH>(2)},
-                  {dxt, dxh, dxb, dxt, dxh, dyh, dxh, x.cst<kLds>(RC_DXT, 2), dyt},
-                  {rxt, rxh, x.cst<kLds>(RC_RDXB, 1), rxt, rxh, ryh, rxh, x.cst<kLds>(RC_RDXT, 2), ryt}, q1);
+        if constexpr (NV) {
+            double q5[5];
+            dvn<E, 5>({a_u0, a_v0, a_h0, a_u1, a_v1}, {dxt, dxh, dxb, dxt, dxh},
+                      {rxt, rxh, x.cst<kLds>(RC_RDXB, 1), rxt, rxh}, q5);
+#pragma unroll
+            for (int i = 0; i < 5; ++i) q1[i] = q5[i];
+            q1[5] = q1[6] = q1[7] = q1[8] = 0.0;
+        } else {
+            dvn<E, 9>({a_u0, a_v0, a_h0, a_u1, a_v1, x.up.s<PH>(2), x.vp.s<PH>(2), x.up.s<PH>(3), x.vp.s<PH>(2)},
+                      {dxt, dxh, dxb, dxt, dxh, dyh, dxh, x.cst<kLds>(RC_DXT, 2), dyt},
+                      {rxt, rxh, x.cst<kLds>(RC_RDXB, 1), rxt, rxh, ryh, rxh, x.cst<kLds>(RC_RDXT, 2), ryt}, q1);
+        }
         dvn<E, 5>({q1[0], q1[1], q1[2], q1[3], q1[4]}, {dyh, dyt, dyb, dyh, dyt},
                   {ryh, ryt, x.cst<kLds>(RC_RDYB, 1), ryh, ryt}, q2);
         const double u0 = q2[0], v0 = q2[1], h0 = q2[2], u1 = q2[3], v1 = q2[4];
@@ -1837,8 +1861,11 @@
         const double vort = (v_r * dyt - v_0 * dyt) - (u_1 * x.cst<kLds>(RC_DXT, 2) - u_0 * dxt)
                             - ((v_r - v_0) * dyb - (u_1 - u_0) * dxb);
         const double qa = q1[5], qb = q1[6], qc1 = q1[7], qe = q1[8];
-        const double st = x.cst<kLds>(RC_RAT0, 1) * (qa - shz(qa, -1)) - x.cst<kLds>(RC_RAT1, 1) * (qb - x.qb);
-        const double ss = x.cst<kLds>(RC_RAT2, 1) * (qc1 - x.qc) + x.cst<kLds>(RC_RAT3, 1) * (shz(qe, 1) - qe);
+        double st = 0.0, ss = 0.0;
+        if constexpr (!NV) {
+            st = x.cst<kLds>(RC_RAT0, 1) * (qa - shz(qa, -1)) - x.cst<kLds>(RC_RAT1, 1) * (qb - x.qb);
+            ss = x.cst<kLds>(RC_RAT2, 1) * (qc1 - x.qc) + x.cst<kLds>(RC_RAT3, 1) * (shz(qe, 1) - qe);
+        }
         qb_next = qb;
         qc_next = qc1;
         const double hu = fb.llu ? u0 : fb.hu;
@@ -1846,10 +1873,13 @@
         const double hh = fb.luh ? h0 : fb.hh;
         const double vt = fb.vt ? vort : fb.vort;
         const double stt = fb.st ? st : fb.stt;
-        x.hu.s<PH>(2) = hu; x.hv.s<PH>(2) = hv; x.hh.s<PH>(2) = hh; x.vort.s<PH>(2) = vt; x.stt.s<PH>(2) = stt;
+        x.hu.s<PH>(2) = hu; x.hv.s<PH>(2) = hv; x.hh.s<PH>(2) = hh; x.vort.s<PH>(2) = vt;
         x.hu1.s<PH>(2) = fb.llu ? u1 : fb.hu1;
         x.hv1.s<PH>(2) = fb.llv ? v1 : fb.hv1;
-        x.sts.s<PH>(2) = fb.ss ? ss : fb.sts;
+        if constexpr (!NV) {
+            x.stt.s<PH>(2) = stt;
+            x.sts.s<PH>(2) = fb.ss ? ss : fb.sts;
+        }
         x.pu.s<PH>(2) = u_0 * dyh * hu;
         x.pv.s<PH>(2) = v_0 * dxh * hv;
         x.vh.s<PH>(2) = vt * hh;
@@ -1858,7 +1888,9 @@
         x.rr.s<PH>(2) = rr;
         x.cx.s<PH>(2) = rr * (v_r + v_0);
         const double hq = x.hr.s<PH>(2) + x.ssh.s<PH>(2);
-        if constexpr (kLds) {
+        if constexpr (NV) {
+            (void)hq; (void)stt;
+        } else if constexpr (kLds) {
             x.dt.s<PH>(2) = x.cst<kLds>(RC_DY2, 1) * hq * stt;
             x.dxq.s<PH>(2) = x.cst<kLds>(RC_DX2, 1) * hq * stt;
         } else {
@@ -1875,11 +1907,50 @@
         x.fyx = (pv + shz(pv, 1)) / 2.0 * (u_n + u) / 2.0 * luu;
         x.vht = x.vh.s<PH>(1) * (v_r + v);
         x.fyy = (pv + pvn) / 2.0 * (v + v_n) / 2.0;
-        if constexpr (ZF) {
+        if constexpr (ZF && !NV) {
             const double mu = x.mu.s<PH>(1), mu_n = x.mu.s<PH>(2), muh_p = (mu + mu + mu_n + mu_n) / 4.0;
             (void)muh_p;
             x.a2t = x.cst<kLds>(RC_DXB2, 0) * x.hh.s<PH>(1) * x.sts.s<PH>(1);
         }
+    }
+
+    template <bool E, int PH>
+    __device__ __forceinline__ void viscous(const StepRegs &x, int m, int n, double a_ssh, int &acc, double &q_ssh,
+                                            double &rxd, double &ryd) const
+    {
+        auto C = [&](int k, int dy) { return x.cst<0>(k, dy); };
+        auto Q = [&](double a, int k, int rk, int dy) { return dv<E>(a, C(k, dy), C(rk, dy)); };
+        const double mu0 = x.mu0, muh = (mu0 + mu0 + mu0 + mu0) / 4.0;
+        auto str_t = [&](int dy) {
+            const int k = dy + 1;
+            const double qa = Q(x.up.s<PH>(k), RC_DYH, RC_RDYH, dy), qb = Q(x.vp.s<PH>(k), RC_DXH, RC_RDXH, dy),
+                         qbm = Q(x.vp.s<PH>(k - 1), RC_DXH, RC_RDXH, dy - 1);
+            const double st = C(RC_RAT0, dy) * (qa - shz(qa, -1)) - C(RC_RAT1, dy) * (qb - qbm);
+            Fallback f;
+            fallback<PH, 0>(x, f, m, n + dy, k);
+            return f.st ? st : 0.0;
+        };
+        auto str_s = [&](int dy) {
+            const int k = dy + 1;
+            const double qc1 = Q(x.up.s<PH>(k + 1), RC_DXT, RC_RDXT, dy + 1), qc = Q(x.up.s<PH>(k), RC_DXT, RC_RDXT, dy),
+                         qe = Q(x.vp.s<PH>(k), RC_DYT, RC_RDYT, dy);
+            const double ss = C(RC_RAT2, dy) * (qc1 - qc) + C(RC_RAT3, dy) * (shz(qe, 1) - qe);
+            Fallback f;
+            fallback<PH, 0>(x, f, m, n + dy, k);
+            return f.ss ? ss : 0.0;
+        };
+        const double stt0 = str_t(0), stt1 = str_t(1), sts0 = str_s(0), stsm = str_s(-1);
+        const double hq0 = x.hr.s<PH>(1) + x.ssh.s<PH>(1), hq1 = x.hr.s<PH>(2) + x.ssh.s<PH>(2);
+        const double dtc = C(RC_DY2, 0) * mu0 * hq0 * stt0;
+        const double dxq0 = C(RC_DX2, 0) * mu0 * hq0 * stt0, dxq1 = C(RC_DX2, 1) * mu0 * hq1 * stt1;
+        const double hh = x.hh.s<PH>(1);
+        const double a2p = C(RC_DXB2, 0) * muh * hh * sts0, a2t = C(RC_DXB2, -1) * muh * x.hh.s<PH>(0) * stsm;
+        const double a4p = C(RC_DYB2, 0) * muh * hh * sts0;
+        const double a1 = shz(dtc, 1) - dtc, a2 = a2p - a2t, a3 = dxq1 - dxq0, a4 = a4p - shz(a4p, -1);
+        if (!E) { exp_check(acc, a1); exp_check(acc, a2); exp_check(acc, a3); exp_check(acc, a4); }
+        q_ssh = Q(a_ssh, RC_AREA, RC_RAREA, 0);
+        rxd = Q(a1, RC_DYH, RC_RDYH, 0) + Q(a2, RC_DXT, RC_RDXT, 0);
+        ryd = -Q(a3, RC_DXH, RC_RDXH, 0) + Q(a4, RC_DYT, RC_RDYT, 0);
     }
 
     struct Out {
@@ -1888,10 +1959,11 @@
         double vort = 0.0, sts = 0.0, stt = 0.0, rxa = 0.0, rxd = 0.0, rya = 0.0, ryd = 0.0;
         double fyx = 0.0, fyy = 0.0, vht = 0.0, a2t = 0.0;
     };
-    template <bool E, int PH>
+    template <bool E, int PH, bool FULL = true, bool RE = E>
     __device__ __forceinline__ void step(const StepRegs &x, const Lane &L, int n, int &acc, bool &bad, Out &o) const
     {
         (void)n;
+        constexpr bool kShort = NV && !FULL;
         const double u = x.u.s<PH>(1), v = x.v.s<PH>(1), hu = x.hu.s<PH>(1), hv = x.hv.s<PH>(1), hh = x.hh.s<PH>(1);
         const double dxt = x.cst<kLds>(RC_DXT, 0), dyt = x.cst<kLds>(RC_DYT, 0), dxh = x.cst<kLds>(RC_DXH, 0),
                      dyh = x.cst<kLds>(RC_DYH, 0);
@@ -1921,9 +1993,15 @@
             rya = -(fx_p - fx_m + fy_p - x.fyy) - (q + shz(q, -1)) / 4.0;
             o.fyy = fy_p;
         }
-        double rxd, ryd;
+        double rxd = 0.0, ryd = 0.0;
         double q_ssh = 0.0;
-        {
+        if constexpr (kShort) {
+            double qd[1];
+            dvn<E, 1>({a_ssh}, {x.cst<kLds>(RC_AREA, 0)}, {x.cst<kLds>(RC_RAREA, 0)}, qd);
+            q_ssh = qd[0];
+        } else if constexpr (NV) {
+            viscous<E, PH>(x, L.m, n, a_ssh, acc, q_ssh, rxd, ryd);
+        } else {
             auto sh = [](double a, int d) { return ZF ? a : shz(a, d); };
             const double mu = x.mu.s<PH>(1), mu_r = sh(mu, 1), mu_l = sh(mu, -1), mu_n = x.mu.s<PH>(2), mu_s = x.mu.s<PH>(0);
             const double muh_p = (mu + mu_r + mu_n + sh(mu_n, 1)) / 4.0;
@@ -1965,19 +2043,29 @@
                 const double bp = qtau(x, hu * dxt * dyh / 2.0);
                 const double bp0 = qtau(x, x.hu1.s<PH>(1) * dxt * dyh / 2.0);
                 const double slx = -(g * (shz(ssh, 1) - ssh) * dyh * hu);
-                const double fric = (kLds ? x.cst<kLds>(RC_RDSELF, 0) : x.cst<kLds>(RC_RDSELF, 0) / 2.0) * x.up.s<PH>(1) * dxt *
-                                    dyh * hu;
-                const double grx = x.rhsx + slx + rxd + rxa - fric + (x.cx.s<PH>(1) + x.cx.s<PH>(0)) / 4.0;
+                double grx;
+                if constexpr (kShort) {
+                    grx = x.rhsx + slx + rxa + (x.cx.s<PH>(1) + x.cx.s<PH>(0)) / 4.0;
+                } else {
+                    const double fric = (kLds == 1 ? x.cst<kFull>(RC_RDSELF, 0) : x.cst<kFull>(RC_RDSELF, 0) / 2.0) *
+                                        x.up.s<PH>(1) * dxt * dyh * hu;
+                    grx = x.rhsx + slx + rxd + rxa - fric + (x.cx.s<PH>(1) + x.cx.s<PH>(0)) / 4.0;
+                }
                 un = (x.up.s<PH>(1) * bp0 + grx) / (bp);
             }
             {
                 const double bp = qtau(x, hv * dyt * dxh / 2.0);
                 const double bp0 = qtau(x, x.hv1.s<PH>(1) * dyt * dxh / 2.0);
                 const double sly = -(g * (x.ssh.s<PH>(2) - ssh) * dxh * hv);
-                const double fric = (kLds ? x.cst<kLds>(RC_RDNEXT, 0) : x.cst<kLds>(RC_RDNEXT, 0) / 2.0) * x.vp.s<PH>(1) * dxh *
-                                    dyt * hv;
                 const double c1 = x.rr.s<PH>(1) * (u_n + u);
-                const double gry = x.rhsy + sly + ryd + rya - fric - (c1 + shz(c1, -1)) / 4.0;
+                double gry;
+                if constexpr (kShort) {
+                    gry = x.rhsy + sly + rya - (c1 + shz(c1, -1)) / 4.0;
+                } else {
+                    const double fric = (kLds == 1 ? x.cst<kFull>(RC_RDNEXT, 0) : x.cst<kFull>(RC_RDNEXT, 0) / 2.0) *
+                                        x.vp.s<PH>(1) * dxh * dyt * hv;
+                    gry = x.rhsy + sly + ryd + rya - fric - (c1 + shz(c1, -1)) / 4.0;
+                }
                 vn = (x.vp.s<PH>(1) * bp0 + gry) / (bp);
             }
         }
@@ -1995,7 +2083,7 @@
             o.rxa = rxa; o.rxd = rxd; o.rya = rya; o.ryd = ryd;
         }
         const bool bd = o.lu && !(sshn < 10000.0 && sshn > -10000.0);
-        if (__builtin_expect(x.nbp && x.cnt && bd != (E && bad), 0)) atomicAdd(x.nbp, bd ? 1 : -1);
+        if (__builtin_expect(x.nbp && x.cnt && bd != (RE && bad), 0)) atomicAdd(x.nbp, bd ? 1 : -1);
         bad = bd;
     }
 
@@ -2038,9 +2126,10 @@
             r[5][x.pj] = o.cv ? o.fb : x.vp.s<PH>(1);
         }
     }
-    static constexpr bool kLds = ZF;
+    static constexpr int kLds = NV ? 2 : ZF ? 1 : 0;
+    static constexpr int kFull = NV ? 0 : kLds;
     static constexpr bool kUnroll = ZF;
-    static constexpr bool kPrologue = kLds;
+    static constexpr bool kPrologue = kLds != 0;
     __device__ void prologue(const MarchRect &R, int ty) const
     {
         const int h = R.vert ? 4 * R.rows : R.rows, nb = R.n0 + ty * h;
@@ -2051,11 +2140,16 @@
             const double mu0 = kc[1], muh = (mu0 + mu0 + mu0 + mu0) / 4.0;
 #pragma unroll
             for (int k = 0; k < kRowC; ++k) {
-                double v = row_const(t.rows, t.nrows, r, k);
-                if (k == RC_DY2 || k == RC_DX2) v = v * mu0;
-                else if (k == RC_DXB2 || k == RC_DYB2) v = v * muh;
-                else if (k == RC_RDSELF || k == RC_RDNEXT) v = v / 2.0;
-                g_step_rc[i * kRowC + k] = v;
+                if constexpr (NV) {
+                    (void)muh;
+                    if (nv_col(k) >= 0) g_step_rc_nv[i * kRowCNV + nv_col(k)] = row_const(t.rows, t.nrows, r, k);
+                } else {
+                    double v = row_const(t.rows, t.nrows, r, k);
+                    if (k == RC_DY2 || k == RC_DX2) v = v * mu0;
+                    else if (k == RC_DXB2 || k == RC_DYB2) v = v * muh;
+                    else if (k == RC_RDSELF || k == RC_RDNEXT) v = v / 2.0;
+                    g_step_rc[i * kRowC + k] = v;
+                }
             }
         }
         if (threadIdx.x == 0) g_step_rlo = (unsigned)lo;
@@ -2085,7 +2179,8 @@
         x.nbp = RO == 2 ? nbad2 : nbad;
         x.cnt = true;
         x.pj = L.j;
-        if (kLds) x.lds = (const __attribute__((address_space(3))) double *)g_step_rc;
+        if constexpr (NV) x.lds = (const __attribute__((address_space(3))) double *)g_step_rc_nv;
+        else if constexpr (kLds != 0) x.lds = (const __attribute__((address_space(3))) double *)g_step_rc;
         x.rows = (const __attribute__((address_space(4))) float *)t.rows;
         x.rcp = (const __attribute__((address_space(4))) double *)(t.rows + recip_offset(t.nrows));
         x.nrows = t.nrows;
@@ -2108,6 +2203,10 @@
             }
             x.hr.s<0>(2) = ZF && !HR ? x.hr0 : ld(t.f(OCN_HHQ_REST), c1);
             x.bits.s<0>(2) = ld(t.bits, c1);
+            if constexpr (NV) {
+                x.big = !HR && !(__builtin_fabs(x.hr0) < 0x1p300);
+                guard(x, x.up.s<0>(2), x.ssh.s<0>(2), x.shp.s<0>(2), x.u.s<0>(2), x.vp.s<0>(1), 0.0, x.hr.s<0>(2));
+            }
         }
         Fallback fb;
         fallback<0, RO>(x, fb, L.m, n0 + 1, 2);
@@ -2115,8 +2214,10 @@
         load<RO>(x, q, L.m, n0);
         if constexpr (PAIR && RO == 1 && kPrologue) pair_barrier();
         if (kLds) x.rlo = g_step_rlo;
-        x.qb = x.vp.s<0>(1) / x.cst<kLds>(RC_DXH, 0);
-        x.qc = x.up.s<0>(2) / x.cst<kLds>(RC_DXT, 1);
+        if constexpr (!NV) {
+            x.qb = x.vp.s<0>(1) / x.cst<kLds>(RC_DXH, 0);
+            x.qc = x.up.s<0>(2) / x.cst<kLds>(RC_DXT, 1);
+        }
         weights<0>(x, 1);
         if (RO != 1) store_out(Out{}, 0u);
         if constexpr (RO == 2) pair_barrier();
@@ -2168,20 +2269,36 @@
             int acc = 0;
             double qb, qc;
             derive<false, PH>(x, fb, acc, qb, qc);
-            if (__builtin_expect(__builtin_amdgcn_ballot_w64(acc < kUdivMinExp) != 0, 0))
+            bool again = __builtin_amdgcn_ballot_w64(acc < kUdivMinExp) != 0;
+            if constexpr (NV) {
+                if (__builtin_expect(!again && __builtin_amdgcn_ballot_w64(x.big) != 0, 0)) {
+                    int a5 = 0;
+                    exp_check(a5, x.up.s<PH>(2)); exp_check(a5, x.vp.s<PH>(2)); exp_check(a5, x.up.s<PH>(3));
+                    again = __builtin_amdgcn_ballot_w64(a5 < kUdivMinExp) != 0;
+                }
+            }
+            if (__builtin_expect(again, 0))
                 derive<true, PH>(x, fb, acc, qb, qc);
             acc = 0;
             if (WARM) {
                 if (n == nb - 1) face<PH>(x);
             } else {
                 bool bad = false;
-                step<false, PH>(x, L, n, acc, bad, o);
-                if (__builtin_expect(__builtin_amdgcn_ballot_w64(acc < kUdivMinExp) != 0, 0))
-                    step<true, PH>(x, L, n, acc, bad, o);
+                step<false, PH, false>(x, L, n, acc, bad, o);
+                bool exact = __builtin_amdgcn_ballot_w64(acc < kUdivMinExp) != 0;
+                if constexpr (NV) {
+                    if (__builtin_expect(!exact && __builtin_amdgcn_ballot_w64(x.big) != 0, 0)) {
+                        acc = 0;
+                        step<false, PH, true, true>(x, L, n, acc, bad, o);
+                        exact = __builtin_amdgcn_ballot_w64(acc < kUdivMinExp) != 0;
+                    }
+                }
+                if (__builtin_expect(exact, 0))
+                    step<true, PH, true>(x, L, n, acc, bad, o);
                 x.fyx = o.fyx;
                 x.fyy = o.fyy;
                 x.vht = o.vht;
-                if (ZF) x.a2t = o.a2t;
+                if (ZF && !NV) x.a2t = o.a2t;
             }
             x.qb = qb;
             x.qc = qc;
@@ -2211,6 +2328,9 @@
         return n >= ne;
     }
 };
+template <bool P2, bool LAST = false, bool ZF = false, bool X2 = false, bool HR = false, bool PAIR = false,
+          bool WT = false>
+struct MarchStep : MarchStepT<P2, LAST, ZF, X2, HR, PAIR, WT, false> {};
 #undef OCN_MD
 
 #define CHECK(...)                                                \
@@ -2414,7 +2534,10 @@
     OCN_HD void operator()(int m, int n) const
     {
         const Pt c = geo(&b)(m, n), c0 = geo(&b)(r.m0, r.n0);
-        if (m == r.m0 && n == r.n0) { kc[0] = ld(hr, c0); kc[1] = ld(mu, c0); }
+        if (m == r.m0 && n == r.n0) {
+            kc[0] = ld(hr, c0); kc[1] = ld(mu, c0);
+            if (fbits64(ld(mu, c0)) != 0) OCN_ATOMIC_OR(flag + 1, 1);
+        }
         if (fbits64(ld(hr, c)) != fbits64(ld(hr, c0))) OCN_ATOMIC_OR(flag, 1);
         if (m < r.m0 - 1 || m > r.m1 + 1 || n < r.n0 - 1 || n > r.n1 + 1) return;
         if (fbits64(ld(mu, c)) != fbits64(ld(mu, c0))) OCN_ATOMIC_OR(flag, 2);
@@ -2842,6 +2965,18 @@
     g.ntiles = g.r[0].tiles;
     int ex;
     const bool p2 = std::frexp(tau, &ex) == 0.5 && ex > -1020 && ex < 1020;
+    if (kc.nv && !last && (kc.mode == OCN_KC_KNOWN || kc.mode == OCN_KC_KNOWN_HR)) {
+#define OCN_PAIR_NV(P, H)                                                                                        \
+    return issue_march(g, MarchStepT<P, false, true, false, H, true, false, true>{*b, t, sw, tau, nbad1, sshp_out,   \
+                                                                                  up_out, vp_out, kc.kc, nullptr, 0, \
+                                                                                  0u, nbad2}, s)
+        const bool hr = kc.mode == OCN_KC_KNOWN_HR;
+        if (p2 && hr) OCN_PAIR_NV(true, true);
+        if (hr) OCN_PAIR_NV(false, true);
+        if (p2) OCN_PAIR_NV(true, false);
+        OCN_PAIR_NV(false, false);
+#undef OCN_PAIR_NV
+    }
 #define OCN_PAIR_LAUNCH(P, L, Z, H)                                                                              \
     return issue_march(g, MarchStep<P, L, Z, false, H, true>{*b, t, sw, tau, nbad1, sshp_out, up_out, vp_out,        \
                                                              kc.kc, nullptr, 0, 0u, nbad2}, s)
@@ -2903,6 +3038,17 @@
         return issue_march(g, body, s);
     };
     const bool p2 = std::frexp(tau, &ex) == 0.5 && ex > -1020 && ex < 1020;
+    if (kc.nv) {
+        const bool hr = kc.mode == OCN_KC_KNOWN_HR;
+#define OCN_X4_NV(P, H)                                                                                              \
+    return go(MarchStepT<P, false, true, true, H, true, false, true>{*bx, t, sw, tau, nbad1, sshp_out, up_out, vp_out, \
+                                                                    kc.kc, nullptr, 0, own, nbad2})
+        if (p2 && hr) OCN_X4_NV(true, true);
+        if (hr) OCN_X4_NV(false, true);
+        if (p2) OCN_X4_NV(true, false);
+        OCN_X4_NV(false, false);
+#undef OCN_X4_NV
+    }
     if (kc.mode == OCN_KC_KNOWN_HR) {
         if (p2)
             return go(MarchStep<true, false, true, true, true, true>{*bx, t, sw, tau, nbad1, sshp_out, up_out, vp_out,
@@ -2946,6 +3092,7 @@
     for (int k = 0; k < kNumRowFields; ++k)
         v[k] = e >= 0 ? ext[e * kNumRowFields + k] : rows[(unsigned)k * nrows + (r - kXRing)];
     if (!write_table_row(rows4, nrows4, r, v)) atomicOr(flags, (int)OCN_COMPACT_DIVISOR_RANGE);
+    if (!row_inviscid(v)) atomicOr(flags, (int)OCN_COMPACT_VISCOUS_ROW);
 }
 
 int launch_x4_tables(const ocn_block *g, const uint8_t *bits, const float *rows, const float *ext, uint8_t *bits4,
diff --git a/ocean_model_arch_amd/csrc/sw_stencils.h b/ocean_model_arch_amd/csrc/sw_stencils.h
--- a/ocean_model_arch_amd/csrc/sw_stencils.h
+++ b/ocean_model_arch_amd/csrc/sw_stencils.h
@@ -731,7 +731,8 @@
 enum { OCN_COMPACT_MASK_NOT_BINARY = 1, OCN_COMPACT_METRIC_NOT_ROW_CONSTANT = 2,
        OCN_COMPACT_RING_SEA = 4,
        OCN_COMPACT_DIVISOR_RANGE = 8,
-       OCN_COMPACT_EDGE_RING_SEA = 16 };
+       OCN_COMPACT_EDGE_RING_SEA = 16,
+       OCN_COMPACT_VISCOUS_ROW = 32 };
 
 OCN_HD inline unsigned own_class(int v, int lo, int hi) { return v < lo ? 0u : v > hi ? 2u : 1u; }
 
@@ -751,6 +752,15 @@
         range &= g[k] >= 0x1p-60f && g[k] <= 0x1p60f;
     }
     return range;
+}
+
+OCN_HD inline bool row_inviscid(const float *v)
+{
+    auto finite = [](float a) { return (fbits(a) & 0x7f800000u) != 0x7f800000u; };
+    bool ok = fbits(v[OCN_R_DISS - OCN_DX]) == 0u;
+    for (int k = 0; k < kNumRowFields; ++k) ok &= finite(v[k]);
+    const float dx = v[0], dy = v[OCN_DY - OCN_DX], dxb = v[OCN_DXB - OCN_DX], dyb = v[OCN_DYB - OCN_DX];
+    return ok && finite(dy / dx) && finite(dx / dy) && finite(dxb / dyb) && finite(dyb / dxb);
 }
 
 struct Prepare {
@@ -796,6 +806,7 @@
             vary |= fbits(v[k]) != fbits(ld(r4[OCN_DX + k], q0));
         }
         if (m == ms && !write_table_row(rows, nrows, q.r, v)) OCN_ATOMIC_OR(flags, (int)OCN_COMPACT_DIVISOR_RANGE);
+        if (m == ms && !row_inviscid(v)) OCN_ATOMIC_OR(flags, (int)OCN_COMPACT_VISCOUS_ROW);
         if (vary) OCN_ATOMIC_OR(flags, (int)OCN_COMPACT_METRIC_NOT_ROW_CONSTANT);
     }
 };
diff --git a/ocean_model_arch_amd/model.py b/ocean_model_arch_amd/model.py
--- a/ocean_model_arch_amd/model.py
+++ b/ocean_model_arch_amd/model.py
@@ -228,6 +228,14 @@
     def co_launched(self) -> bool:
         return self.option(_lib.OPT_CO_LAUNCH) == 2
 
+    def set_inviscid(self, on: bool = True):
+        check(lib().ocn_ctx_set_option(self.ctx, _lib.OPT_INVISCID, int(on)), "ocn_ctx_set_option")
+        return self
+
+    @property
+    def onepass_inviscid(self) -> bool:
+        return self.option(_lib.OPT_INVISCID) == 2
+
     def set_multi_spin(self, polls: int):
         check(lib().ocn_ctx_set_option(self.ctx, _lib.OPT_MULTI_SPIN, int(polls)), "ocn_ctx_set_option")
         return self
```

After: 67.07 billion, median of 6. +10.7%, better.
